# Moryu-Io/Roboken-FMSKF-robot-controller

Hardware: AMD Instinct MI355X
Metric: KF predict+update steps/s (whole node), 6-state fp32, at 1/2/4/8 MI355X (higher is better)
Workload: dtype f32; 1 GPU; cfg2: 2^20 independent 6-state fp32 KF instances per GPU, fused correct+predict per tick (fmskf_tick; every ensemble_every-th tick fmskf_tick_ensemble_begin: the tick kernel also writes the ensemble record, its fold carried by the next tick, libfmskf's ncclAllGather + copy-out on a side stream, fmskf_ensemble_end two events later); instances_per_gpu=1048576, global_instances=1048576, trig=table512, inputs=records, ensemble_every=16, ensemble=fused, gather=native, parallelism=instance-sharded x1

## Files before the change

roboken-fmskf-robot-controller_amd/csrc/api_comm.cpp:

```cpp
#include <dlfcn.h>
#include <elf.h>

#include <atomic>

#include "api_ctx.hpp"

using namespace fmskf;
using namespace fmskf::capi;

namespace fmskf {
namespace capi {

bool ens_exchanges(const fmskf_ctx *h) { return h->comm && h->world > 1; }
double *ens_fold_dst(const fmskf_ctx *h, const fmskf_ctx::EnsSlot &S) { return ens_exchanges(h) ? S.rec : S.host_dev; }
void ens_gather_async(fmskf_ctx *h, fmskf_ctx::EnsSlot &S);
void ens_fold_queued(fmskf_ctx *h, fmskf_ctx::EnsSlot &S) {
  if (ens_exchanges(h)) ens_gather_async(h, S);
  else hip_check(hipEventRecord(S.done, h->stream), "hipEventRecord");
  h->ens_carry = -1;
}
fmskf_ctx::EnsSlot *ens_carry_attach(fmskf_ctx *h, TickIn &t) {
  if (h->ens_carry < 0) return nullptr;
  fmskf_ctx::EnsSlot &C = h->eslot[h->ens_carry];
  t.fold_blocks = C.blocks;
  t.fold_nb = (uint32_t)C.nb;
  t.fold_out = ens_fold_dst(h, C);
  t.ens_shift = h->ens_shift;
  if (!ens_exchanges(h) && !h->timing) t.ens_done = C.done;
  return &C;
}
void ens_carry_launched(fmskf_ctx *h, fmskf_ctx::EnsSlot *C, const TickIn &t) {
  if (!C) return;
  if (t.ens_done) h->ens_carry = -1;
  else ens_fold_queued(h, *C);
}
bool ens_carry_plain() { return FMSKF_ENV_INT("FMSKF_ENS_CARRY_PLAIN", 1) != 0; }
void ens_flush(fmskf_ctx *h) {
  if (h->ens_carry < 0) return;
  fmskf_ctx::EnsSlot &S = h->eslot[h->ens_carry];
  launch_check(launch_ens_fold((int)h->d.nx, S.blocks, S.nb, h->ens_shift, ens_fold_dst(h, S), h->stream),
               "ensemble fold launch");
  ens_fold_queued(h, S);
}

void ensure_shift(fmskf_ctx *h) {
  if (h->ens_shift_ok) return;
  if (h->capturing) fail(FMSKF_EINVAL, "ensemble shift first taken inside a graph capture");
  ens_flush(h);
  launch_check(launch_ens_shift(h->s, (int)h->d.nx, h->d.elem == 8, h->ens_shift, h->stream),
               "ensemble shift launch");
  h->ens_shift_ok = true;
}

bool fused_record(const fmskf_ctx *h) {
  return (h->cfg.model == FMSKF_MODEL_KF6 && !h->gate_on) ||
         (h->cfg.model == FMSKF_MODEL_EKF9 && h->s.tile && !h->rowgate_on) ||
         (h->cfg.model == FMSKF_MODEL_KF12D && h->s.tile && h->kf12.decor);
}

}
}

namespace {

struct RcclApi {
  bool ok = false;
  std::string why;
  std::string path;
  ncclResult_t (*get_unique_id)(ncclUniqueId *) = nullptr;
  ncclResult_t (*comm_init_rank)(ncclComm_t *, int, ncclUniqueId, int) = nullptr;
  ncclResult_t (*comm_destroy)(ncclComm_t) = nullptr;
  ncclResult_t (*all_gather)(const void *, void *, size_t, ncclDataType_t, ncclComm_t, hipStream_t) = nullptr;
  ncclResult_t (*comm_count)(const ncclComm_t, int *) = nullptr;
  ncclResult_t (*comm_user_rank)(const ncclComm_t, int *) = nullptr;
  const char *(*error_string)(ncclResult_t) = nullptr;
};

bool elf_exports(const char *path, const char *name) {
  FILE *f = fopen(path, "rb");
  if (!f) return false;
  std::vector<unsigned char> img;
  unsigned char buf[1 << 16];
  size_t got;
  while ((got = fread(buf, 1, sizeof(buf), f)) > 0 && img.size() < ((size_t)256 << 20)) img.insert(img.end(), buf, buf + got);
  fclose(f);
  if (img.size() < sizeof(Elf64_Ehdr) || memcmp(img.data(), ELFMAG, SELFMAG) != 0 || img[EI_CLASS] != ELFCLASS64)
    return false;
  Elf64_Ehdr eh;
  memcpy(&eh, img.data(), sizeof(eh));
  const uint64_t size = img.size();
  auto within = [size](uint64_t off, uint64_t len) { return off <= size && len <= size - off; };
  if (eh.e_shentsize != sizeof(Elf64_Shdr) || eh.e_shoff > size ||
      eh.e_shnum > (size - eh.e_shoff) / sizeof(Elf64_Shdr))
    return false;
  auto shdr = [&](uint32_t k) {
    Elf64_Shdr sh;
    memcpy(&sh, img.data() + eh.e_shoff + (uint64_t)k * sizeof(Elf64_Shdr), sizeof(sh));
    return sh;
  };
  const size_t nlen = strlen(name);
  for (uint32_t k = 0; k < eh.e_shnum; k++) {
    const Elf64_Shdr sy = shdr(k);
    if (sy.sh_type != SHT_DYNSYM || sy.sh_link >= eh.e_shnum || !within(sy.sh_offset, sy.sh_size)) continue;
    const Elf64_Shdr st = shdr(sy.sh_link);
    if (!within(st.sh_offset, st.sh_size)) continue;
    for (uint64_t o = 0; o + sizeof(Elf64_Sym) <= sy.sh_size; o += sizeof(Elf64_Sym)) {
      Elf64_Sym sym;
      memcpy(&sym, img.data() + sy.sh_offset + o, sizeof(sym));
      if (sym.st_shndx == SHN_UNDEF || sym.st_name >= st.sh_size || nlen >= st.sh_size - sym.st_name) continue;
      if (memcmp(img.data() + st.sh_offset + sym.st_name, name, nlen + 1) == 0) return true;
    }
  }
  return false;
}

std::atomic<const RcclApi *> g_rccl_loaded{nullptr};

const RcclApi &rccl() {
  static RcclApi api = [] {
    RcclApi a;
    const char *alt = getenv("FMSKF_RCCL_LIBRARY");
    void *lib = nullptr;
    if (alt && *alt) {
      if (!elf_exports(alt, "fmskf_rccl_stand_in")) {
        a.why = std::string("FMSKF_RCCL_LIBRARY=") + alt + " is not the test stand-in (no fmskf_rccl_stand_in)";
        return a;
      }
      lib = dlopen(alt, RTLD_NOW | RTLD_LOCAL);
    } else {
      lib = dlopen("librccl.so.1", RTLD_NOW | RTLD_GLOBAL);
      if (!lib) lib = dlopen("/opt/rocm/lib/librccl.so.1", RTLD_NOW | RTLD_GLOBAL);
    }
    if (!lib) {
      a.why = std::string("cannot load librccl.so.1: ") + dlerror();
      return a;
    }
    a.get_unique_id = (decltype(a.get_unique_id))dlsym(lib, "ncclGetUniqueId");
    a.comm_init_rank = (decltype(a.comm_init_rank))dlsym(lib, "ncclCommInitRank");
    a.comm_destroy = (decltype(a.comm_destroy))dlsym(lib, "ncclCommDestroy");
    a.all_gather = (decltype(a.all_gather))dlsym(lib, "ncclAllGather");
    a.comm_count = (decltype(a.comm_count))dlsym(lib, "ncclCommCount");
    a.comm_user_rank = (decltype(a.comm_user_rank))dlsym(lib, "ncclCommUserRank");
    a.error_string = (decltype(a.error_string))dlsym(lib, "ncclGetErrorString");
    a.ok = a.get_unique_id && a.comm_init_rank && a.comm_destroy && a.all_gather && a.comm_count &&
           a.comm_user_rank && a.error_string;
    if (!a.ok) a.why = "librccl.so.1 lacks an entry point";
    Dl_info di{};
    if (a.all_gather && dladdr((void *)a.all_gather, &di) && di.dli_fname) a.path = di.dli_fname;
    return a;
  }();
  g_rccl_loaded.store(&api, std::memory_order_release);
  return api;
}

const RcclApi &need_rccl() {
  const RcclApi &a = rccl();
  if (!a.ok) fail(FMSKF_ERCCL, a.why);
  return a;
}

void nccl_check(ncclResult_t r, const char *what) {
  if (r != ncclSuccess) fail(FMSKF_ERCCL, std::string(what) + ": " + rccl().error_string(r));
}

}

void fmskf::capi::ens_gather_async(fmskf_ctx *h, fmskf_ctx::EnsSlot &S) {
  if (!h->ens_stream) {
    int lo = 0, hi = 0;
    hip_check(hipDeviceGetStreamPriorityRange(&lo, &hi), "hipDeviceGetStreamPriorityRange");
    hip_check(hipStreamCreateWithPriority(&h->ens_stream, hipStreamNonBlocking, hi), "hipStreamCreate");
    hip_check(hipEventCreateWithFlags(&h->ens_ticked, kSyncEvent), "hipEventCreate");
  }
  const uint32_t nx = h->d.nx, len = 1 + nx + nx * (nx + 1) / 2;
  const bool xtime = FMSKF_ENV_INT("FMSKF_ENS_XTIME", 1) != 0;
  if (xtime && !S.x0) {
    hip_check(hipEventCreate(&S.x0), "hipEventCreate");
    hip_check(hipEventCreate(&S.x1), "hipEventCreate");
  }
  hip_check(hipEventRecord(h->ens_ticked, h->stream), "hipEventRecord");
  hip_check(hipStreamWaitEvent(h->ens_stream, h->ens_ticked, 0), "hipStreamWaitEvent");
  if (xtime) hip_check(hipEventRecord(S.x0, h->ens_stream), "hipEventRecord");
  nccl_check(need_rccl().all_gather(S.rec, S.gather, len, ncclFloat64, h->comm, h->ens_stream),
             "ncclAllGather");
  hip_check(hipMemcpyAsync(S.host, S.gather, (size_t)S.ranks * len * 8, hipMemcpyDeviceToHost, h->ens_stream),
            "D2H");
  if (xtime) hip_check(hipEventRecord(S.x1, h->ens_stream), "hipEventRecord");
  hip_check(hipEventRecord(S.done, h->ens_stream), "hipEventRecord");
  S.exchanged = xtime;
}


void fmskf_ctx::destroy_comm() {
  if (comm) {
    (void)rccl().comm_destroy(comm);
    comm = nullptr;
  }
}

extern "C" {

int fmskf_comm_unique_id(uint8_t id[FMSKF_COMM_ID_BYTES]) {
  static_assert(sizeof(ncclUniqueId) == FMSKF_COMM_ID_BYTES, "RCCL unique id size");
  return guarded([&] {
    if (!id) fail(FMSKF_EINVAL, "null id");
    ncclUniqueId u;
    nccl_check(need_rccl().get_unique_id(&u), "ncclGetUniqueId");
    memcpy(id, &u, sizeof(u));
  });
}

int fmskf_comm_init(fmskf_handle h, const uint8_t id[FMSKF_COMM_ID_BYTES], int rank, int world) {
  return guarded([&] {
    check_handle(h);
    if (!id || world < 1 || rank < 0 || rank >= world) fail(FMSKF_EINVAL, "bad rank / world / id");
    if (h->ens_pending) fail(FMSKF_EINVAL, "collect the pending ensemble results (fmskf_ensemble_end) first");
    const RcclApi &a = need_rccl();
    DeviceGuard g(h->cfg.device);
    h->destroy_comm();
    h->rank = 0;
    h->world = 1;
    if ((size_t)world > h->ens_gather_cap) {
      double *buf = h->alloc<double>((size_t)world * 91);
      h->release(h->ens_gather);
      h->ens_gather = buf;
      h->ens_gather_cap = (size_t)world;
    }
    ncclUniqueId u;
    memcpy(&u, id, sizeof(u));
    ncclComm_t c = nullptr;
    nccl_check(a.comm_init_rank(&c, world, u, rank), "ncclCommInitRank");
    h->comm = c;
    h->rank = rank;
    h->world = world;
  });
}

int fmskf_comm_info(fmskf_handle h, int *world, int *rank) {
  return guarded([&] {
    check_handle(h);
    if (!h->comm) fail(FMSKF_EINVAL, "the handle has no communicator (fmskf_comm_init)");
    const RcclApi &a = need_rccl();
    int w = 0, r = -1;
    nccl_check(a.comm_count(h->comm, &w), "ncclCommCount");
    nccl_check(a.comm_user_rank(h->comm, &r), "ncclCommUserRank");
    if (world) *world = w;
    if (rank) *rank = r;
  });
}

const char *fmskf_rccl_library(void) {
  const RcclApi *a = g_rccl_loaded.load(std::memory_order_acquire);
  return a ? a->path.c_str() : "";
}

int fmskf_ensemble_stats(fmskf_handle h, double *mean, double *cov_packed) {
  return guarded([&] {
    check_handle(h);
    DeviceGuard g(h->cfg.device);
    const uint32_t nx = h->d.nx, len = 1 + nx + nx * (nx + 1) / 2;
    ensure_shift(h);
    launch_check(launch_ensemble(h->s, (int)nx, h->d.elem == 8, h->ens_blocks, h->ens_shift, h->ens_out,
                                 h->stream),
                 "ensemble launch");
    const double *src = h->ens_out;
    int ranks = 1;
    if (h->comm) {
      nccl_check(need_rccl().all_gather(h->ens_out, h->ens_gather, len, ncclFloat64, h->comm,
                                        h->stream),
                 "ncclAllGather");
      src = h->ens_gather;
      ranks = h->world;
    }
    std::vector<double> recs((size_t)ranks * len);
    hip_check(hipMemcpyAsync(recs.data(), src, recs.size() * 8, hipMemcpyDeviceToHost, h->stream),
              "D2H");
    hip_check(hipStreamSynchronize(h->stream), "hipStreamSynchronize");
    const int rc = fmskf_ensemble_combine(nx, recs.data(), (uint32_t)ranks, mean, cov_packed);
    if (rc != FMSKF_OK) fail(rc, "ensemble combine");
  });
}

}

namespace {


void ens_async_begin(fmskf_ctx *h, const fmskf_tick_inputs *in) {
  check_handle(h);
  if (h->capturing) fail(FMSKF_EINVAL, "asynchronous ensemble inside a graph capture");
  if (h->ens_pending == fmskf_ctx::kEnsSlots)
    fail(FMSKF_EINVAL, "four ensemble results pending: call fmskf_ensemble_end first");
  DeviceGuard g(h->cfg.device);
  const uint32_t nx = h->d.nx, len = 1 + nx + nx * (nx + 1) / 2;
  const int ranks = ens_exchanges(h) ? h->world : 1;
  const int si = (h->ens_head + h->ens_pending) % fmskf_ctx::kEnsSlots;
  fmskf_ctx::EnsSlot &S = h->eslot[si];
  if (!S.blocks) {
    size_t nb = (size_t)ensemble_nblocks(h->s.n);
    nb = std::max(nb, (size_t)((h->s.n + kBlock - 1) / kBlock));
    S.blocks = h->alloc<double>(nb * len);
    S.rec = h->alloc<double>(91);
    hip_check(hipEventCreateWithFlags(&S.done, kSyncEvent), "hipEventCreate");
  }
  if ((size_t)ranks > S.cap) {
    double *gbuf = h->alloc<double>((size_t)ranks * 91);
    if (S.gather) h->release(S.gather);
    S.gather = gbuf;
    if (S.host) hip_check(hipHostFree(S.host), "hipHostFree");
    S.host = nullptr;
    hip_check(hipHostMalloc((void **)&S.host, (size_t)ranks * 91 * 8, hipHostMallocMapped | hipHostMallocCoherent),
              "hipHostMalloc");
    S.host_dev = (double *)fmskf_ctx::dev_ptr(S.host);
    S.cap = (size_t)ranks;
  }
  ensure_shift(h);
  int nb = 0;
  if (in && fused_record(h)) {
    TickIn t = resolve_inputs(h, in, true, true, 1, h->s.n);
    t.ens_blocks = S.blocks;
    t.ens_shift = h->ens_shift;
    fmskf_ctx::EnsSlot *C = ens_carry_attach(h, t);
    const bool libm = h->cfg.trig == FMSKF_TRIG_LIBM;
    h->time_begin();
    int e = 0;
    if (h->cfg.model == FMSKF_MODEL_KF6) e = launch_kf6(h->s, t, h->kf6, libm, true, true, h->stream, &nb);
    else if (h->cfg.model == FMSKF_MODEL_EKF9) e = launch_ekf9(h->s, t, h->ekf9, libm, true, true, h->stream, &nb);
    else e = launch_kf12d(h->s, t, h->kf12, true, true, h->stream, &nb);
    launch_check(e, "tick kernel launch");
    h->time_end();
    ens_carry_launched(h, C, t);
  } else {
    ens_flush(h);
    if (in) run_tick(h, in, true, true, 1, h->s.n);
    launch_check(launch_ens_partial(h->s, (int)nx, h->d.elem == 8, S.blocks, h->ens_shift, h->stream, &nb),
                 "ensemble partial launch");
  }
  S.nb = nb;
  S.ranks = ranks;
  S.exchanged = false;
  h->ens_carry = si;
  h->ens_pending++;
}

}

extern "C" {

int fmskf_tick_ensemble_begin(fmskf_handle h, const fmskf_tick_inputs *in) {
  return guarded([&] {
    if (!in) fail(FMSKF_EINVAL, "null inputs");
    ens_async_begin(h, in);
  });
}

int fmskf_ensemble_begin(fmskf_handle h) {
  return guarded([&] { ens_async_begin(h, nullptr); });
}

int fmskf_ensemble_end(fmskf_handle h, double *mean, double *cov_packed) {
  return fmskf_ensemble_end_count(h, mean, cov_packed, nullptr, nullptr);
}

int fmskf_ensemble_end_count(fmskf_handle h, double *mean, double *cov_packed, double *count,
                             uint32_t *n_records) {
  return guarded([&] {
    check_handle(h);
    if (h->ens_pending == 0) fail(FMSKF_EINVAL, "no ensemble pending (fmskf_*ensemble_begin)");
    DeviceGuard g(h->cfg.device);
    fmskf_ctx::EnsSlot &S = h->eslot[h->ens_head];
    if (h->ens_carry == h->ens_head) {
      if (h->capturing) fail(FMSKF_EINVAL, "the newest ensemble result collected inside a graph capture");
      ens_flush(h);
    }
    hip_check(hipEventSynchronize(S.done), "hipEventSynchronize");
    h->ens_xms = -1.f;
    if (S.exchanged) {
      hip_check(hipEventElapsedTime(&h->ens_xms, S.x0, S.x1), "hipEventElapsedTime");
      S.exchanged = false;
    }
    h->ens_head = (h->ens_head + 1) % fmskf_ctx::kEnsSlots;
    h->ens_pending--;
    const int rc = fmskf_ensemble_combine(h->d.nx, S.host, (uint32_t)S.ranks, mean, cov_packed);
    if (rc != FMSKF_OK) fail(rc, "ensemble combine");
    const uint32_t len = 1 + h->d.nx + h->d.nx * (h->d.nx + 1) / 2;
    double c = 0.0;
    for (int r = 0; r < S.ranks; r++) c += S.host[(size_t)r * len];
    if (count) *count = c;
    if (n_records) *n_records = (uint32_t)S.ranks;
  });
}

int fmskf_ensemble_exchange_ms(fmskf_handle h, float *ms) {
  return guarded([&] {
    check_handle(h);
    if (!ms) fail(FMSKF_EINVAL, "null ms");
    *ms = h->ens_xms;
  });
}

}
```

roboken-fmskf-robot-controller_amd/csrc/api_ctrl.cpp:

```cpp
#include "api_ctx.hpp"

using namespace fmskf;
using namespace fmskf::capi;

namespace {

void ctrl_params_defaults(fmskf_ctrl_params *p) {
  memset(p, 0, sizeof(*p));
  p->ctrl_freq_hz = 100.0f;
  p->ff_gain = 0.0075f;
  p->p_gain = 0.02f;
  p->i_gain = 0.01f;
  p->d_gain = 0.0f;
  p->i_limit = 0.5f;
  p->lpf_freq_hz = 10.0f;
  p->ff_limit = 1.0f;
  p->interp_ts = 1.0f / (float)1000;
  p->curr_limit_raw = 3000;
}

CtrlPrm make_ctrl_prm(const fmskf_ctx *h) {
  const fmskf_ctrl_params &c = h->cprm;
  CtrlPrm p{};
  p.freq = c.ctrl_freq_hz;
  p.dt = 1.0f / c.ctrl_freq_hz;
  p.ff_gain = c.ff_gain;
  p.p_gain = c.p_gain;
  p.i_gain = c.i_gain;
  p.d_gain = c.d_gain;
  p.i_limit = c.i_limit;
  p.ff_limit = c.ff_limit;
  p.a1 = (2.0f * c.ctrl_freq_hz - c.lpf_freq_hz) / (2.0f * c.ctrl_freq_hz + c.lpf_freq_hz);
  p.b0 = c.lpf_freq_hz / (2.0f * c.ctrl_freq_hz + c.lpf_freq_hz);
  p.b1 = c.lpf_freq_hz / (2.0f * c.ctrl_freq_hz + c.lpf_freq_hz);
  p.ts = c.interp_ts;
  p.curr_limit = c.curr_limit_raw;
  for (int w = 0; w < 4; w++) p.dir[w] = h->cfg.motor_dir[w];
  return p;
}

CtrlPrm ctrl_step_prm(fmskf_ctx *h) {
  CtrlPrm p = make_ctrl_prm(h);
  p.store_derived = h->capturing ? 1u : 0u;
  if (h->capturing) {
    h->graph_has_ctrl = true;
  } else {
    h->ctrl_prm_last = p;
    h->ctrl_derived_stale = true;
  }
  return p;
}

}

namespace fmskf {
namespace capi {

void ctrl_materialize(fmskf_ctx *h) {
  if (!h->ctrl_ready || !h->ctrl_derived_stale) return;
  launch_check(launch_ctrl_derive(h->ctrl, h->ctrl_prm_last, h->stream), "control outputs");
  h->ctrl_derived_stale = false;
}

void zero_ctrl(fmskf_ctx *h) {
  CtrlDev &c = h->ctrl;
  hip_check(hipMemsetAsync(c.ax, 0, (size_t)3 * kAxF * c.pitch * 4, h->stream), "ctrl init");
  hip_check(hipMemsetAsync(c.pid, 0, (size_t)4 * kPidF * c.pitch * 4, h->stream), "ctrl init");
  hip_check(hipMemsetAsync(c.vel_tgt, 0, (size_t)3 * c.pitch * 4, h->stream), "ctrl init");
  hip_check(hipMemsetAsync(c.rpm_prev, 0, (size_t)4 * c.n * 2, h->stream), "ctrl init");
  hip_check(hipMemsetAsync(c.curr, 0, (size_t)4 * c.n * 2, h->stream), "ctrl init");
  hip_check(hipMemsetAsync(c.power, 0, (size_t)c.n, h->stream), "ctrl init");
  ctrl_params_defaults(&h->cprm);
  h->ctrl_derived_stale = false;
}

void ensure_ctrl(fmskf_ctx *h) {
  if (h->ctrl_ready) return;
  CtrlDev &c = h->ctrl;
  c.n = h->s.n;
  const uint64_t w = tile_w_elem(4);
  c.pitch = std::max(h->s.pitch, (c.n + w - 1) / w * w);
  c.ax = h->alloc<float>((size_t)3 * kAxF * c.pitch);
  c.pid = h->alloc<float>((size_t)4 * kPidF * c.pitch);
  c.vel_tgt = h->alloc<float>((size_t)3 * c.pitch);
  c.rpm_prev = h->alloc<int16_t>((size_t)4 * c.n);
  c.curr = h->alloc<int16_t>((size_t)4 * c.n);
  c.power = h->alloc<uint8_t>((size_t)c.n);
  zero_ctrl(h);
  h->ctrl_ready = true;
}

}
}

extern "C" {

int fmskf_ctrl_params_init(fmskf_ctrl_params *p) {
  return guarded([&] {
    if (!p) fail(FMSKF_EINVAL, "null params");
    ctrl_params_defaults(p);
  });
}

int fmskf_set_ctrl_params(fmskf_handle h, const fmskf_ctrl_params *p) {
  return guarded([&] {
    check_handle(h);
    if (!p) fail(FMSKF_EINVAL, "null params");
    if (!(p->ctrl_freq_hz > 0.0f) || !(p->interp_ts > 0.0f) || p->curr_limit_raw < 0)
      fail(FMSKF_EINVAL, "ctrl params: freq and ts must be > 0, current limit >= 0");
    DeviceGuard g(h->cfg.device);
    ensure_ctrl(h);
    h->cprm = *p;
  });
}

int fmskf_set_power(fmskf_handle h, const uint8_t *on, uint32_t mem) {
  return guarded([&] {
    check_handle(h);
    DeviceGuard g(h->cfg.device);
    ensure_ctrl(h);
    ctrl_materialize(h);
    const uint64_t n = h->s.n;
    if (!on) {
      hip_check(hipMemsetAsync(h->ctrl.power, 1, n, h->stream), "power");
      return;
    }
    if (mem != FMSKF_MEM_HOST && mem != FMSKF_MEM_DEVICE) fail(FMSKF_EINVAL, "bad mem flag");
    hip_check(hipMemcpyAsync(h->ctrl.power, on, n,
                             mem == FMSKF_MEM_HOST ? hipMemcpyHostToDevice : hipMemcpyDeviceToDevice,
                             h->stream),
              "power");
    finish_out(h, mem);
  });
}

int fmskf_set_target_vel(fmskf_handle h, const float *vel, const float *acl, const float *jrk,
                         const uint8_t *mask, uint32_t mem) {
  return guarded([&] {
    check_handle(h);
    if (!vel || !acl || !jrk) fail(FMSKF_EINVAL, "null vel/acl/jrk");
    DeviceGuard g(h->cfg.device);
    ensure_ctrl(h);
    const uint64_t n = h->s.n;
    Stager sg(h, mem);
    const void *v = vel, *a = acl, *j = jrk, *m = mask;
    sg.add(&v, 3 * n * 4);
    sg.add(&a, 3 * n * 4);
    sg.add(&j, 3 * n * 4);
    sg.add(&m, n);
    sg.run();
    launch_check(launch_ctrl_set_target(h->ctrl, (const float *)v, (const float *)a,
                                        (const float *)j, (const uint8_t *)m, h->stream),
                 "set_target_vel launch");
  });
}

int fmskf_control(fmskf_handle h, const int16_t *rpm, uint32_t mem) {
  return guarded([&] {
    check_handle(h);
    DeviceGuard g(h->cfg.device);
    ensure_ctrl(h);
    const void *r = rpm;
    if (r) {
      Stager sg(h, mem);
      sg.add(&r, h->s.n * 8);
      sg.run();
    } else {
      ensure_motors(h);
      r = h->s.m_rpm;
    }
    h->time_begin();
    launch_check(launch_ctrl_step(h->ctrl, ctrl_step_prm(h), (const int16_t *)r, 1, h->stream),
                 "control launch");
    h->time_end();
  });
}

int fmskf_can_tx(fmskf_handle h, uint8_t *frames, uint32_t mem) {
  return guarded([&] {
    check_handle(h);
    if (!frames) fail(FMSKF_EINVAL, "null frames");
    if (mem != FMSKF_MEM_HOST && mem != FMSKF_MEM_DEVICE) fail(FMSKF_EINVAL, "bad mem flag");
    DeviceGuard g(h->cfg.device);
    ensure_ctrl(h);
    const size_t bytes = h->s.n * 8;
    uint8_t *dst = mem == FMSKF_MEM_DEVICE ? frames : (uint8_t *)host_result(h, bytes);
    launch_check(launch_can_tx(h->ctrl, dst, h->stream), "can_tx launch");
    copy_out_sync(h, frames, dst, bytes, mem);
  });
}

static bool rs_prev_skip() { return FMSKF_ENV_INT("FMSKF_RS_PREV_SKIP", 1) != 0; }
static bool isr_kf6_fused() { return FMSKF_ENV_INT("FMSKF_ISR_FUSED", 1) != 0; }

static void isr_launches(fmskf_ctx *h, const TickIn &t, uint8_t *dst) {
  const bool libm = h->cfg.trig == FMSKF_TRIG_LIBM;
  const CtrlPrm p = ctrl_step_prm(h);
  int fused = (int)hipErrorNotSupported;
  if (h->cfg.model == FMSKF_MODEL_KF6 && isr_kf6_fused() && !h->gate_on) {
    if (!t.rec && !t.rpm) ensure_motors(h);
    fused = launch_isr_kf6(h->s, t, h->kf6, libm, h->ctrl, p, dst, h->stream);
    if (fused != (int)hipErrorNotSupported) launch_check(fused, "isr launch");
  } else if (h->cfg.model == FMSKF_MODEL_EKF9 && isr_kf6_fused() && !h->rowgate_on) {
    if (!t.rpm) ensure_motors(h);
    fused = launch_isr_ekf9(h->s, t, h->ekf9, libm, h->ctrl, p, t.rpm ? t.rpm : h->s.m_rpm, dst, h->stream);
    if (fused != (int)hipErrorNotSupported) launch_check(fused, "isr launch");
  }
  if (h->cfg.model == FMSKF_MODEL_RS) {
    rs_prev_materialize(h);
    launch_check(launch_isr_rs(h->s, t, libm, h->ctrl, p, dst, h->stream), "isr launch");
    h->rs_prev_synced = t.msum_lo != nullptr;
  } else if (fused == (int)hipErrorNotSupported) {
    h->isr_ctrl_split++;
    int e = 0;
    switch (h->cfg.model) {
      case FMSKF_MODEL_KF6: e = kf6_tick_launch(h, t, libm, true, true); break;
      case FMSKF_MODEL_EKF9: e = ekf9_tick_launch(h, t, libm, true, true); break;
      case FMSKF_MODEL_KF12D: e = launch_kf12d(h->s, t, h->kf12, true, true, h->stream); break;
    }
    launch_check(e, "tick kernel launch");
    if (!t.rec && !t.rpm) ensure_motors(h);
    const int16_t *rpm = t.rec ? (const int16_t *)(t.rec + 2) : t.rpm ? t.rpm : h->s.m_rpm;
    launch_check(launch_ctrl_step(h->ctrl, p, rpm, t.rec ? 2 : 1, h->stream), "control launch");
    if (dst) launch_check(launch_can_tx(h->ctrl, dst, h->stream), "can_tx launch");
  }
}

int fmskf_isr_tick(fmskf_handle h, const fmskf_tick_inputs *in, uint8_t *frames, uint32_t mem) {
  return guarded([&] {
    check_handle(h);
    if (frames && mem != FMSKF_MEM_HOST && mem != FMSKF_MEM_DEVICE) fail(FMSKF_EINVAL, "bad mem flag");
    DeviceGuard g(h->cfg.device);
    ensure_ctrl(h);
    const uint64_t n = h->s.n;
    const TickIn t = resolve_inputs(h, in, true, true, 1, n);
    const size_t bytes = n * 8;
    uint8_t *dst = !frames ? nullptr : mem == FMSKF_MEM_DEVICE ? frames : (uint8_t *)host_result(h, bytes);
    h->time_begin();
    isr_launches(h, t, dst);
    h->time_end();
    if (frames) copy_out_sync(h, frames, dst, bytes, mem);
  });
}

int fmskf_isr_tick_can(fmskf_handle h, const uint8_t *can_frames, const int16_t *can_stamps,
                       const fmskf_tick_inputs *in, uint8_t *frames, uint32_t mem) {
  return guarded([&] {
    check_handle(h);
    if (!can_frames || !can_stamps) fail(FMSKF_EINVAL, "null can_frames/can_stamps");
    if (!in) fail(FMSKF_EINVAL, "null inputs");
    if (mem != FMSKF_MEM_HOST && mem != FMSKF_MEM_DEVICE) fail(FMSKF_EINVAL, "bad mem flag");
    DeviceGuard g(h->cfg.device);
    ensure_ctrl(h);
    ensure_motors(h);
    const uint64_t n = h->s.n;
    const void *f = can_frames, *s = can_stamps;
    std::vector<std::pair<const void **, size_t>> cf{{&f, n * 32}, {&s, n * 8}};
    const bool together = in->mem == mem;
    const TickIn t = resolve_inputs(h, in, true, true, 1, n, together ? &cf : nullptr);
    if (!together) {
      Stager sg(h, mem);
      for (const auto &it : cf) sg.add(it.first, it.second);
      sg.run();
    }
    const bool libm = h->cfg.trig == FMSKF_TRIG_LIBM;
    const size_t bytes = n * 8;
    uint8_t *dst = !frames ? nullptr : mem == FMSKF_MEM_DEVICE ? frames : (uint8_t *)host_result(h, bytes);
    int fused = (int)hipErrorNotSupported;
    h->time_begin();
    if (h->cfg.model == FMSKF_MODEL_KF6 && isr_kf6_fused() && !h->gate_on && !in->kf6_rec && !in->rpm) {
      fused = launch_isr_kf6_can(h->s, t, h->kf6, libm, h->ctrl, ctrl_step_prm(h), dst, (const uint8_t *)f,
                                 (const int16_t *)s, h->cfg.motor_dir, h->stream);
    } else if (h->cfg.model == FMSKF_MODEL_EKF9 && isr_kf6_fused() && !h->rowgate_on && !in->rpm) {
      fused = launch_isr_ekf9_can(h->s, t, h->ekf9, libm, h->ctrl, ctrl_step_prm(h), dst, (const uint8_t *)f,
                                  (const int16_t *)s, h->cfg.motor_dir, h->stream);
    } else if (h->cfg.model == FMSKF_MODEL_RS && !in->rpm && !in->angle_sum) {
      const bool ps = h->rs_prev_synced && !h->capturing && rs_prev_skip();
      if (!ps) rs_prev_materialize(h);
      fused = launch_isr_rs_can(h->s, t, libm, h->ctrl, ctrl_step_prm(h), dst, (const uint8_t *)f,
                                (const int16_t *)s, h->cfg.motor_dir, ps, h->stream);
      if (fused != (int)hipErrorNotSupported) {
        h->rs_prev_synced = true;
        h->rs_prev_stale = h->rs_prev_stale || ps;
      }
    }
    if (fused != (int)hipErrorNotSupported) {
      launch_check(fused, "isr+can launch");
      h->s.m_par ^= 1u;
    }
    if (fused == (int)hipErrorNotSupported) {
      h->isr_can_split++;
      rs_prev_materialize(h);
      h->rs_prev_synced = false;
      launch_check(launch_can(h->s, (const uint8_t *)f, (const int16_t *)s, nullptr, h->cfg.motor_dir, h->stream),
                   "can launch");
      h->s.m_par ^= 1u;
      isr_launches(h, t, dst);
    }
    h->time_end();
    if (frames) copy_out_sync(h, frames, dst, bytes, mem);
  });
}

int fmskf_get_ctrl(fmskf_handle h, float *vel_tgt, int16_t *curr_raw, float *wheel_tgt,
                   float *wheel_ctrl, uint32_t mem) {
  return guarded([&] {
    check_handle(h);
    DeviceGuard g(h->cfg.device);
    ensure_ctrl(h);
    ctrl_materialize(h);
    const CtrlDev &c = h->ctrl;
    const size_t row = c.n * 4, pb = c.pitch * 4;
    copy_planes_out(h, vel_tgt, c.vel_tgt, row, pb, 3, mem);
    copy_out(h, curr_raw, c.curr, c.n * 8, mem);
    if (wheel_tgt || wheel_ctrl) {
      float *dense = (float *)h->stage_for((size_t)4 * kPidF * row);
      launch_check(launch_untile(c.pid, dense, 4 * kPidF, c.n, 4, h->stream), "untile pid");
      copy_planes_out(h, wheel_tgt, dense + 4 * c.n, row, row * kPidF, 4, mem);
      copy_planes_out(h, wheel_ctrl, dense + 5 * c.n, row, row * kPidF, 4, mem);
    }
    finish_out(h, mem);
  });
}

int fmskf_export_vehicle_info(fmskf_handle h, fmskf_vehicle_info *out, const uint8_t *floor,
                              const float *cam_pitch, const uint32_t *fault, uint32_t mem) {
  static_assert(sizeof(fmskf_vehicle_info) == 84, "VehicleInfo record layout");
  return guarded([&] {
    check_handle(h);
    if (!out) fail(FMSKF_EINVAL, "null out");
    DeviceGuard g(h->cfg.device);
    const uint64_t n = h->s.n;
    ensure_imu(h);
    Stager sg(h, mem);
    const void *f = floor, *c = cam_pitch, *u = fault;
    sg.add(&f, n * 8);
    sg.add(&c, n * 4);
    sg.add(&u, n * 4);
    sg.run();
    launch_check(launch_readout(h->s, h->readout, h->stream), "readout");
    const size_t bytes = n * sizeof(fmskf_vehicle_info);
    void *dst = mem == FMSKF_MEM_DEVICE ? (void *)out : host_result(h, bytes);
    launch_check(launch_vehicle_info(h->s, h->readout, dst, (const uint8_t *)f, (const float *)c,
                                     (const uint32_t *)u, h->stream),
                 "vehicle_info launch");
    copy_out_sync(h, out, dst, bytes, mem);
  });
}

int fmskf_eval_trig(fmskf_handle h, const float *x, float *s, float *c, uint64_t n, uint32_t mem) {
  return guarded([&] {
    check_handle(h);
    if (!x || !s || !c) fail(FMSKF_EINVAL, "null argument");
    DeviceGuard g(h->cfg.device);
    const bool libm = h->cfg.trig == FMSKF_TRIG_LIBM;
    if (mem == FMSKF_MEM_DEVICE) {
      launch_check(launch_trig(x, s, c, n, libm, h->s.sintab, h->stream), "trig launch");
      return;
    }
    if (mem != FMSKF_MEM_HOST) fail(FMSKF_EINVAL, "bad mem flag");
    if (n == 0) return;
    char *buf = (char *)h->stage_for(3 * n * 4);
    float *dx = (float *)buf, *ds = dx + n, *dc = ds + n;
    hip_check(hipMemcpyAsync(dx, x, n * 4, hipMemcpyHostToDevice, h->stream), "H2D");
    launch_check(launch_trig(dx, ds, dc, n, libm, h->s.sintab, h->stream), "trig launch");
    hip_check(hipMemcpyAsync(s, ds, n * 4, hipMemcpyDeviceToHost, h->stream), "D2H");
    hip_check(hipMemcpyAsync(c, dc, n * 4, hipMemcpyDeviceToHost, h->stream), "D2H");
    hip_check(hipStreamSynchronize(h->stream), "sync");
  });
}

int fmskf_set_timing(fmskf_handle h, int enable) {
  return guarded([&] {
    check_handle(h);
    h->timing = enable != 0;
    h->tcount = 0;
  });
}

int fmskf_kernel_time_total(fmskf_handle h, double *total_ms, uint32_t *count) {
  return guarded([&] {
    check_handle(h);
    if (!total_ms || !count) fail(FMSKF_EINVAL, "null argument");
    DeviceGuard g(h->cfg.device);
    double sum = 0.0;
    if (h->tcount) hip_check(hipEventSynchronize(h->tpool[2 * h->tcount - 1]), "hipEventSynchronize");
    for (size_t k = 0; k < h->tcount; k++) {
      float ms = 0.f;
      hip_check(hipEventElapsedTime(&ms, h->tpool[2 * k], h->tpool[2 * k + 1]), "hipEventElapsedTime");
      sum += ms;
    }
    *total_ms = sum;
    *count = (uint32_t)h->tcount;
  });
}

int fmskf_last_kernel_ms(fmskf_handle h, float *ms) {
  return guarded([&] {
    check_handle(h);
    if (!ms) fail(FMSKF_EINVAL, "null ms");
    if (!h->timing) fail(FMSKF_EINVAL, "timing not enabled");
    DeviceGuard g(h->cfg.device);
    hip_check(hipEventSynchronize(h->ev1), "hipEventSynchronize");
    hip_check(hipEventElapsedTime(ms, h->ev0, h->ev1), "hipEventElapsedTime");
  });
}

}
```

roboken-fmskf-robot-controller_amd/csrc/api_ctx.hpp:

```cpp
#pragma once
#include "../../include/fmskf.h"

#include <hip/hip_runtime.h>
#include <math.h>
#include <rccl/rccl.h>
#include <stdio.h>
#include <stdlib.h>
#include <string.h>

#include <algorithm>
#include <string>
#include <vector>

#include "fmskf_internal.hpp"
#include "window_pieces.hpp"

namespace fmskf {
namespace capi {

extern thread_local std::string g_last_error;

struct ApiError {
  int code;
  std::string msg;
};

[[noreturn]] inline void fail(int code, const std::string &msg) { throw ApiError{code, msg}; }

inline void hip_check(hipError_t e, const char *what) {
  if (e != hipSuccess) fail(FMSKF_EDEVICE, std::string(what) + ": " + hipGetErrorString(e));
}
inline void launch_check(int e, const char *what) { hip_check((hipError_t)e, what); }
constexpr unsigned kSyncEvent = hipEventDisableTiming | hipEventDisableSystemFence;

template <class F>
int guarded(F &&f) {
  try {
    g_last_error.clear();
    f();
    return FMSKF_OK;
  } catch (const ApiError &e) {
    g_last_error = e.msg;
    return e.code;
  } catch (const std::bad_alloc &) {
    g_last_error = "host allocation failed";
    return FMSKF_ENOMEM;
  } catch (...) {
    g_last_error = "unexpected exception";
    return FMSKF_EDEVICE;
  }
}

struct DeviceGuard {
  int prev = -1;
  explicit DeviceGuard(int dev) {
    hip_check(hipGetDevice(&prev), "hipGetDevice");
    if (prev != dev) hip_check(hipSetDevice(dev), "hipSetDevice");
  }
  ~DeviceGuard() {
    int cur = -1;
    if (hipGetDevice(&cur) == hipSuccess && cur != prev && prev >= 0) (void)hipSetDevice(prev);
  }
};

struct Dims {
  uint32_t nx, m, elem;
};

inline Dims dims_of(uint32_t model) {
  switch (model) {
    case FMSKF_MODEL_RS: return {6, 0, 4};
    case FMSKF_MODEL_KF6: return {6, 4, 4};
    case FMSKF_MODEL_EKF9: return {9, 6, 4};
    case FMSKF_MODEL_KF12D: return {12, 8, 8};
    default: fail(FMSKF_EINVAL, "unknown model");
  }
}

}
}


struct fmskf_ctx {
  fmskf_config cfg{};
  fmskf::capi::Dims d{};
  fmskf::DevState s{};
  hipStream_t stream = nullptr;
  std::vector<void *> allocs;
  void *stage = nullptr;
  size_t stage_bytes = 0;
  static constexpr size_t kPinned = (size_t)1 << 20;
  void *pin_in[2] = {nullptr, nullptr};
  hipEvent_t pin_ev[2] = {nullptr, nullptr};
  bool pin_open[2] = {false, false};
  int pin_slot = 0;
  void *pin_out = nullptr;
  double *ens_blocks = nullptr;
  double *ens_out = nullptr;
  double *ens_shift = nullptr;
  bool ens_shift_ok = false;
  size_t ens_gather_cap = 0;
  float *readout = nullptr;
  void *oscratch = nullptr;
  size_t oscratch_bytes = 0;
  hipGraph_t graph = nullptr;
  hipGraphExec_t graph_exec = nullptr;
  bool capturing = false;
  ncclComm_t comm = nullptr;
  int rank = 0, world = 1;
  double *ens_gather = nullptr;
  static constexpr int kEnsSlots = 4;
  struct EnsSlot {
    double *blocks = nullptr, *rec = nullptr, *gather = nullptr;
    double *host = nullptr;
    double *host_dev = nullptr;
    size_t cap = 0;
    hipEvent_t done = nullptr;
    hipEvent_t x0 = nullptr, x1 = nullptr;
    bool exchanged = false;
    int nb = 0;
    int ranks = 1;
  } eslot[kEnsSlots];
  hipEvent_t ens_ticked = nullptr;
  hipStream_t ens_stream = nullptr;
  int ens_head = 0, ens_pending = 0;
  int ens_carry = -1;
  float ens_xms = -1.f;
  fmskf::CtrlDev ctrl{};
  fmskf_ctrl_params cprm{};
  bool ctrl_ready = false;
  fmskf::Kf6Params kf6{};
  fmskf::Ekf9Params ekf9{};
  fmskf::Kf12dParams kf12{};
  bool gate_on = false;
  fmskf::GateDev gate{};
  bool rowgate_on = false;
  fmskf::RowGateDev rowgate{};
  unsigned long long *fix_ignored = nullptr;
  unsigned long long *subset_ignored = nullptr;
  float *anchors = nullptr;
  std::vector<float> anchors_host;
  uint32_t n_anchors = 0;
  unsigned long long *range_ignored = nullptr;
  uint8_t *sel_flag = nullptr;
  uint32_t *sel_blk = nullptr, *sel_chunk = nullptr;
  void *smooth_ws = nullptr;
  size_t smooth_ws_bytes = 0;
  double *loglik_partial = nullptr;
  double *em_partial = nullptr;
  uint64_t isr_can_split = 0, isr_ctrl_split = 0;
  bool rs_prev_synced = false, rs_prev_stale = false;
  bool ctrl_derived_stale = false, graph_has_ctrl = false;
  uint32_t graph_par0 = 0, graph_par_end = 0;
  fmskf::CtrlPrm ctrl_prm_last{};
  bool timing = false;
  hipEvent_t ev0 = nullptr, ev1 = nullptr;
  std::vector<hipEvent_t> tpool;
  size_t tcount = 0;
  static constexpr size_t kMaxTimed = 65536;

  void time_begin() {
    if (!timing) return;
    if (tcount < kMaxTimed) {
      while (tpool.size() < 2 * (tcount + 1)) {
        hipEvent_t e;
        fmskf::capi::hip_check(hipEventCreate(&e), "hipEventCreate");
        tpool.push_back(e);
      }
      fmskf::capi::hip_check(hipEventRecord(tpool[2 * tcount], stream), "hipEventRecord");
    }
    fmskf::capi::hip_check(hipEventRecord(ev0, stream), "hipEventRecord");
  }
  void time_end() {
    if (!timing) return;
    fmskf::capi::hip_check(hipEventRecord(ev1, stream), "hipEventRecord");
    if (tcount < kMaxTimed) {
      fmskf::capi::hip_check(hipEventRecord(tpool[2 * tcount + 1], stream), "hipEventRecord");
      tcount++;
    }
  }

  template <typename T>
  T *alloc(size_t count) {
    void *p = nullptr;
    if (count == 0) count = 1;
    hipError_t e = hipMalloc(&p, count * sizeof(T));
    if (e != hipSuccess) fmskf::capi::fail(FMSKF_ENOMEM, std::string("hipMalloc: ") + hipGetErrorString(e));
    allocs.push_back(p);
    return (T *)p;
  }
  void release(void *p) {
    if (!p) return;
    for (size_t i = 0; i < allocs.size(); i++)
      if (allocs[i] == p) {
        fmskf::capi::hip_check(hipStreamSynchronize(stream), "hipStreamSynchronize");
        (void)hipFree(p);
        allocs.erase(allocs.begin() + (long)i);
        return;
      }
  }
  void *stage_for(size_t bytes) {
    if (bytes > stage_bytes) {
      if (stage) {
        fmskf::capi::hip_check(hipStreamSynchronize(stream), "hipStreamSynchronize");
        fmskf::capi::hip_check(hipFree(stage), "hipFree");
        stage = nullptr;
        stage_bytes = 0;
      }
      hipError_t e = hipMalloc(&stage, bytes);
      if (e != hipSuccess) fmskf::capi::fail(FMSKF_ENOMEM, "staging hipMalloc failed");
      stage_bytes = bytes;
    }
    return stage;
  }
  char *pinned_in() {
    const int prev = pin_slot ^ 1, slot = pin_slot;
    if (pin_open[prev]) {
      fmskf::capi::hip_check(hipEventRecord(pin_ev[prev], stream), "hipEventRecord");
      pin_open[prev] = false;
    }
    pin_slot ^= 1;
    if (!pin_in[slot]) {
      fmskf::capi::hip_check(hipHostMalloc(&pin_in[slot], kPinned, hipHostMallocDefault), "hipHostMalloc");
      fmskf::capi::hip_check(hipEventCreateWithFlags(&pin_ev[slot], fmskf::capi::kSyncEvent), "hipEventCreate");
    } else {
      fmskf::capi::hip_check(hipEventSynchronize(pin_ev[slot]), "hipEventSynchronize");
    }
    pin_open[slot] = true;
    return (char *)pin_in[slot];
  }
  char *pinned_out() {
    if (!pin_out) fmskf::capi::hip_check(hipHostMalloc(&pin_out, kPinned, hipHostMallocDefault), "hipHostMalloc");
    return (char *)pin_out;
  }
  static void *dev_ptr(void *host) {
    void *d = nullptr;
    fmskf::capi::hip_check(hipHostGetDevicePointer(&d, host, 0), "hipHostGetDevicePointer");
    return d;
  }
  void destroy_comm();
  void *out_for(size_t bytes) {
    if (bytes > oscratch_bytes) {
      if (oscratch) {
        fmskf::capi::hip_check(hipStreamSynchronize(stream), "hipStreamSynchronize");
        fmskf::capi::hip_check(hipFree(oscratch), "hipFree");
        oscratch = nullptr;
        oscratch_bytes = 0;
      }
      hipError_t e = hipMalloc(&oscratch, bytes);
      if (e != hipSuccess) {
        oscratch = nullptr;
        (void)hipGetLastError();
        fmskf::capi::fail(FMSKF_ENOMEM, "output scratch hipMalloc failed");
      }
      oscratch_bytes = bytes;
    }
    return oscratch;
  }
  ~fmskf_ctx() {
    if (ens_stream) (void)hipStreamSynchronize(ens_stream);
    if (stream) (void)hipStreamSynchronize(stream);
    else (void)hipDeviceSynchronize();
    for (void *p : allocs) (void)hipFree(p);
    if (stage) (void)hipFree(stage);
    if (oscratch) (void)hipFree(oscratch);
    if (smooth_ws) (void)hipFree(smooth_ws);
    if (loglik_partial) (void)hipFree(loglik_partial);
    if (em_partial) (void)hipFree(em_partial);
    for (int k = 0; k < 2; k++) {
      if (pin_in[k]) (void)hipHostFree(pin_in[k]);
      if (pin_ev[k]) (void)hipEventDestroy(pin_ev[k]);
    }
    if (pin_out) (void)hipHostFree(pin_out);
    for (EnsSlot &e : eslot) {
      if (e.host) (void)hipHostFree(e.host);
      if (e.done) (void)hipEventDestroy(e.done);
      if (e.x0) (void)hipEventDestroy(e.x0);
      if (e.x1) (void)hipEventDestroy(e.x1);
    }
    if (ens_ticked) (void)hipEventDestroy(ens_ticked);
    if (ens_stream) (void)hipStreamDestroy(ens_stream);
    destroy_comm();
    if (graph_exec) (void)hipGraphExecDestroy(graph_exec);
    if (graph) (void)hipGraphDestroy(graph);
    if (ev0) (void)hipEventDestroy(ev0);
    if (ev1) (void)hipEventDestroy(ev1);
    for (hipEvent_t e : tpool) (void)hipEventDestroy(e);
  }
};

namespace fmskf {
namespace capi {

inline void check_handle(fmskf_handle h) {
  if (!h) fail(FMSKF_EINVAL, "null handle");
}


struct Stager {
  fmskf_ctx *h;
  bool host;
  std::vector<std::pair<const void **, size_t>> items;
  Stager(fmskf_ctx *hh, uint32_t mem) : h(hh), host(mem == FMSKF_MEM_HOST) {
    if (mem != FMSKF_MEM_HOST && mem != FMSKF_MEM_DEVICE) fail(FMSKF_EINVAL, "bad mem flag");
  }
  void add(const void **p, size_t bytes) {
    if (*p && host) items.push_back({p, bytes});
  }
  void run() {
    if (!host || items.empty()) return;
    size_t total = 0;
    for (auto &it : items) total += (it.second + 255) & ~size_t(255);
    size_t off = 0;
    if (total <= fmskf_ctx::kPinned && !h->capturing) {
      char *pin = h->pinned_in();
      char *base = (char *)fmskf_ctx::dev_ptr(pin);
      for (auto &it : items) {
        memcpy(pin + off, *it.first, it.second);
        *it.first = base + off;
        off += (it.second + 255) & ~size_t(255);
      }
      return;
    }
    char *base = (char *)h->stage_for(total);
    for (auto &it : items) {
      hip_check(hipMemcpyAsync(base + off, *it.first, it.second, hipMemcpyHostToDevice, h->stream),
                "stage H2D");
      *it.first = base + off;
      off += (it.second + 255) & ~size_t(255);
    }
  }
};

void zero_imu(fmskf_ctx *h);
void zero_motors(fmskf_ctx *h);
void ensure_imu(fmskf_ctx *h);
void ensure_motors(fmskf_ctx *h);
void rs_prev_materialize(fmskf_ctx *h);
TickIn resolve_inputs(fmskf_ctx *h, const fmskf_tick_inputs *in, bool need_upd, bool need_pred,
                      uint32_t n_ticks, uint64_t stride,
                      const std::vector<std::pair<const void **, size_t>> *extra = nullptr);
void run_tick(fmskf_ctx *h, const fmskf_tick_inputs *in, bool upd, bool pred, uint32_t n_ticks,
              uint64_t stride);
inline int kf6_tick_launch(fmskf_ctx *h, const TickIn &t, bool libm, bool upd, bool pred) {
  if (h->gate_on && upd) return launch_kf6_gate(h->s, t, h->kf6, h->gate, libm, pred, h->stream);
  return launch_kf6(h->s, t, h->kf6, libm, upd, pred, h->stream);
}
void zero_gate(fmskf_ctx *h);
inline int ekf9_tick_launch(fmskf_ctx *h, const TickIn &t, bool libm, bool upd, bool pred) {
  if (h->rowgate_on && upd) return launch_ekf9_rowgate(h->s, t, h->ekf9, h->rowgate, libm, pred, h->stream);
  return launch_ekf9(h->s, t, h->ekf9, libm, upd, pred, h->stream);
}
void zero_rowgate(fmskf_ctx *h);
void copy_out(fmskf_ctx *h, void *dst, const void *src, size_t bytes, uint32_t mem);
void copy_planes_out(fmskf_ctx *h, void *dst, const void *src, size_t row, size_t dev_pitch,
                     size_t planes, uint32_t mem);
void copy_planes_in(fmskf_ctx *h, void *dst, const void *src, size_t row, size_t dev_pitch,
                    size_t planes, uint32_t mem);
void finish_out(fmskf_ctx *h, uint32_t mem);
void *host_result(fmskf_ctx *h, size_t bytes);
void copy_out_sync(fmskf_ctx *h, void *dst, const void *src, size_t bytes, uint32_t mem);
void check_list_model(const fmskf_ctx *h, const char *what);
struct EntryOut {
  float *value = nullptr;
  uint8_t *status = nullptr;
  EntryOut(fmskf_ctx *h, float *value, uint8_t *status, uint64_t count, uint32_t mem);
  void deliver();

 private:
  fmskf_ctx *h;
  float *user_value;
  uint8_t *user_status;
  size_t count;
  uint32_t mem;
  char *res = nullptr;
};
double *ens_fold_dst(const fmskf_ctx *h, const fmskf_ctx::EnsSlot &S);
void ens_fold_queued(fmskf_ctx *h, fmskf_ctx::EnsSlot &S);
fmskf_ctx::EnsSlot *ens_carry_attach(fmskf_ctx *h, TickIn &t);
void ens_carry_launched(fmskf_ctx *h, fmskf_ctx::EnsSlot *C, const TickIn &t);
bool ens_carry_plain();
void ens_flush(fmskf_ctx *h);
void ensure_shift(fmskf_ctx *h);
bool fused_record(const fmskf_ctx *h);
SmoothHist smooth_hist(fmskf_ctx *h, uint32_t n_ticks);
void ensure_ctrl(fmskf_ctx *h);
void zero_ctrl(fmskf_ctx *h);
void ctrl_materialize(fmskf_ctx *h);


inline void check_window_model(const fmskf_ctx *h, const char *what) {
  const std::string w(what);
  if (h->cfg.model != FMSKF_MODEL_KF6) fail(FMSKF_ENOTSUP, w + " for KF6");
  if (h->cfg.flags & FMSKF_CFG_COMP_POS) fail(FMSKF_ENOTSUP, w + " for KF6 without FMSKF_CFG_COMP_POS");
  if (h->gate_on) fail(FMSKF_ENOTSUP, w + " for a KF6 handle without a gate (fmskf_set_gate)");
}

inline uint64_t bytes_mul(uint64_t a, uint64_t b, const char *what) {
  uint64_t r;
  if (!bytes_fit(a, b, &r)) fail(FMSKF_ENOMEM, std::string(what) + " too large");
  return r;
}

template <class F>
void window_call(fmskf_ctx *h, const char *name, const char *what, uint32_t mem, uint64_t pitch, bool misaligned,
                 const fmskf_tick_inputs *in, uint32_t n_ticks, uint64_t tick_stride, F &&body) {
  const std::string w(what), captured = std::string(name) + " cannot be captured";
  if (mem != FMSKF_MEM_HOST && mem != FMSKF_MEM_DEVICE) fail(FMSKF_EINVAL, "bad mem flag");
  if (pitch && pitch < h->s.n) fail(FMSKF_EINVAL, w + " output pitch < N");
  if (n_ticks == 0) fail(FMSKF_EINVAL, "n_ticks == 0");
  if (mem == FMSKF_MEM_DEVICE && misaligned) fail(FMSKF_EINVAL, "misaligned " + w + " device output");
  if (h->capturing) fail(FMSKF_EINVAL, captured);
  DeviceGuard g(h->cfg.device);
  hipStreamCaptureStatus cs = hipStreamCaptureStatusNone;
  if (h->stream && hipStreamIsCapturing(h->stream, &cs) == hipSuccess && cs != hipStreamCaptureStatusNone)
    fail(FMSKF_EINVAL, captured);
  TickIn t = resolve_inputs(h, in, true, true, n_ticks, tick_stride);
  body(t);
}

inline double *ensure_partial(fmskf_ctx *h, double **slot, size_t K, const char *what) {
  if (!*slot) {
    const size_t blocks = (size_t)((h->s.n + kBlock - 1) / kBlock);
    const hipError_t e = hipMalloc((void **)slot, K * blocks * sizeof(double));
    if (e != hipSuccess) {
      *slot = nullptr;
      (void)hipGetLastError();
      fail(FMSKF_ENOMEM, std::string(what) + " scratch hipMalloc: " + hipGetErrorString(e));
    }
  }
  return *slot;
}

inline char *stage_pieces(fmskf_ctx *h, Piece *pc, int count, const char *what) {
  uint64_t bytes;
  if (!plan_pieces(pc, count, &bytes)) fail(FMSKF_ENOMEM, std::string(what) + " output staging too large");
  return (char *)h->out_for(bytes);
}
template <class T>
T *piece_at(char *stg, const Piece &p) {
  return p.user ? (T *)(stg + p.off) : nullptr;
}
inline void pieces_in(fmskf_ctx *h, const Piece *pc, int count, const char *what) {
  const std::string msg = std::string(what) + " outputs H2D";
  for (int k = 0; k < count; k++)
    if (pc[k].user)
      hip_check(hipMemcpy2DAsync((char *)h->oscratch + pc[k].off, pc[k].step_bytes(), pc[k].user, pc[k].step_bytes(),
                                 pc[k].row_bytes(), pc[k].rows, hipMemcpyHostToDevice, h->stream), msg.c_str());
}
inline void pieces_out(fmskf_ctx *h, const Piece *pc, int count, const char *what) {
  const std::string msg = std::string(what) + " outputs D2H";
  for (int k = 0; k < count; k++)
    if (pc[k].user)
      hip_check(hipMemcpy2DAsync(pc[k].user, pc[k].step_bytes(), (char *)h->oscratch + pc[k].off, pc[k].step_bytes(),
                                 pc[k].row_bytes(), pc[k].rows, hipMemcpyDeviceToHost, h->stream), msg.c_str());
  finish_out(h, FMSKF_MEM_HOST);
}

template <class F, class B>
void timed_passes(fmskf_ctx *h, F &&fwd, B &&bwd) {
  const char *e = env_knob("FMSKF_SMOOTH_TIME");
  const int only = !e ? 0 : !strcmp(e, "fwd") ? 1 : !strcmp(e, "bwd") ? 2 : 0;
  if (only != 2) h->time_begin();
  fwd();
  if (only == 1) h->time_end();
  if (only == 2) h->time_begin();
  bwd();
  if (only != 1) h->time_end();
}

}
}
```

roboken-fmskf-robot-controller_amd/csrc/api_handle.cpp:

```cpp
#include "api_ctx.hpp"

using namespace fmskf;
using namespace fmskf::capi;

thread_local std::string fmskf::capi::g_last_error;

namespace {

void apply_defaults(fmskf_config *c, uint32_t model, uint64_t n) {
  memset(c, 0, sizeof(*c));
  c->abi_version = FMSKF_ABI_VERSION;
  c->model = model;
  c->n_instances = n;
  c->device = 0;
  c->trig = FMSKF_TRIG_TABLE512;
  c->dt = 0.001;
  c->motor_dir[0] = 1;
  c->motor_dir[1] = 1;
  c->motor_dir[2] = -1;
  c->motor_dir[3] = -1;
  c->imu_read_reg = 0x51;
  const double dt = c->dt;
  auto setq = [&](int i, int j, double v) { c->q[i * (i + 1) / 2 + j] = v; };
  auto setr = [&](int i, int j, double v) { c->r[i * (i + 1) / 2 + j] = v; };
  auto setp = [&](int i, double v) { c->p0[i * (i + 1) / 2 + i] = v; };
  auto cv_block = [&](int p, int v, double qc) {
    setq(p, p, qc * dt * dt * dt / 3.0);
    setq(v, p, qc * dt * dt / 2.0);
    setq(v, v, qc * dt);
  };
  switch (model) {
    case FMSKF_MODEL_KF6:
      cv_block(0, 3, 4.0);
      cv_block(1, 4, 4.0);
      cv_block(2, 5, 100.0);
      setr(0, 0, 2.5e-5);
      setr(1, 1, 2.5e-3);
      setr(2, 2, 4e-4);
      setr(3, 3, 4e-4);
      setr(3, 2, 1e-5);
      for (int i = 0; i < 6; i++) setp(i, i < 3 ? 1.0 : 0.25);
      break;
    case FMSKF_MODEL_EKF9: {
      const double qd[9] = {1e-10, 1e-10, 1e-10, 4e-3 * dt, 4e-3 * dt, 100.0 * dt, 1e-12, 2500.0 * dt, 2500.0 * dt};
      for (int i = 0; i < 9; i++) setq(i, i, qd[i]);
      const double rd[6] = {2.5e-5, 2.5e-3, 0.25, 0.25, 4e-4, 4e-4};
      for (int i = 0; i < 6; i++) setr(i, i, rd[i]);
      for (int i = 0; i < 9; i++) setp(i, i < 3 ? 1.0 : (i == 6 ? 1e-2 : 0.25));
      break;
    }
    case FMSKF_MODEL_KF12D: {
      cv_block(0, 3, 4.0);
      cv_block(1, 4, 4.0);
      cv_block(2, 5, 100.0);
      cv_block(6, 9, 1.0);
      cv_block(7, 10, 1.0);
      cv_block(8, 11, 1.0);
      const double rd[8] = {2.5e-5, 2.5e-3, 4e-4, 4e-4, 1e-6, 1e-6, 1e-6, 1e-4};
      for (int i = 0; i < 8; i++) setr(i, i, rd[i]);
      setr(3, 2, 1e-5);
      for (int i = 0; i < 12; i++) setp(i, (i % 6) < 3 ? 1.0 : 0.25);
      break;
    }
    default: break;
  }
}

void convert_params(fmskf_ctx *h) {
  const fmskf_config &c = h->cfg;
  h->kf6.dt = (float)c.dt;
  for (int k = 0; k < 21; k++) h->kf6.q[k] = (float)c.q[k];
  for (int k = 0; k < 10; k++) h->kf6.r[k] = (float)c.r[k];
  h->ekf9.dt = (float)c.dt;
  for (int k = 0; k < 45; k++) h->ekf9.q[k] = (float)c.q[k];
  for (int k = 0; k < 21; k++) h->ekf9.r[k] = (float)c.r[k];
  h->kf12.dt = c.dt;
  for (int k = 0; k < 78; k++) h->kf12.q[k] = c.q[k];
  for (int k = 0; k < 36; k++) h->kf12.r[k] = c.r[k];
  for (int a = 0; a < 4; a++)
    for (int b = 0; b <= a; b++) h->kf12.r2[a * (a + 1) / 2 + b] = c.r[(a + 4) * (a + 5) / 2 + (b + 4)];
  h->kf12.decor = kf12d_cinv(h->kf12.r, h->kf12.cinv) ? 1 : 0;
  h->kf12.sparse = h->kf12.decor && kf12d_sparse(h->kf12.cinv, h->kf12.q) ? 1 : 0;
}

}

namespace fmskf {
namespace capi {

void zero_imu(fmskf_ctx *h) {
  DevState &s = h->s;
  const uint64_t n = s.n;
  hipStream_t st = h->stream;
  hip_check(hipMemsetAsync(s.imu_reg, 0, 0x90 * n * 2, st), "reset imu");
  hip_check(hipMemsetAsync(s.imu_parser, 0, 3 * n * 4, st), "reset imu");
  hip_check(hipMemsetAsync(s.imu_cnt, 0, n, st), "reset imu");
  hip_check(hipMemsetAsync(s.imu_flags, 0, n, st), "reset imu");
  hip_check(hipMemsetAsync(s.imu_err, 0, n, st), "reset imu");
  hip_check(hipMemsetAsync(s.imu_qinit, 0, 4 * n * 4, st), "reset imu");
  hip_check(hipMemsetAsync(s.imu_snap, 0, kRowWords * n * 2, st), "reset imu");
  hip_check(hipMemsetAsync(s.imu_mag, 0, 4 * n * 2, st), "reset imu");
  hip_check(hipMemsetAsync(s.imu_yg, 0, n * 4, st), "reset imu");
  hip_check(hipMemsetAsync(s.imu_qprev, 0, 4 * n * 4, st), "reset imu");
}
void zero_motors(fmskf_ctx *h) {
  DevState &s = h->s;
  const uint64_t n = s.n;
  hipStream_t st = h->stream;
  hip_check(hipMemsetAsync(s.m_micro, 0, 4 * n * 2, st), "reset motors");
  hip_check(hipMemsetAsync(s.m_angle, 0, 4 * n * 2, st), "reset motors");
  hip_check(hipMemsetAsync(s.m_prev, 0, 4 * n * 2, st), "reset motors");
  hip_check(hipMemsetAsync(s.m_rpm, 0, 4 * n * 2, st), "reset motors");
  hip_check(hipMemsetAsync(s.m_curr, 0, 4 * n * 2, st), "reset motors");
  hip_check(hipMemsetAsync(s.m_sum_lo, 0, 4 * n * 4, st), "reset motors");
  hip_check(hipMemsetAsync(s.m_sum_hi, 0, 4 * n * 4, st), "reset motors");
  hip_check(hipMemsetAsync(s.m_iir_y, 0, 4 * n * 4, st), "reset motors");
  hip_check(hipMemsetAsync(s.m_prev_micro, 0, 4 * n * 2, st), "reset motors");
}

void ensure_imu(fmskf_ctx *h) {
  DevState &s = h->s;
  if (s.imu_reg) return;
  if (h->capturing) fail(FMSKF_EINVAL, "IMU state first used inside a graph capture");
  const uint64_t n = s.n;
  s.imu_reg = h->alloc<int16_t>(0x90 * n);
  s.imu_parser = h->alloc<uint32_t>(3 * n);
  s.imu_cnt = h->alloc<uint8_t>(n);
  s.imu_flags = h->alloc<uint8_t>(n);
  s.imu_err = h->alloc<uint8_t>(n);
  s.imu_qinit = h->alloc<float>(4 * n);
  s.imu_snap = h->alloc<int16_t>(kRowWords * n);
  s.imu_mag = h->alloc<int16_t>(4 * n);
  s.imu_yg = h->alloc<uint32_t>(n);
  s.imu_qprev = h->alloc<float>(4 * n);
  zero_imu(h);
}
void rs_prev_materialize(fmskf_ctx *h) {
  if (!h->rs_prev_stale) return;
  const DevState &s = h->s;
  launch_check(launch_motor_sums(s.m_sum_lo, s.m_sum_hi, s.prev_sum, s.n, 0, true, h->stream), "previous sums");
  h->rs_prev_stale = false;
}

void zero_gate(fmskf_ctx *h) {
  if (!h->gate.word) return;
  hip_check(hipMemsetAsync(h->gate.word, 0, h->s.n * 4, h->stream), "reset gate");
  hip_check(hipMemsetAsync(h->gate.nis, 0, h->s.n * 4, h->stream), "reset gate");
}

void zero_rowgate(fmskf_ctx *h) {
  if (!h->rowgate.word) return;
  hip_check(hipMemsetAsync(h->rowgate.word, 0, h->s.n * 8, h->stream), "reset row gate");
  hip_check(hipMemsetAsync(h->rowgate.d2, 0, (size_t)FMSKF_EKF9_ROWS * h->rowgate.d2_pitch * 4, h->stream),
            "reset row gate");
}

void ensure_motors(fmskf_ctx *h) {
  DevState &s = h->s;
  if (s.m_sum_lo) return;
  if (h->capturing) fail(FMSKF_EINVAL, "motor state first used inside a graph capture");
  const uint64_t n = s.n;
  s.m_micro = h->alloc<int16_t>(4 * n);
  s.m_angle = h->alloc<int16_t>(4 * n);
  s.m_prev = h->alloc<int16_t>(4 * n);
  s.m_rpm = h->alloc<int16_t>(4 * n);
  s.m_curr = h->alloc<int16_t>(4 * n);
  s.m_sum_lo = h->alloc<uint32_t>(4 * n);
  s.m_sum_hi = h->alloc<int32_t>(4 * n);
  s.m_iir_y = h->alloc<float>(4 * n);
  s.m_prev_micro = h->alloc<int16_t>(4 * n);
  zero_motors(h);
}

}
}

namespace {

void do_reset(fmskf_ctx *h) {
  DevState &s = h->s;
  const uint64_t n = s.n;
  const Dims d = h->d;
  const uint32_t np = d.nx * (d.nx + 1) / 2;
  hipStream_t st = h->stream;
  const uint64_t pp = s.pitch;
  hip_check(hipMemsetAsync(s.x, 0, (size_t)d.nx * pp * d.elem, st), "reset x");
  if (d.m > 0) {
    std::vector<uint64_t> bits(np);
    for (uint32_t k = 0; k < np; k++) {
      const double v = h->cfg.p0[k];
      if (d.elem == 4) {
        const float f = (float)v;
        uint32_t b;
        memcpy(&b, &f, 4);
        bits[k] = b;
      } else {
        memcpy(&bits[k], &v, 8);
      }
    }
    launch_check(launch_tiled_fill(s.P, np, n, bits.data(), d.elem, st), "reset P0");
  }
  if (s.prev_sum) hip_check(hipMemsetAsync(s.prev_sum, 0, 4 * pp * 8, st), "reset prev");
  if (s.thlo) hip_check(hipMemsetAsync(s.thlo, 0, n * 4, st), "reset heading low part");
  if (s.xlo) hip_check(hipMemsetAsync(s.xlo, 0, (size_t)kKf6LoRows * pp * 4, st), "reset position low parts");
  if (s.imu_reg) zero_imu(h);
  if (s.m_sum_lo) zero_motors(h);
  zero_gate(h);
  zero_rowgate(h);
  if (h->ctrl_ready) {
    const CtrlDev &c = h->ctrl;
    hip_check(hipMemsetAsync(c.ax, 0, (size_t)3 * kAxF * c.pitch * 4, st), "reset ctrl");
    hip_check(hipMemsetAsync(c.pid, 0, (size_t)4 * kPidF * c.pitch * 4, st), "reset ctrl");
    hip_check(hipMemsetAsync(c.vel_tgt, 0, (size_t)3 * c.pitch * 4, st), "reset ctrl");
    hip_check(hipMemsetAsync(c.rpm_prev, 0, (size_t)4 * c.n * 2, st), "reset ctrl");
    hip_check(hipMemsetAsync(c.curr, 0, (size_t)4 * c.n * 2, st), "reset ctrl");
    hip_check(hipMemsetAsync(c.power, 0, (size_t)c.n, st), "reset ctrl");
  }
  hip_check(hipMemsetAsync(s.counters, 0, 8 * 8, st), "reset counters");
  hip_check(hipMemsetAsync(h->fix_ignored, 0, 8, st), "reset counters");
  hip_check(hipMemsetAsync(h->subset_ignored, 0, 8, st), "reset counters");
  hip_check(hipMemsetAsync(h->range_ignored, 0, 8, st), "reset counters");
  h->isr_can_split = h->isr_ctrl_split = 0;
  h->rs_prev_synced = h->rs_prev_stale = false;
  h->ctrl_derived_stale = false;
  h->ens_shift_ok = false;
}

}

namespace fmskf {
namespace capi {

TickIn resolve_inputs(fmskf_ctx *h, const fmskf_tick_inputs *in, bool need_upd, bool need_pred,
                      uint32_t n_ticks, uint64_t stride,
                      const std::vector<std::pair<const void **, size_t>> *extra) {
  if (!in) fail(FMSKF_EINVAL, "null inputs");
  DevState &s = h->s;
  const uint64_t n = s.n;
  if (stride < n) fail(FMSKF_EINVAL, "tick_stride < N");
  if (n_ticks == 0) fail(FMSKF_EINVAL, "n_ticks == 0");
  TickIn t{};
  t.yaw_deg = in->yaw_deg;
  t.gyro_z = in->gyro_z_dps;
  t.rpm = in->rpm;
  t.angle_sum = in->angle_sum;
  t.raw = in->raw;
  t.z = in->z;
  t.valid = in->valid;
  t.rec = (const uint32_t *)in->kf6_rec;
  t.sintab = s.sintab;
  t.stride = stride;
  t.sum_pitch = stride;
  t.n_ticks = n_ticks;
  if (t.rec && h->cfg.model != FMSKF_MODEL_KF6) fail(FMSKF_EINVAL, "kf6_rec is a KF6 input");
  if (t.rec && (t.yaw_deg || t.gyro_z || t.rpm))
    fail(FMSKF_EINVAL, "kf6_rec replaces yaw_deg / gyro_z_dps / rpm: pass one or the other");
  if (in->angle_sum_pitch) {
    if (n_ticks != 1 || stride != n) fail(FMSKF_EINVAL, "angle_sum_pitch is for single-tick calls (tick_many: tick_stride)");
    if (in->angle_sum_pitch < n) fail(FMSKF_EINVAL, "angle_sum_pitch < N");
    t.sum_pitch = in->angle_sum_pitch;
  }
  const uint64_t span = (uint64_t)(n_ticks - 1) * stride + n;
  Stager sg(h, in->mem);
  sg.add((const void **)&t.yaw_deg, span * 4);
  sg.add((const void **)&t.gyro_z, span * 4);
  sg.add((const void **)&t.rpm, span * 8);
  sg.add((const void **)&t.angle_sum, ((uint64_t)(n_ticks - 1) * stride * 4 + 3 * t.sum_pitch + n) * 8);
  sg.add((const void **)&t.raw, span * 16);
  sg.add((const void **)&t.z, ((uint64_t)(n_ticks - 1) * stride * 8 + 7 * stride + n) * 8);
  sg.add((const void **)&t.valid, span);
  sg.add((const void **)&t.rec, span * 16);
  if (extra)
    for (const auto &it : *extra) sg.add(it.first, it.second);
  sg.run();
  const bool many = n_ticks > 1 || stride != n;
  auto dev_default = [&](const void *p, const char *name) {
    if (!p && many) fail(FMSKF_EINVAL, std::string("tick_many needs explicit plane ") + name);
  };
  switch (h->cfg.model) {
    case FMSKF_MODEL_RS:
      if (need_upd) {
        dev_default(t.yaw_deg, "yaw_deg");
        if (!t.yaw_deg) {
          ensure_imu(h);
          t.yaw_deg = (const float *)s.imu_yg;
          t.imu_words |= 1u;
        }
      }
      if (need_pred) {
        dev_default(t.rpm, "rpm");
        dev_default(t.angle_sum, "angle_sum");
        if (!t.rpm || !t.angle_sum) ensure_motors(h);
        if (!t.rpm) t.rpm = s.m_rpm;
        if (!t.angle_sum) {
          t.msum_lo = s.m_sum_lo;
          t.msum_hi = s.m_sum_hi;
        }
      }
      break;
    case FMSKF_MODEL_KF6:
      if (need_upd && !t.rec) {
        dev_default(t.yaw_deg, "yaw_deg");
        dev_default(t.gyro_z, "gyro_z_dps");
        dev_default(t.rpm, "rpm");
        if (!t.yaw_deg || !t.gyro_z) ensure_imu(h);
        if (!t.rpm) ensure_motors(h);
        if (!t.yaw_deg) {
          t.yaw_deg = (const float *)s.imu_yg;
          t.imu_words |= 1u;
        }
        if (!t.gyro_z) {
          t.gyro_z = (const float *)s.imu_yg;
          t.imu_words |= 2u;
        }
        if (!t.rpm) t.rpm = s.m_rpm;
      }
      break;
    case FMSKF_MODEL_EKF9:
      if (need_upd && !t.raw) fail(FMSKF_EINVAL, "EKF9 needs raw words");
      break;
    case FMSKF_MODEL_KF12D:
      if (need_upd && !t.z) fail(FMSKF_EINVAL, "KF12D needs z");
      break;
  }
  return t;
}

void run_tick(fmskf_ctx *h, const fmskf_tick_inputs *in, bool upd, bool pred, uint32_t n_ticks,
              uint64_t stride) {
  check_handle(h);
  DeviceGuard g(h->cfg.device);
  TickIn t = resolve_inputs(h, in, upd, pred, n_ticks, stride);
  fmskf_ctx::EnsSlot *C = nullptr;
  if (!h->capturing) {
    if (h->cfg.model == FMSKF_MODEL_KF6 && fused_record(h) && upd && pred && n_ticks == 1 && ens_carry_plain())
      C = ens_carry_attach(h, t);
    else
      ens_flush(h);
  }
  const bool libm = h->cfg.trig == FMSKF_TRIG_LIBM;
  const bool rs_pred = h->cfg.model == FMSKF_MODEL_RS && pred;
  if (rs_pred) rs_prev_materialize(h);
  h->time_begin();
  int e = 0;
  switch (h->cfg.model) {
    case FMSKF_MODEL_RS: e = launch_rs(h->s, t, libm, upd, pred, h->stream); break;
    case FMSKF_MODEL_KF6: e = kf6_tick_launch(h, t, libm, upd, pred); break;
    case FMSKF_MODEL_EKF9: e = ekf9_tick_launch(h, t, libm, upd, pred); break;
    case FMSKF_MODEL_KF12D: e = launch_kf12d(h->s, t, h->kf12, upd, pred, h->stream); break;
  }
  launch_check(e, "tick kernel launch");
  ens_carry_launched(h, C, t);
  if (rs_pred) h->rs_prev_synced = t.msum_lo != nullptr;
  h->time_end();
}

void copy_out(fmskf_ctx *h, void *dst, const void *src, size_t bytes, uint32_t mem) {
  if (!dst) return;
  if (mem == FMSKF_MEM_HOST) {
    hip_check(hipMemcpyAsync(dst, src, bytes, hipMemcpyDeviceToHost, h->stream), "D2H");
  } else if (mem == FMSKF_MEM_DEVICE) {
    hip_check(hipMemcpyAsync(dst, src, bytes, hipMemcpyDeviceToDevice, h->stream), "D2D");
  } else {
    fail(FMSKF_EINVAL, "bad mem flag");
  }
}
void copy_planes_out(fmskf_ctx *h, void *dst, const void *src, size_t row, size_t dev_pitch,
                     size_t planes, uint32_t mem) {
  if (!dst) return;
  if (mem != FMSKF_MEM_HOST && mem != FMSKF_MEM_DEVICE) fail(FMSKF_EINVAL, "bad mem flag");
  const hipMemcpyKind k = mem == FMSKF_MEM_HOST ? hipMemcpyDeviceToHost : hipMemcpyDeviceToDevice;
  hip_check(hipMemcpy2DAsync(dst, row, src, dev_pitch, row, planes, k, h->stream), "copy planes");
}
void copy_planes_in(fmskf_ctx *h, void *dst, const void *src, size_t row, size_t dev_pitch,
                    size_t planes, uint32_t mem) {
  if (mem != FMSKF_MEM_HOST && mem != FMSKF_MEM_DEVICE) fail(FMSKF_EINVAL, "bad mem flag");
  const hipMemcpyKind k = mem == FMSKF_MEM_HOST ? hipMemcpyHostToDevice : hipMemcpyDeviceToDevice;
  hip_check(hipMemcpy2DAsync(dst, dev_pitch, src, row, row, planes, k, h->stream), "copy planes");
}
void finish_out(fmskf_ctx *h, uint32_t mem) {
  if (mem == FMSKF_MEM_HOST) hip_check(hipStreamSynchronize(h->stream), "hipStreamSynchronize");
}
void *host_result(fmskf_ctx *h, size_t bytes) {
  if (bytes <= fmskf_ctx::kPinned && !h->capturing) return fmskf_ctx::dev_ptr(h->pinned_out());
  return h->out_for(bytes);
}
void copy_out_sync(fmskf_ctx *h, void *dst, const void *src, size_t bytes, uint32_t mem) {
  if (mem == FMSKF_MEM_HOST && h->pin_out && src == fmskf_ctx::dev_ptr(h->pin_out)) {
    hip_check(hipStreamSynchronize(h->stream), "hipStreamSynchronize");
    memcpy(dst, h->pin_out, bytes);
    return;
  }
  if (mem == FMSKF_MEM_HOST && bytes <= fmskf_ctx::kPinned && !h->capturing) {
    char *pin = h->pinned_out();
    hip_check(hipMemcpyAsync(pin, src, bytes, hipMemcpyDeviceToHost, h->stream), "D2H");
    hip_check(hipStreamSynchronize(h->stream), "hipStreamSynchronize");
    memcpy(dst, pin, bytes);
    return;
  }
  if (mem == FMSKF_MEM_HOST) copy_out(h, dst, src, bytes, mem);
  finish_out(h, mem);
}

void check_list_model(const fmskf_ctx *h, const char *what) {
  const uint32_t model = h->cfg.model;
  const bool comp = (h->cfg.flags & FMSKF_CFG_COMP_POS) != 0;
  if ((model != FMSKF_MODEL_KF6 && model != FMSKF_MODEL_EKF9) || (model == FMSKF_MODEL_EKF9 && comp))
    fail(FMSKF_ENOTSUP, std::string(what) + " for KF6 (plain, FMSKF_CFG_COMP_POS) and plain EKF9");
}

EntryOut::EntryOut(fmskf_ctx *hh, float *v, uint8_t *s, uint64_t n, uint32_t m)
    : value(v), status(s), h(hh), user_value(v), user_status(s), count((size_t)n), mem(m) {
  if (mem != FMSKF_MEM_HOST || (!v && !s)) return;
  res = (char *)host_result(h, count * 5);
  value = v ? (float *)res : nullptr;
  status = s ? (uint8_t *)res + count * 4 : nullptr;
}
void EntryOut::deliver() {
  if (!res) return;
  if (h->pin_out && res == fmskf_ctx::dev_ptr(h->pin_out)) {
    hip_check(hipStreamSynchronize(h->stream), "hipStreamSynchronize");
    if (user_value) memcpy(user_value, h->pin_out, count * 4);
    if (user_status) memcpy(user_status, (char *)h->pin_out + count * 4, count);
  } else {
    copy_out(h, user_value, res, count * 4, mem);
    copy_out(h, user_status, res + count * 4, count, mem);
    finish_out(h, mem);
  }
}

}
}

extern "C" {

int fmskf_abi_version(void) { return (int)FMSKF_ABI_VERSION; }

const char *fmskf_strerror(int status) {
  switch (status) {
    case FMSKF_OK: return "ok";
    case FMSKF_EINVAL: return "invalid argument";
    case FMSKF_ENOMEM: return "out of memory";
    case FMSKF_EDEVICE: return "device error";
    case FMSKF_ERCCL: return "collective error";
    case FMSKF_ENOTSUP: return "not supported for this model";
    default: return "unknown status";
  }
}

const char *fmskf_last_error(void) { return g_last_error.c_str(); }

int fmskf_model_dims(uint32_t model, uint32_t *n, uint32_t *m, uint32_t *elem_bytes) {
  return guarded([&] {
    Dims d = dims_of(model);
    if (n) *n = d.nx;
    if (m) *m = d.m;
    if (elem_bytes) *elem_bytes = d.elem;
  });
}

int fmskf_config_init(fmskf_config *cfg, uint32_t model, uint64_t n) {
  return guarded([&] {
    if (!cfg) fail(FMSKF_EINVAL, "null config");
    (void)dims_of(model);
    apply_defaults(cfg, model, n);
  });
}

int fmskf_create(const fmskf_config *cfg, fmskf_handle *out) {
  return guarded([&] {
    if (!cfg || !out) fail(FMSKF_EINVAL, "null argument");
    *out = nullptr;
    if (cfg->abi_version != FMSKF_ABI_VERSION) fail(FMSKF_EINVAL, "ABI version mismatch");
    const Dims d = dims_of(cfg->model);
    if (cfg->n_instances == 0) fail(FMSKF_EINVAL, "n_instances == 0");
    if (cfg->n_instances > (1ull << 30)) fail(FMSKF_EINVAL, "n_instances > 2^30 per handle");
    if (cfg->trig > FMSKF_TRIG_LIBM) fail(FMSKF_EINVAL, "bad trig policy");
    if (!(cfg->dt > 0.0) || !isfinite(cfg->dt)) fail(FMSKF_EINVAL, "dt must be > 0");
    if (cfg->imu_read_reg + 4 > 0x90) fail(FMSKF_EINVAL, "imu_read_reg out of range");
    if ((cfg->flags & ~FMSKF_CFG_COMP_POS) || cfg->reserved) fail(FMSKF_EINVAL, "unknown config flags");
    if ((cfg->flags & FMSKF_CFG_COMP_POS) && cfg->model != FMSKF_MODEL_KF6 && cfg->model != FMSKF_MODEL_EKF9)
      fail(FMSKF_ENOTSUP, "FMSKF_CFG_COMP_POS is a KF6 / EKF9 mode");
    for (int w = 0; w < 4; w++)
      if (cfg->motor_dir[w] != 1 && cfg->motor_dir[w] != -1) fail(FMSKF_EINVAL, "motor_dir must be +-1");
    int ndev = 0;
    if (hipGetDeviceCount(&ndev) != hipSuccess || ndev == 0) fail(FMSKF_EDEVICE, "no HIP device");
    if (cfg->device < 0 || cfg->device >= ndev) fail(FMSKF_EINVAL, "bad device ordinal");
    DeviceGuard g(cfg->device);
    fmskf_ctx *h = new fmskf_ctx();
    try {
      h->cfg = *cfg;
      h->d = d;
      const uint64_t n = cfg->n_instances;
      DevState &s = h->s;
      s.n = n;
      s.model = cfg->model;
      const uint32_t np = d.nx * (d.nx + 1) / 2;
      s.tile = cfg->model == FMSKF_MODEL_RS ? 0 : tile_w_elem(d.elem);
      s.pitch = s.tile ? std::max(plane_pitch(n), (n + s.tile - 1) / s.tile * s.tile) : plane_pitch(n);
      s.x = h->alloc<char>((size_t)d.nx * s.pitch * d.elem);
      s.P = d.m ? h->alloc<char>((size_t)np * s.pitch * d.elem) : nullptr;
      s.prev_sum = cfg->model == FMSKF_MODEL_RS ? h->alloc<int64_t>(4 * s.pitch) : nullptr;
      s.thlo = cfg->model == FMSKF_MODEL_EKF9 ? h->alloc<float>(n) : nullptr;
      s.xlo = (cfg->flags & FMSKF_CFG_COMP_POS) ? h->alloc<float>((size_t)kKf6LoRows * s.pitch) : nullptr;
      h->kf6.lo = s.xlo;
      s.counters = h->alloc<unsigned long long>(8);
      h->fix_ignored = h->alloc<unsigned long long>(1);
      h->subset_ignored = h->alloc<unsigned long long>(1);
      h->range_ignored = h->alloc<unsigned long long>(1);
      h->anchors = h->alloc<float>((size_t)FMSKF_RANGE_ANCHORS_MAX * 4);
      s.sintab = h->alloc<float>(513);
      {
        const size_t len = 1 + d.nx + np;
        size_t nb = (size_t)ensemble_nblocks(n);
        if (cfg->model == FMSKF_MODEL_KF6 || cfg->model == FMSKF_MODEL_EKF9 || cfg->model == FMSKF_MODEL_KF12D)
          nb = std::max(nb, (size_t)((n + kBlock - 1) / kBlock));
        h->ens_blocks = h->alloc<double>(nb * len);
        h->ens_out = h->alloc<double>(91);
        h->ens_shift = h->alloc<double>(12);
      }
      h->readout = h->alloc<float>(6 * n);
      static const float tab[513] = {
#include "cmsis_sintab.inc"
      };
      hip_check(hipMemcpy(s.sintab, tab, sizeof(tab), hipMemcpyHostToDevice), "sintab upload");
      hip_check(hipEventCreate(&h->ev0), "hipEventCreate");
      hip_check(hipEventCreate(&h->ev1), "hipEventCreate");
      convert_params(h);
      {
        double *coef = h->alloc<double>(36 + 78);
        hip_check(hipMemcpy(coef, h->kf12.cinv, 36 * sizeof(double), hipMemcpyHostToDevice), "coef upload");
        hip_check(hipMemcpy(coef + 36, h->kf12.q, 78 * sizeof(double), hipMemcpyHostToDevice), "coef upload");
        h->kf12.coef = coef;
      }
      do_reset(h);
      hip_check(hipStreamSynchronize(h->stream), "hipStreamSynchronize");
    } catch (...) {
      delete h;
      throw;
    }
    *out = h;
  });
}

int fmskf_destroy(fmskf_handle h) {
  return guarded([&] {
    if (!h) return;
    DeviceGuard g(h->cfg.device);
    delete h;
  });
}

int fmskf_reset(fmskf_handle h) {
  return guarded([&] {
    check_handle(h);
    DeviceGuard g(h->cfg.device);
    do_reset(h);
  });
}

int fmskf_set_stream(fmskf_handle h, void *stream) {
  return guarded([&] {
    check_handle(h);
    if (h->stream != (hipStream_t)stream && !h->capturing)
      hip_check(hipStreamSynchronize(h->stream), "hipStreamSynchronize");
    h->stream = (hipStream_t)stream;
  });
}

int fmskf_graph_begin(fmskf_handle h) {
  return guarded([&] {
    check_handle(h);
    if (!h->stream) fail(FMSKF_EINVAL, "graph capture needs a stream (fmskf_set_stream)");
    if (h->capturing) fail(FMSKF_EINVAL, "capture already open");
    if (h->timing) fail(FMSKF_EINVAL, "disable per-launch timing before capturing");
    DeviceGuard g(h->cfg.device);
    ensure_imu(h);
    ensure_motors(h);
    ensure_ctrl(h);
    ensure_shift(h);
    rs_prev_materialize(h);
    h->rs_prev_synced = false;
    ctrl_materialize(h);
    h->graph_has_ctrl = false;
    h->graph_par0 = h->s.m_par;
    hip_check(hipStreamBeginCapture(h->stream, hipStreamCaptureModeThreadLocal),
              "hipStreamBeginCapture");
    h->capturing = true;
  });
}

int fmskf_graph_end(fmskf_handle h) {
  return guarded([&] {
    check_handle(h);
    if (!h->capturing) fail(FMSKF_EINVAL, "no capture open");
    DeviceGuard g(h->cfg.device);
    h->capturing = false;
    h->rs_prev_synced = false;
    h->graph_par_end = h->s.m_par;
    h->s.m_par = h->graph_par0;
    hipGraph_t gnew = nullptr;
    hip_check(hipStreamEndCapture(h->stream, &gnew), "hipStreamEndCapture");
    if (h->graph_exec) hip_check(hipGraphExecDestroy(h->graph_exec), "hipGraphExecDestroy");
    if (h->graph) hip_check(hipGraphDestroy(h->graph), "hipGraphDestroy");
    h->graph_exec = nullptr;
    h->graph = gnew;
    hip_check(hipGraphInstantiate(&h->graph_exec, h->graph, nullptr, nullptr, 0),
              "hipGraphInstantiate");
  });
}

int fmskf_graph_launch(fmskf_handle h, uint32_t times) {
  return guarded([&] {
    check_handle(h);
    if (!h->graph_exec) fail(FMSKF_EINVAL, "no graph captured");
    if (h->capturing) fail(FMSKF_EINVAL, "capture still open");
    DeviceGuard g(h->cfg.device);
    rs_prev_materialize(h);
    ctrl_materialize(h);
    for (uint32_t k = 0; k < times; k++) {
      if (h->s.m_par != h->graph_par0) {
        launch_check(launch_motor_swap(h->s, h->stream), "motor history order");
        h->s.m_par ^= 1u;
      }
      hip_check(hipGraphLaunch(h->graph_exec, h->stream), "hipGraphLaunch");
      h->s.m_par = h->graph_par_end;
    }
    h->rs_prev_synced = false;
    if (h->graph_has_ctrl && times > 0) h->ctrl_derived_stale = false;
  });
}

int fmskf_sync(fmskf_handle h) {
  return guarded([&] {
    check_handle(h);
    DeviceGuard g(h->cfg.device);
    hip_check(hipStreamSynchronize(h->stream), "hipStreamSynchronize");
  });
}

int fmskf_get_config(fmskf_handle h, fmskf_config *out) {
  return guarded([&] {
    check_handle(h);
    if (!out) fail(FMSKF_EINVAL, "null out");
    *out = h->cfg;
  });
}

int fmskf_ingest_wt901(fmskf_handle h, const uint8_t *bytes, uint32_t stride, const uint32_t *len,
                       int latch_qinit, uint32_t mem) {
  return guarded([&] {
    check_handle(h);
    if (!bytes || !len) fail(FMSKF_EINVAL, "null bytes/len");
    DeviceGuard g(h->cfg.device);
    const uint64_t n = h->s.n;
    if (mem == FMSKF_MEM_HOST) {
      for (uint64_t i = 0; i < n; i++)
        if (len[i] > stride) fail(FMSKF_EINVAL, "len[i] > stride");
    }
    ensure_imu(h);
    Stager sg(h, mem);
    const void *b = bytes, *l = len;
    sg.add(&b, (size_t)stride * n);
    sg.add(&l, n * 4);
    sg.run();
    launch_check(launch_wt901(h->s, (const uint8_t *)b, stride, (const uint32_t *)l, latch_qinit,
                              h->cfg.imu_read_reg, h->stream),
                 "wt901 launch");
  });
}

int fmskf_ingest_can(fmskf_handle h, const uint8_t *frames, const int16_t *stamps,
                     const uint8_t *present, uint32_t mem) {
  return guarded([&] {
    check_handle(h);
    if (!frames || !stamps) fail(FMSKF_EINVAL, "null frames/stamps");
    DeviceGuard g(h->cfg.device);
    const uint64_t n = h->s.n;
    ensure_motors(h);
    Stager sg(h, mem);
    const void *f = frames, *s = stamps, *p = present;
    sg.add(&f, n * 32);
    sg.add(&s, n * 8);
    sg.add(&p, n);
    sg.run();
    rs_prev_materialize(h);
    launch_check(launch_can(h->s, (const uint8_t *)f, (const int16_t *)s, (const uint8_t *)p,
                            h->cfg.motor_dir, h->stream),
                 "can launch");
    h->s.m_par ^= 1u;
    h->rs_prev_synced = false;
  });
}

int fmskf_correct(fmskf_handle h, const fmskf_tick_inputs *in) {
  return guarded([&] { run_tick(h, in, true, false, 1, h ? h->s.n : 0); });
}

int fmskf_predict(fmskf_handle h, const fmskf_tick_inputs *in) {
  return guarded([&] { run_tick(h, in, false, true, 1, h ? h->s.n : 0); });
}

int fmskf_tick(fmskf_handle h, const fmskf_tick_inputs *in) {
  return guarded([&] { run_tick(h, in, true, true, 1, h ? h->s.n : 0); });
}

int fmskf_tick_many(fmskf_handle h, const fmskf_tick_inputs *in, uint32_t n_ticks,
                    uint64_t tick_stride) {
  return guarded([&] { run_tick(h, in, true, true, n_ticks, tick_stride); });
}

int fmskf_get_pose(fmskf_handle h, float *x, float *y, float *th, uint32_t mem) {
  return guarded([&] {
    check_handle(h);
    DeviceGuard g(h->cfg.device);
    const uint64_t n = h->s.n;
    launch_check(launch_readout(h->s, h->readout, h->stream), "readout");
    copy_out(h, x, h->readout, n * 4, mem);
    copy_out(h, y, h->readout + n, n * 4, mem);
    copy_out(h, th, h->readout + 2 * n, n * 4, mem);
    finish_out(h, mem);
  });
}

int fmskf_get_vel(fmskf_handle h, float *vx, float *vy, float *vth, uint32_t mem) {
  return guarded([&] {
    check_handle(h);
    DeviceGuard g(h->cfg.device);
    const uint64_t n = h->s.n;
    launch_check(launch_readout(h->s, h->readout, h->stream), "readout");
    copy_out(h, vx, h->readout + 3 * n, n * 4, mem);
    copy_out(h, vy, h->readout + 4 * n, n * 4, mem);
    copy_out(h, vth, h->readout + 5 * n, n * 4, mem);
    finish_out(h, mem);
  });
}

int fmskf_get_state(fmskf_handle h, void *x, void *p_packed, uint32_t mem) {
  return guarded([&] {
    check_handle(h);
    DeviceGuard g(h->cfg.device);
    const uint64_t n = h->s.n;
    const Dims d = h->d;
    const size_t row = (size_t)n * d.elem, pb = (size_t)h->s.pitch * d.elem;
    const uint32_t np = d.nx * (d.nx + 1) / 2;
    if (p_packed && !d.m) fail(FMSKF_ENOTSUP, "RS model has no covariance");
    if (h->s.tile) {
      if (mem != FMSKF_MEM_HOST && mem != FMSKF_MEM_DEVICE) fail(FMSKF_EINVAL, "bad mem flag");
      auto out = [&](void *dst, const void *src, uint32_t rows) {
        if (!dst) return;
        void *dense = mem == FMSKF_MEM_DEVICE ? dst : h->out_for(row * rows);
        launch_check(launch_untile(src, dense, rows, n, d.elem, h->stream), "untile");
        if (mem == FMSKF_MEM_HOST) {
          copy_out(h, dst, dense, row * rows, mem);
          hip_check(hipStreamSynchronize(h->stream), "get_state sync");
        }
      };
      out(x, h->s.x, d.nx);
      if (p_packed) out(p_packed, h->s.P, np);
    } else {
      copy_planes_out(h, x, h->s.x, row, pb, d.nx, mem);
      if (p_packed) copy_planes_out(h, p_packed, h->s.P, row, pb, np, mem);
    }
    finish_out(h, mem);
  });
}

int fmskf_set_state(fmskf_handle h, const void *x, const void *p_packed, uint32_t mem) {
  return guarded([&] {
    check_handle(h);
    DeviceGuard g(h->cfg.device);
    const uint64_t n = h->s.n;
    const Dims d = h->d;
    if (mem != FMSKF_MEM_HOST && mem != FMSKF_MEM_DEVICE) fail(FMSKF_EINVAL, "bad mem flag");
    const size_t row = (size_t)n * d.elem, pb = (size_t)h->s.pitch * d.elem;
    const uint32_t np = d.nx * (d.nx + 1) / 2;
    if (p_packed && !d.m) fail(FMSKF_ENOTSUP, "RS model has no covariance");
    if (h->s.tile) {
      auto in = [&](void *dst, const void *src, uint32_t rows) {
        if (!src) return;
        const void *dense = src;
        if (mem == FMSKF_MEM_HOST) {
          void *stg = h->stage_for(row * rows);
          hip_check(hipMemcpyAsync(stg, src, row * rows, hipMemcpyHostToDevice, h->stream), "stage H2D");
          dense = stg;
        }
        launch_check(launch_tile(dense, dst, rows, n, d.elem, h->stream), "tile");
        if (mem == FMSKF_MEM_HOST) hip_check(hipStreamSynchronize(h->stream), "set_state sync");
      };
      in(h->s.x, x, d.nx);
      if (p_packed) in(h->s.P, p_packed, np);
    } else {
      if (x) copy_planes_in(h, h->s.x, x, row, pb, d.nx, mem);
      if (p_packed) copy_planes_in(h, h->s.P, p_packed, row, pb, np, mem);
    }
    if (x) h->ens_shift_ok = false;
    if (x && h->s.thlo) hip_check(hipMemsetAsync(h->s.thlo, 0, n * 4, h->stream), "heading low part");
    if ((x || p_packed) && h->s.xlo)
      hip_check(hipMemsetAsync(h->s.xlo, 0, (size_t)kKf6LoRows * h->s.pitch * 4, h->stream), "position low parts");
    finish_out(h, mem);
  });
}

int fmskf_set_gate(fmskf_handle h, const fmskf_gate *g) {
  return guarded([&] {
    check_handle(h);
    if (h->cfg.model != FMSKF_MODEL_KF6 || (h->cfg.flags & FMSKF_CFG_COMP_POS))
      fail(FMSKF_ENOTSUP, "the innovation gate is for KF6 without FMSKF_CFG_COMP_POS");
    if (h->capturing) fail(FMSKF_EINVAL, "gate changed inside a graph capture");
    if (!g) {
      h->gate_on = false;
      return;
    }
    if (!(g->nis_max > 0.0f)) fail(FMSKF_EINVAL, "nis_max must be > 0 (+INFINITY: monitor only)");
    DeviceGuard dg(h->cfg.device);
    if (!h->gate.word) {
      h->gate.word = h->alloc<uint32_t>(h->s.n);
      h->gate.nis = h->alloc<float>(h->s.n);
    }
    if (!h->gate_on) zero_gate(h);
    h->gate.nis_max = g->nis_max;
    h->gate.max_run = g->max_consecutive;
    h->gate_on = true;
  });
}

int fmskf_get_gate(fmskf_handle h, float *nis, uint8_t *status, uint8_t *run, uint32_t *rejects, uint32_t mem) {
  return guarded([&] {
    check_handle(h);
    if (!h->gate_on) fail(FMSKF_EINVAL, "no gate set (fmskf_set_gate)");
    if (mem != FMSKF_MEM_HOST && mem != FMSKF_MEM_DEVICE) fail(FMSKF_EINVAL, "bad mem flag");
    DeviceGuard dg(h->cfg.device);
    const uint64_t n = h->s.n;
    copy_out(h, nis, h->gate.nis, n * 4, mem);
    if (status || run || rejects) {
      if (mem == FMSKF_MEM_DEVICE) {
        launch_check(launch_gate_unpack(h->gate.word, n, status, run, rejects, h->stream), "gate readout");
      } else {
        char *scr = (char *)h->out_for(n * 6);
        launch_check(launch_gate_unpack(h->gate.word, n, (uint8_t *)scr + 4 * n, (uint8_t *)scr + 5 * n,
                                        (uint32_t *)scr, h->stream),
                     "gate readout");
        copy_out(h, rejects, scr, n * 4, mem);
        copy_out(h, status, scr + 4 * n, n, mem);
        copy_out(h, run, scr + 5 * n, n, mem);
      }
    }
    finish_out(h, mem);
  });
}

int fmskf_set_row_gate(fmskf_handle h, const fmskf_row_gate *g) {
  return guarded([&] {
    check_handle(h);
    if (h->cfg.model != FMSKF_MODEL_EKF9 || (h->cfg.flags & FMSKF_CFG_COMP_POS) || !h->s.tile)
      fail(FMSKF_ENOTSUP, "the row gate is for EKF9 without FMSKF_CFG_COMP_POS");
    if (!ekf9_r_diagonal(h->ekf9.r))
      fail(FMSKF_ENOTSUP, "the row gate needs a diagonal R (the sequential scalar update)");
    if (h->capturing) fail(FMSKF_EINVAL, "row gate changed inside a graph capture");
    if (!g) {
      h->rowgate_on = false;
      return;
    }
    for (int a = 0; a < FMSKF_EKF9_ROWS; a++)
      if (!(g->d2_max[a] > 0.0f)) fail(FMSKF_EINVAL, "d2_max entries must be > 0 (+INFINITY: never reject)");
    if (g->max_consecutive > 255) fail(FMSKF_EINVAL, "max_consecutive above 255 (the runs saturate there)");
    if (g->flags & ~FMSKF_ROW_GATE_D2) fail(FMSKF_EINVAL, "unknown row gate flags");
    DeviceGuard dg(h->cfg.device);
    if (!h->rowgate.word) {
      h->rowgate.word = h->alloc<uint64_t>(h->s.n);
      h->rowgate.d2_pitch = h->s.pitch;
      h->rowgate.d2 = h->alloc<float>((size_t)FMSKF_EKF9_ROWS * h->s.pitch);
    }
    if (!h->rowgate_on) zero_rowgate(h);
    for (int a = 0; a < FMSKF_EKF9_ROWS; a++) h->rowgate.d2_max[a] = g->d2_max[a];
    h->rowgate.max_run = g->max_consecutive;
    h->rowgate.flags = g->flags;
    h->rowgate_on = true;
  });
}

int fmskf_get_row_gate(fmskf_handle h, uint8_t *status, uint8_t *run, float *d2, uint32_t mem) {
  return guarded([&] {
    check_handle(h);
    if (!h->rowgate_on) fail(FMSKF_EINVAL, "no row gate set (fmskf_set_row_gate)");
    if (d2 && !(h->rowgate.flags & FMSKF_ROW_GATE_D2))
      fail(FMSKF_EINVAL, "d2 is kept only with FMSKF_ROW_GATE_D2");
    if (mem != FMSKF_MEM_HOST && mem != FMSKF_MEM_DEVICE) fail(FMSKF_EINVAL, "bad mem flag");
    DeviceGuard dg(h->cfg.device);
    const uint64_t n = h->s.n;
    const size_t rows = FMSKF_EKF9_ROWS;
    copy_planes_out(h, d2, h->rowgate.d2, n * 4, h->rowgate.d2_pitch * 4, rows, mem);
    if (status || run) {
      if (mem == FMSKF_MEM_DEVICE) {
        launch_check(launch_rowgate_unpack(h->rowgate.word, n, status, run, h->stream), "row gate readout");
      } else {
        uint8_t *scr = (uint8_t *)h->out_for(2 * rows * n);
        launch_check(launch_rowgate_unpack(h->rowgate.word, n, scr, scr + rows * n, h->stream), "row gate readout");
        copy_out(h, status, scr, rows * n, mem);
        copy_out(h, run, scr + rows * n, rows * n, mem);
      }
    }
    finish_out(h, mem);
  });
}

}
```

roboken-fmskf-robot-controller_amd/csrc/api_readout.cpp:

```cpp
#include "api_ctx.hpp"

using namespace fmskf;
using namespace fmskf::capi;

extern "C" {

int fmskf_get_prev_sum(fmskf_handle h, int64_t *prev, uint32_t mem) {
  return guarded([&] {
    check_handle(h);
    if (!h->s.prev_sum) fail(FMSKF_ENOTSUP, "prev_sum exists in the RS model only");
    DeviceGuard g(h->cfg.device);
    if (mem != FMSKF_MEM_HOST && mem != FMSKF_MEM_DEVICE) fail(FMSKF_EINVAL, "bad mem flag");
    rs_prev_materialize(h);
    if (!prev) return;
    const uint64_t n = h->s.n;
    int64_t *dense = mem == FMSKF_MEM_DEVICE ? prev : (int64_t *)h->out_for((size_t)4 * n * 8);
    launch_check(launch_prev_out(h->s.prev_sum, dense, n, n, h->stream), "previous sums");
    if (mem == FMSKF_MEM_HOST) copy_out(h, prev, dense, (size_t)4 * n * 8, mem);
    finish_out(h, mem);
  });
}

int fmskf_get_imu(fmskf_handle h, float *data, uint8_t *is_error, uint32_t mem) {
  return guarded([&] {
    check_handle(h);
    DeviceGuard g(h->cfg.device);
    ensure_imu(h);
    if (data) {
      if (mem != FMSKF_MEM_HOST && mem != FMSKF_MEM_DEVICE) fail(FMSKF_EINVAL, "bad mem flag");
      float *dst = mem == FMSKF_MEM_DEVICE ? data : (float *)h->out_for(16 * h->s.n * 4);
      launch_check(launch_imu_data(h->s, dst, h->stream), "imu data");
      if (mem == FMSKF_MEM_HOST) copy_out(h, data, dst, 16 * h->s.n * 4, mem);
    }
    copy_out(h, is_error, h->s.imu_err, h->s.n, mem);
    finish_out(h, mem);
  });
}

int fmskf_get_imu_regs(fmskf_handle h, int16_t *regs, uint8_t *pending, uint32_t mem) {
  return guarded([&] {
    check_handle(h);
    DeviceGuard g(h->cfg.device);
    ensure_imu(h);
    launch_check(launch_wt901_regs_sync(h->s, h->stream), "register file sync");
    copy_out(h, regs, h->s.imu_reg, 0x90 * h->s.n * 2, mem);
    copy_out(h, pending, h->s.imu_cnt, h->s.n, mem);
    finish_out(h, mem);
  });
}

int fmskf_get_motors(fmskf_handle h, int16_t *angle, int16_t *rpm, int16_t *curr,
                     int64_t *angle_sum, float *speed_radps, uint32_t mem) {
  return guarded([&] {
    check_handle(h);
    DeviceGuard g(h->cfg.device);
    if (mem != FMSKF_MEM_HOST && mem != FMSKF_MEM_DEVICE) fail(FMSKF_EINVAL, "bad mem flag");
    const uint64_t n = h->s.n;
    ensure_motors(h);
    copy_out(h, angle, motor_slots(h->s).angle, 4 * n * 2, mem);
    copy_out(h, rpm, h->s.m_rpm, 4 * n * 2, mem);
    copy_out(h, curr, h->s.m_curr, 4 * n * 2, mem);
    if (angle_sum) {
      int64_t *dense = mem == FMSKF_MEM_DEVICE ? angle_sum : (int64_t *)h->out_for((size_t)4 * n * 8);
      launch_check(launch_motor_sums(h->s.m_sum_lo, h->s.m_sum_hi, dense, n, n, false, h->stream), "motor sums");
      if (mem == FMSKF_MEM_HOST) copy_out(h, angle_sum, dense, (size_t)4 * n * 8, mem);
    }
    if (speed_radps) {
      if (mem == FMSKF_MEM_HOST) {
        std::vector<float> rows(4 * n);
        copy_out(h, rows.data(), h->s.m_iir_y, 4 * n * 4, mem);
        hip_check(hipStreamSynchronize(h->stream), "hipStreamSynchronize");
        for (uint64_t i = 0; i < n; i++)
          for (int w = 0; w < 4; w++) speed_radps[(size_t)w * n + i] = rows[4 * i + w];
      } else if (mem == FMSKF_MEM_DEVICE) {
        for (int w = 0; w < 4; w++)
          hip_check(hipMemcpy2DAsync(speed_radps + (size_t)w * n, 4, h->s.m_iir_y + w, 16, 4, n,
                                     hipMemcpyDeviceToDevice, h->stream),
                    "speed transpose");
      } else {
        fail(FMSKF_EINVAL, "bad mem flag");
      }
    }
    finish_out(h, mem);
  });
}

int fmskf_get_motor_status(fmskf_handle h, int16_t *microsec_id, int16_t *angle, int16_t *rpm,
                           int16_t *curr, float *dlt_out_angle_rad, float *speed_radps, uint32_t mem) {
  return guarded([&] {
    check_handle(h);
    if (mem != FMSKF_MEM_HOST && mem != FMSKF_MEM_DEVICE) fail(FMSKF_EINVAL, "bad mem flag");
    DeviceGuard g(h->cfg.device);
    const uint64_t n = h->s.n;
    ensure_motors(h);
    const MotorSlots ms = motor_slots(h->s);
    copy_out(h, microsec_id, ms.micro, 4 * n * 2, mem);
    copy_out(h, angle, ms.angle, 4 * n * 2, mem);
    copy_out(h, rpm, h->s.m_rpm, 4 * n * 2, mem);
    copy_out(h, curr, h->s.m_curr, 4 * n * 2, mem);
    if (dlt_out_angle_rad) {
      float *dst = mem == FMSKF_MEM_DEVICE ? dlt_out_angle_rad : (float *)h->out_for(4 * n * 4);
      launch_check(launch_motor_dlt(ms.angle, ms.prev, dst, 4 * n, h->stream), "motor dlt");
      if (mem == FMSKF_MEM_HOST) copy_out(h, dlt_out_angle_rad, dst, 4 * n * 4, mem);
    }
    copy_out(h, speed_radps, h->s.m_iir_y, 4 * n * 4, mem);
    finish_out(h, mem);
  });
}

int fmskf_get_state_lo(fmskf_handle h, float *lo, uint32_t *rows, uint32_t mem) {
  return guarded([&] {
    check_handle(h);
    if (mem != FMSKF_MEM_HOST && mem != FMSKF_MEM_DEVICE) fail(FMSKF_EINVAL, "bad mem flag");
    DeviceGuard g(h->cfg.device);
    const uint64_t n = h->s.n;
    const uint32_t rh = h->s.thlo ? 1u : 0u, rx = h->s.xlo ? kKf6LoRows : 0u;
    if (rows) *rows = rh + rx;
    if (!lo || !(rh + rx)) return;
    if (rh) copy_out(h, lo, h->s.thlo, n * 4, mem);
    if (rx) {
      float *dst = lo + (size_t)rh * n;
      void *dense = mem == FMSKF_MEM_DEVICE ? (void *)dst : h->out_for((size_t)rx * n * 4);
      launch_check(launch_untile(h->s.xlo, dense, rx, n, 4, h->stream), "untile");
      if (mem == FMSKF_MEM_HOST) copy_out(h, dst, dense, (size_t)rx * n * 4, mem);
    }
    finish_out(h, mem);
  });
}

int fmskf_set_state_lo(fmskf_handle h, const float *lo, uint32_t mem) {
  return guarded([&] {
    check_handle(h);
    if (mem != FMSKF_MEM_HOST && mem != FMSKF_MEM_DEVICE) fail(FMSKF_EINVAL, "bad mem flag");
    if (!lo) fail(FMSKF_EINVAL, "null lo");
    DeviceGuard g(h->cfg.device);
    const uint64_t n = h->s.n;
    const uint32_t rh = h->s.thlo ? 1u : 0u, rx = h->s.xlo ? kKf6LoRows : 0u, r = rh + rx;
    if (!r) fail(FMSKF_ENOTSUP, "this model keeps no low-part rows");
    const float *src = lo;
    if (mem == FMSKF_MEM_HOST) {
      void *stg = h->stage_for((size_t)r * n * 4);
      hip_check(hipMemcpyAsync(stg, lo, (size_t)r * n * 4, hipMemcpyHostToDevice, h->stream), "stage H2D");
      src = (const float *)stg;
    }
    if (rh) hip_check(hipMemcpyAsync(h->s.thlo, src, n * 4, hipMemcpyDeviceToDevice, h->stream), "lo");
    if (rx) launch_check(launch_tile(src + (size_t)rh * n, h->s.xlo, rx, n, 4, h->stream), "tile");
    h->ens_shift_ok = false;
    finish_out(h, FMSKF_MEM_HOST);
  });
}

int fmskf_get_counters(fmskf_handle h, uint64_t *counters, uint32_t n_counters) {
  return guarded([&] {
    check_handle(h);
    if (!counters || n_counters == 0) return;
    DeviceGuard g(h->cfg.device);
    unsigned long long tmp[8];
    hip_check(hipMemcpyAsync(tmp, h->s.counters, sizeof(tmp), hipMemcpyDeviceToHost, h->stream), "D2H");
    unsigned long long ignored = 0;
    hip_check(hipMemcpyAsync(&ignored, h->fix_ignored, sizeof(ignored), hipMemcpyDeviceToHost, h->stream), "D2H");
    unsigned long long sub_ignored = 0;
    hip_check(hipMemcpyAsync(&sub_ignored, h->subset_ignored, sizeof(sub_ignored), hipMemcpyDeviceToHost, h->stream),
              "D2H");
    unsigned long long rng_ignored = 0;
    hip_check(hipMemcpyAsync(&rng_ignored, h->range_ignored, sizeof(rng_ignored), hipMemcpyDeviceToHost, h->stream),
              "D2H");
    hip_check(hipStreamSynchronize(h->stream), "sync");
    tmp[1] = h->isr_can_split;
    tmp[2] = h->isr_ctrl_split;
    tmp[3] = ignored;
    tmp[4] = sub_ignored;
    tmp[5] = rng_ignored;
    for (uint32_t k = 0; k < n_counters && k < 8; k++) counters[k] = tmp[k];
  });
}

int fmskf_ensemble_record_len(fmskf_handle h, uint32_t *len) {
  return guarded([&] {
    check_handle(h);
    if (!len) fail(FMSKF_EINVAL, "null len");
    const uint32_t nx = h->d.nx;
    *len = 1 + nx + nx * (nx + 1) / 2;
  });
}

int fmskf_ensemble_partial(fmskf_handle h, double *out, uint32_t mem) {
  return guarded([&] {
    check_handle(h);
    if (!out) fail(FMSKF_EINVAL, "null out");
    DeviceGuard g(h->cfg.device);
    const uint32_t nx = h->d.nx;
    const uint32_t len = 1 + nx + nx * (nx + 1) / 2;
    double *dst = mem == FMSKF_MEM_DEVICE ? out : h->ens_out;
    ensure_shift(h);
    launch_check(launch_ensemble(h->s, (int)nx, h->d.elem == 8, h->ens_blocks, h->ens_shift, dst,
                                 h->stream),
                 "ensemble launch");
    if (mem == FMSKF_MEM_HOST) {
      copy_out(h, out, h->ens_out, len * 8, mem);
      finish_out(h, mem);
    } else if (mem != FMSKF_MEM_DEVICE) {
      fail(FMSKF_EINVAL, "bad mem flag");
    }
  });
}

int fmskf_tick_ensemble(fmskf_handle h, const fmskf_tick_inputs *in, double *out, uint32_t mem) {
  return guarded([&] {
    check_handle(h);
    if (!out) fail(FMSKF_EINVAL, "null out");
    if (mem != FMSKF_MEM_HOST && mem != FMSKF_MEM_DEVICE) fail(FMSKF_EINVAL, "bad mem flag");
    DeviceGuard g(h->cfg.device);
    const uint32_t nx = h->d.nx;
    const uint32_t len = 1 + nx + nx * (nx + 1) / 2;
    double *dst = mem == FMSKF_MEM_DEVICE ? out : h->ens_out;
    ensure_shift(h);
    if (fused_record(h)) {
      TickIn t = resolve_inputs(h, in, true, true, 1, h->s.n);
      t.ens_blocks = h->ens_blocks;
      t.ens_shift = h->ens_shift;
      int nb = 0;
      const bool libm = h->cfg.trig == FMSKF_TRIG_LIBM;
      h->time_begin();
      if (h->cfg.model == FMSKF_MODEL_KF6)
        launch_check(launch_kf6(h->s, t, h->kf6, libm, true, true, h->stream, &nb), "tick kernel launch");
      else if (h->cfg.model == FMSKF_MODEL_EKF9)
        launch_check(launch_ekf9(h->s, t, h->ekf9, libm, true, true, h->stream, &nb), "tick kernel launch");
      else
        launch_check(launch_kf12d(h->s, t, h->kf12, true, true, h->stream, &nb), "tick kernel launch");
      h->time_end();
      launch_check(launch_ens_fold((int)nx, h->ens_blocks, nb, h->ens_shift, dst, h->stream),
                   "ensemble fold launch");
    } else {
      run_tick(h, in, true, true, 1, h->s.n);
      launch_check(launch_ensemble(h->s, (int)nx, h->d.elem == 8, h->ens_blocks, h->ens_shift, dst,
                                   h->stream),
                   "ensemble launch");
    }
    if (mem == FMSKF_MEM_HOST) {
      copy_out(h, out, h->ens_out, len * 8, mem);
      finish_out(h, mem);
    }
  });
}

int fmskf_ensemble_combine(uint32_t n_state, const double *records, uint32_t n_records,
                           double *mean, double *cov_packed) {
  return guarded([&] {
    if (n_state == 0 || n_state > 12 || !records) fail(FMSKF_EINVAL, "bad arguments");
    const uint32_t nx = n_state, np = nx * (nx + 1) / 2, len = 1 + nx + np;
    std::vector<double> acc(len, 0.0);
    for (uint32_t r = 0; r < n_records; r++) {
      const double *b = records + (size_t)r * len;
      const double na = acc[0], nb = b[0];
      if (nb == 0.0) continue;
      if (na == 0.0) {
        acc.assign(b, b + len);
        continue;
      }
      const double nn = na + nb;
      double d[12];
      for (uint32_t k = 0; k < nx; k++) d[k] = b[1 + k] - acc[1 + k];
      const double f = na * nb / nn;
      for (uint32_t k = 0; k < nx; k++) acc[1 + k] = acc[1 + k] + d[k] * (nb / nn);
      for (uint32_t p = 0; p < nx; p++)
        for (uint32_t q = 0; q <= p; q++) {
          const uint32_t k = p * (p + 1) / 2 + q;
          acc[1 + nx + k] = acc[1 + nx + k] + b[1 + nx + k] + d[p] * d[q] * f;
        }
      acc[0] = nn;
    }
    if (mean)
      for (uint32_t k = 0; k < nx; k++) mean[k] = acc[1 + k];
    if (cov_packed)
      for (uint32_t k = 0; k < np; k++) cov_packed[k] = acc[0] > 1.0 ? acc[1 + nx + k] / (acc[0] - 1.0) : 0.0;
  });
}

}
```

roboken-fmskf-robot-controller_amd/csrc/fmskf_internal.hpp:

```cpp
#pragma once
#include <cstdlib>
#include <cmath>
#include <type_traits>
#include <hip/hip_runtime.h>
#include <hip/hip_ext.h>
#include <stdint.h>
#include "../../include/fmskf.h"
#include "launch_regime.hpp"

namespace fmskf {

constexpr int kBlock = 256;

constexpr int kSnapWords = 16, kRowWords = 12;
enum : int { kSnapValid = 1, kSnapLatched = 2 };

struct DevState {
  uint64_t n = 0;
  uint64_t pitch = 0;
  uint32_t tile = 0;
  uint32_t model = 0;
  void *x = nullptr;
  void *P = nullptr;
  int64_t *prev_sum = nullptr;
  float *thlo = nullptr;
  float *xlo = nullptr;
  int16_t *imu_reg = nullptr;
  uint32_t *imu_parser = nullptr;
  uint8_t *imu_cnt = nullptr;
  uint8_t *imu_flags = nullptr;
  uint8_t *imu_err = nullptr;
  float *imu_qinit = nullptr;
  int16_t *imu_snap = nullptr;
  int16_t *imu_mag = nullptr;
  uint32_t *imu_yg = nullptr;
  float *imu_qprev = nullptr;
  int16_t *m_micro = nullptr;
  int16_t *m_angle = nullptr;
  int16_t *m_prev = nullptr;
  int16_t *m_rpm = nullptr;
  int16_t *m_curr = nullptr;
  uint32_t *m_sum_lo = nullptr;
  int32_t *m_sum_hi = nullptr;
  float *m_iir_y = nullptr;
  int16_t *m_prev_micro = nullptr;
  uint32_t m_par = 0;
  unsigned long long *counters = nullptr;
  float *sintab = nullptr;
};

struct MotorSlots {
  int16_t *micro, *angle, *prev_micro, *prev;
};
inline MotorSlots motor_slots(const DevState &s) {
  return s.m_par ? MotorSlots{s.m_prev_micro, s.m_prev, s.m_micro, s.m_angle}
                 : MotorSlots{s.m_micro, s.m_angle, s.m_prev_micro, s.m_prev};
}

struct TickIn {
  const float *yaw_deg;
  const float *gyro_z;
  const int16_t *rpm;
  const int64_t *angle_sum;
  const int16_t *raw;
  const double *z;
  const uint8_t *valid;
  const uint32_t *rec;
  const float *sintab;
  uint64_t stride;
  uint64_t sum_pitch;
  const uint32_t *msum_lo;
  const int32_t *msum_hi;
  uint32_t n_ticks;
  double *ens_blocks;
  const double *ens_shift;
  uint32_t ens_grid;
  uint32_t fold_nb;
  const double *fold_blocks;
  double *fold_out;
  hipEvent_t ens_done;
  uint32_t imu_words;
};

template <typename A>
inline void launch_signal(void (*k)(A), dim3 g, unsigned lds, hipStream_t st, hipEvent_t done, const A &a) {
  if (done) hipExtLaunchKernelGGL(k, g, dim3(kBlock), lds, st, nullptr, done, 0u, a);
  else k<<<g, kBlock, lds, st>>>(a);
}

template <typename T, int NP, int MP>
struct KfParams {
  T dt;
  T q[NP];
  T r[MP];
};
struct Kf6Params {
  float dt;
  float q[21];
  float r[10];
  float *lo;
};
struct GateDev {
  uint32_t *word;
  float *nis;
  float nis_max;
  uint32_t max_run;
};
constexpr uint32_t kGateRunShift = 2, kGateRunMax = 255, kGateRejShift = 10, kGateRejMax = (1u << 22) - 1u;
struct RowGateDev {
  uint64_t *word;
  float *d2;
  uint64_t d2_pitch;
  float d2_max[6];
  uint32_t max_run;
  uint32_t flags;
};
struct PoseFixDev {
  const uint32_t *fixes;
  uint64_t count;
  float *nis;
  uint8_t *status;
  unsigned long long *ignored;
  float r[6];
  float nis_max;
  uint32_t m;
};
struct RangeDev {
  const uint32_t *fixes;
  uint64_t count;
  const float *anchors;
  uint32_t n_anchors;
  float *d2;
  uint8_t *status;
  unsigned long long *ignored;
  float tag[3];
  float var, d2_max, d_min;
};
struct SelectDev {
  uint32_t criteria;
  float pos_var_min;
  uint32_t run_min, row_mask;
  const uint32_t *gate_word;
  const uint64_t *rowgate_word;
  uint8_t *flag;
  uint32_t *blk, *chunk;
  uint32_t *robots;
  uint8_t *reason;
  uint64_t capacity;
  uint64_t *count;
};
constexpr uint32_t kSelChunk = 256;
struct SubsetDev {
  const uint32_t *robots;
  uint64_t count;
  float *x, *p, *lo;
  unsigned long long *ignored;
  bool set;
};
struct SmoothHist {
  float *x, *P;
  uint64_t sx, sp;
};
struct SmoothOut {
  float *x, *P;
  uint64_t pitch;
};
struct LoglikOut {
  uint32_t *n_meas;
  double *nis_sum, *logdet_sum, *innov_sum, *innov_outer;
  uint64_t pitch;
  double *partial;
  uint32_t accumulate;
};
struct EmOut {
  uint32_t *n_meas;
  double *sq, *sr;
  uint64_t pitch;
  double *partial;
  uint32_t accumulate;
};
struct TraceOut {
  float *nis;
  uint8_t *status;
  uint8_t *applied;
  float *x, *P;
  uint64_t pitch;
  uint32_t every;
};
struct Ekf9Params {
  float dt;
  float q[45];
  float r[21];
  float *thlo;
  float *clo;
};
struct Kf12dParams {
  double dt;
  double q[78];
  double r[36];
  double r2[10];
  double cinv[36];
  int decor;
  int sparse;
  const double *coef;
};
inline bool kf12d_sparse(const double *cinv36, const double *q78) {
  for (int a = 0; a < 8; a++)
    for (int b = 0; b < a; b++)
      if (!(a == 3 && b == 2) && cinv36[a * (a + 1) / 2 + b] != 0.0) return false;
  auto pair = [](int s) { return s < 6 ? s % 3 : 3 + (s - 6) % 3; };
  for (int i = 0; i < 12; i++)
    for (int j = 0; j <= i; j++)
      if (pair(i) != pair(j) && q78[i * (i + 1) / 2 + j] != 0.0) return false;
  return true;
}
inline bool kf12d_cinv(const double *r, double *ci) {
  auto pk2 = [](int i, int j) { return i >= j ? i * (i + 1) / 2 + j : j * (j + 1) / 2 + i; };
  double c[8][8] = {}, v[8][8] = {};
  for (int j = 0; j < 8; j++) {
    double s = r[pk2(j, j)];
    for (int k = 0; k < j; k++) s = s - c[j][k] * c[j][k];
    if (!(s > 0.0) || !std::isfinite(s)) return false;
    c[j][j] = std::sqrt(s);
    for (int i = j + 1; i < 8; i++) {
      double t = r[pk2(i, j)];
      for (int k = 0; k < j; k++) t = t - c[i][k] * c[j][k];
      c[i][j] = t / c[j][j];
    }
  }
  for (int j = 0; j < 8; j++) {
    v[j][j] = 1.0 / c[j][j];
    for (int i = j + 1; i < 8; i++) {
      double t = 0.0;
      for (int k = j; k < i; k++) t = t + c[i][k] * v[k][j];
      v[i][j] = -t / c[i][i];
    }
  }
  for (int i = 0; i < 8; i++)
    for (int j = 0; j <= i; j++) ci[pk2(i, j)] = v[i][j];
  return true;
}
inline bool kf12d_sequential(const double *r36) {
  for (int i = 4; i < 8; i++)
    for (int j = 0; j < 4; j++)
      if (r36[i * (i + 1) / 2 + j] != 0.0) return false;
  return true;
}

inline bool ekf9_r_diagonal(const float *r21) {
  for (int i = 1; i < 6; i++)
    for (int j = 0; j < i; j++)
      if (r21[i * (i + 1) / 2 + j] != 0.0f) return false;
  return true;
}

struct CtrlDev {
  uint64_t n = 0, pitch = 0;
  float *ax = nullptr;
  float *pid = nullptr;
  float *vel_tgt = nullptr;
  int16_t *rpm_prev = nullptr;
  int16_t *curr = nullptr;
  uint8_t *power = nullptr;
};
constexpr int kAxF = 12, kPidF = 6;
struct CtrlPrm {
  float freq, dt, ff_gain, p_gain, i_gain, d_gain, i_limit, ff_limit, a1, b0, b1, ts;
  int32_t curr_limit;
  int32_t dir[4];
  uint32_t store_derived;
};

inline uint64_t plane_pitch(uint64_t n) { return ((n + 511) / 512) * 512 + 256; }

template <typename T>
constexpr uint32_t tile_w() { return sizeof(T) == 8 ? 4096u : 2048u; }
inline uint32_t tile_w_elem(uint32_t elem) { return elem == 8 ? 4096u : 2048u; }

constexpr int kStateNT = 2;
#ifndef FMSKF_ST_CACHED
#define FMSKF_ST_CACHED 16
#endif
#ifndef FMSKF_ST_STREAM
#define FMSKF_ST_STREAM 2
#endif
constexpr int st_pol(int cp) { return cp == kStateNT ? FMSKF_ST_STREAM : FMSKF_ST_CACHED; }

inline uint64_t est_state_bytes(const DevState &s) { return est_state_bytes(s.model, s.xlo != nullptr); }

inline bool kf6_small(const DevState &s) { return s.pitch * 84 < 0xFFFFFFFFull; }
inline bool ctrl_small(const CtrlDev &c) { return c.pitch * 4 * 3 * kAxF < 0xFFFFFFFFull; }

template <class F>
inline auto with_bools(F &&f) { return f(); }
template <class F, class... Bs>
inline auto with_bools(F &&f, bool b, Bs... bs) {
  return b ? with_bools([&](auto... k) { return f(std::true_type{}, k...); }, bs...)
           : with_bools([&](auto... k) { return f(std::false_type{}, k...); }, bs...);
}

__host__ __device__ inline uint64_t st_at(uint32_t tile, uint64_t pitch, uint32_t rows, uint32_t k,
                                          uint64_t i) {
  return tile ? ((i / tile) * rows + k) * tile + i % tile : k * pitch + i;
}

struct Wt901Cfg {
  uint32_t read_reg_index;
};

int launch_rs(const DevState &s, const TickIn &in, bool libm, bool correct, bool predict,
              hipStream_t st);
int launch_kf6(const DevState &s, const TickIn &in, const Kf6Params &p, bool libm, bool upd,
               bool pred, hipStream_t st, int *ens_nb = nullptr);
int launch_kf6_gate(const DevState &s, const TickIn &in, const Kf6Params &p, const GateDev &g, bool libm,
                    bool pred, hipStream_t st);
int launch_kf6_smooth_fwd(const DevState &s, const TickIn &in, const Kf6Params &p, bool libm, const SmoothHist &hist,
                          hipStream_t st);
int launch_kf6_smooth_bwd(const DevState &s, const TickIn &in, const Kf6Params &p, bool libm, const SmoothHist &hist,
                          const SmoothOut &out, hipStream_t st);
int launch_kf6_loglik(const DevState &s, const TickIn &in, const Kf6Params &p, bool libm, const LoglikOut &out,
                      double *total, hipStream_t st);
int launch_kf6_em_bwd(const DevState &s, const TickIn &in, const Kf6Params &p, bool libm, const SmoothHist &hist,
                      const EmOut &out, double *total, hipStream_t st);
int launch_kf6_trace(const DevState &s, const TickIn &in, const Kf6Params &p, const GateDev *gate, bool libm,
                     const TraceOut &out, hipStream_t st);
int launch_gate_unpack(const uint32_t *word, uint64_t n, uint8_t *status, uint8_t *run, uint32_t *rejects,
                       hipStream_t st);
int launch_pose_fix(const DevState &s, const PoseFixDev &f, hipStream_t st);
int launch_range_fix(const DevState &s, const RangeDev &f, bool libm, hipStream_t st);
int launch_select(const DevState &s, const SelectDev &d, hipStream_t st);
int launch_state_subset(const DevState &s, const SubsetDev &d, hipStream_t st);
int launch_ekf9(const DevState &s, const TickIn &in, const Ekf9Params &p, bool libm, bool upd,
                bool pred, hipStream_t st, int *ens_nb = nullptr);
int launch_ekf9_rowgate(const DevState &s, const TickIn &in, const Ekf9Params &p, const RowGateDev &g,
                        bool libm, bool pred, hipStream_t st);
int launch_rowgate_unpack(const uint64_t *word, uint64_t n, uint8_t *status, uint8_t *run, hipStream_t st);
int launch_kf12d(const DevState &s, const TickIn &in, const Kf12dParams &p, bool upd, bool pred,
                 hipStream_t st, int *ens_nb = nullptr);
int launch_wt901(const DevState &s, const uint8_t *bytes, uint32_t stride, const uint32_t *len,
                 int latch_qinit, uint32_t read_reg_index, hipStream_t st);
int launch_can(const DevState &s, const uint8_t *frames, const int16_t *stamps,
               const uint8_t *present, const int8_t dir[4], hipStream_t st);
int launch_trig(const float *x, float *sv, float *cv, uint64_t n, bool libm, const float *tab,
                hipStream_t st);
int launch_ensemble(const DevState &s, int nx, bool f64, double *blocks, const double *shift,
                    double *out, hipStream_t st);
int launch_ens_fold(int nx, const double *blocks, int nb, const double *shift, double *out,
                    hipStream_t st);
int launch_ens_partial(const DevState &s, int nx, bool f64, double *blocks, const double *shift,
                       hipStream_t st, int *nb);
int launch_ens_shift(const DevState &s, int nx, bool f64, double *shift, hipStream_t st);
int ensemble_nblocks(uint64_t n);
int launch_ctrl_set_target(const CtrlDev &c, const float *vel, const float *acl, const float *jrk,
                           const uint8_t *mask, hipStream_t st);
int launch_ctrl_derive(const CtrlDev &c, const CtrlPrm &p, hipStream_t st);
int launch_ctrl_step(const CtrlDev &c, const CtrlPrm &p, const int16_t *rpm, uint32_t rstride,
                     hipStream_t st);
int launch_can_tx(const CtrlDev &c, uint8_t *frames, hipStream_t st);
int launch_isr_kf6(const DevState &s, const TickIn &in, const Kf6Params &kp, bool libm, const CtrlDev &c,
                   const CtrlPrm &p, uint8_t *frames, hipStream_t st);
int launch_isr_kf6_can(const DevState &s, const TickIn &in, const Kf6Params &kp, bool libm, const CtrlDev &c,
                       const CtrlPrm &p, uint8_t *frames, const uint8_t *can_frames, const int16_t *can_stamps,
                       const int8_t dir[4], hipStream_t st);
int launch_isr_ekf9(const DevState &s, const TickIn &in, const Ekf9Params &prm, bool libm, const CtrlDev &c,
                    const CtrlPrm &p, const int16_t *rpm, uint8_t *frames, hipStream_t st);
int launch_isr_ekf9_can(const DevState &s, const TickIn &in, const Ekf9Params &prm, bool libm, const CtrlDev &c,
                        const CtrlPrm &p, uint8_t *frames, const uint8_t *can_frames, const int16_t *can_stamps,
                        const int8_t dir[4], hipStream_t st);
int launch_prev_out(const int64_t *prev, int64_t *dst, uint64_t n, uint64_t pitch, hipStream_t st);
int launch_motor_sums(const uint32_t *lo, const int32_t *hi, int64_t *dst, uint64_t n, uint64_t pitch, bool to_prev,
                      hipStream_t st);
int launch_wt901_regs_sync(const DevState &s, hipStream_t st);
int launch_isr_rs_can(const DevState &s, const TickIn &in, bool libm, const CtrlDev &c, const CtrlPrm &p,
                      uint8_t *frames, const uint8_t *can_frames, const int16_t *can_stamps, const int8_t dir[4],
                      bool prev_in_sums, hipStream_t st);
int launch_isr_rs(const DevState &s, const TickIn &in, bool libm, const CtrlDev &c,
                  const CtrlPrm &p, uint8_t *frames, hipStream_t st);
int launch_imu_data(const DevState &s, float *out, hipStream_t st);
int launch_vehicle_info(const DevState &s, const float *readout, void *out, const uint8_t *floor,
                        const float *cam_pitch, const uint32_t *fault, hipStream_t st);
int launch_tiled_fill(void *base, uint32_t rows, uint64_t n, const uint64_t *bits, uint32_t elem,
                      hipStream_t st);
int launch_untile(const void *tiled, void *dense, uint32_t rows, uint64_t n, uint32_t elem,
                  hipStream_t st);
int launch_tile(const void *dense, void *tiled, uint32_t rows, uint64_t n, uint32_t elem,
                hipStream_t st);
int launch_readout(const DevState &s, float *out, hipStream_t st);
int launch_motor_dlt(const int16_t *angle, const int16_t *prev, float *out, uint64_t count, hipStream_t st);
int launch_motor_swap(const DevState &s, hipStream_t st);

}
```

roboken-fmskf-robot-controller_amd/csrc/kernels_kf6.hip:

```cpp
#include "ens_device.hpp"
#include "kf6_lane.hpp"

#pragma clang fp contract(off)

namespace fmskf {

template <int WPE, class O, class A = Kf6Args>
__global__ __launch_bounds__(kBlock) __attribute__((amdgpu_waves_per_eu(WPE, 8))) void k_kf6(A aa) {
  const Kf6Args &a = kf_args(aa);
  __shared__ float stab[O::LIBM ? 1 : 513];
  const uint64_t n = a.n;
  const uint32_t i = blockIdx.x * kBlock + threadIdx.x;
  const bool live = i < (uint32_t)n;
  const uint32_t ic = live ? i : (uint32_t)n - 1u;
  const uint32_t T = a.in.n_ticks;
  float x[6], P[21];
  Kf6Lo<O> lo;
  Kf6GateOf<O, A> gt;
  Kf6In ma, mb;
  kf6_load_state<O>(a.x, a.P, a.pitch, ic, x, P);
  const auto old = kf6_keep_old<kf6_mask<O>()>(P);
  kf6_load_lo<O>(a.prm.lo, ic, lo);
  gt.load(gate_dev(aa), ic, n);
  if (O::UPD) ma = kf6_load_in<O>(a.in, n, 0, ic);
  stage_table<O::LIBM>(stab, a.in.sintab);
  for (uint32_t t = 0; t < T; t += 2) {
    if (O::UPD && t + 1 < T) mb = kf6_load_in<O>(a.in, n, t + 1, ic);
    kf6_tick1<O>(ma, stab, a.prm, x, P, lo, gt);
    if (t + 1 >= T) break;
    if (O::UPD && t + 2 < T) ma = kf6_load_in<O>(a.in, n, t + 2, ic);
    kf6_tick1<O>(mb, stab, a.prm, x, P, lo, gt);
  }
  if (live) {
    kf6_store_state<O>(a.x, a.P, a.pitch, i, x, P, old);
    kf6_store_lo<O>(a.prm.lo, i, lo);
    gt.store(gate_dev(aa), i, n);
  }
  nan_guard(x, P, a.counters, live);
}

template <int WPE, class O>
__global__ __launch_bounds__(kBlock) __attribute__((amdgpu_waves_per_eu(WPE, 8))) void k_kf6t(Kf6Args a) {
  uint32_t bid = blockIdx.x;
  if constexpr (O::ENS || O::FOLD) {
    if (ens_fold_front<6>(a.in, bid)) return;
  }
  const uint64_t n = a.n;
  const uint32_t i = bid * kBlock + threadIdx.x;
  const bool live = i < (uint32_t)n;
  const uint32_t ic = live ? i : (uint32_t)n - 1u;
  float x[6], P[21];
  Kf6In m;
  __shared__ float wtab[O::LIBM ? 1 : kBlock / 64][O::LIBM ? 1 : kWaveTab];
  float *stab = wtab[O::LIBM ? 0 : threadIdx.x >> 6];
  WaveTable<O::LIBM> tv(a.in.sintab);
  Kf6Lo<O> lo;
  Kf6Gate<O, false> gt;
  kf6_load_state<O>(a.x, a.P, a.pitch, ic, x, P);
  const auto old = kf6_keep_old<kf6_mask<O>()>(P);
  kf6_load_lo<O>(a.prm.lo, ic, lo);
  if (O::UPD) m = kf6_load_in<O>(a.in, n, 0, ic);
  tv.store(stab);
  kf6_tick1<O>(m, stab, a.prm, x, P, lo, gt);
  if (live) {
    kf6_store_state<O>(a.x, a.P, a.pitch, i, x, P, old);
    kf6_store_lo<O>(a.prm.lo, i, lo);
  }
  nan_guard(x, P, a.counters, live);
  if constexpr (O::ENS) {
    float xs[1][6];
#pragma unroll
    for (int k = 0; k < 6; k++) xs[0][k] = x[k];
    const bool lv[1] = {live};
    ens_epilogue<6, 1>(a.in, xs, lv, bid);
  }
}

template <int WPE, int R, class O, class A = Kf6Args>
__global__ __launch_bounds__(kBlock) __attribute__((amdgpu_waves_per_eu(WPE, 8))) void k_kf6p(A aa) {
  const Kf6Args &a = kf_args(aa);
  uint32_t bid = blockIdx.x;
  if constexpr (O::ENS || O::FOLD) {
    if (ens_fold_front<6>(a.in, bid)) return;
  }
  const uint64_t n = a.n;
  const uint32_t nn = (uint32_t)n, last = nn - 1u;
  const uint32_t G = (O::ENS || O::FOLD ? a.in.ens_grid : gridDim.x) * kBlock;
  const uint32_t i0 = bid * kBlock + threadIdx.x;
  float x[6], P[21];
  __shared__ float wtab[O::LIBM ? 1 : kBlock / 64][O::LIBM ? 1 : kWaveTab];
  float *stab = wtab[O::LIBM ? 0 : threadIdx.x >> 6];
  WaveTable<O::LIBM> tv(a.in.sintab);
  Kf6In m[R];
  float xs[O::ENS ? R : 1][6];
  bool lv[R];
  if (O::UPD) {
#pragma unroll
    for (int r = 0; r < R; r++) m[r] = kf6_load_in<O>(a.in, n, 0, min(i0 + r * G, last));
  }
#pragma unroll
  for (int r = 0; r < R; r++) {
    const uint32_t i = i0 + r * G;
    const bool live = i < nn;
    Kf6Lo<O> lo;
    Kf6GateOf<O, A> gt;
    kf6_load_state<O>(a.x, a.P, a.pitch, live ? i : last, x, P);
    const auto old = kf6_keep_old<kf6_mask<O>()>(P);
    kf6_load_lo<O>(a.prm.lo, live ? i : last, lo);
    gt.load(gate_dev(aa), live ? i : last, n);
    if (r == 0) tv.store(stab);
    kf6_tick1<O>(m[r], stab, a.prm, x, P, lo, gt);
    if (live) {
      kf6_store_state<O>(a.x, a.P, a.pitch, i, x, P, old);
      kf6_store_lo<O>(a.prm.lo, i, lo);
      gt.store(gate_dev(aa), i, n);
    }
    nan_guard(x, P, a.counters, live);
    if constexpr (O::ENS) {
#pragma unroll
      for (int k = 0; k < 6; k++) xs[r][k] = x[k];
    }
    lv[r] = live;
  }
  if constexpr (O::ENS) ens_epilogue<6, R>(a.in, xs, lv, bid);
}

template <class A>
static void launch_fold(void (*k)(A), A a, unsigned g, unsigned lds, hipStream_t st) {
  a.in.ens_grid = g;
  launch_signal(k, dim3(g + (unsigned)EnsRec<6>::LEN), lds, st, a.in.ens_done, a);
}

template <class O, class A>
static void launch_one(const A &aa, unsigned lds, hipStream_t st) {
  const dim3 g = grid_for(kf_args(aa).n);
  if constexpr (std::is_same<A, GateArgs>::value) k_kf6p<4, 1, O, A><<<g, kBlock, lds, st>>>(aa);
  else if constexpr (O::FOLD) launch_fold(k_kf6t<4, O>, aa, g.x, lds, st);
  else k_kf6t<4, O><<<g, kBlock, lds, st>>>(aa);
}

template <class O, class A>
static void launch_o(const A &aa, hipStream_t st) {
  constexpr bool GATED = std::is_same<A, GateArgs>::value;
  const Kf6Args &a = kf_args(aa);
  if constexpr (GATED && !O::PRED) {
    launch_one<O>(aa, 0u, st);
  } else {
    if (a.in.n_ticks != 1) {
      k_kf6<4, O, A><<<grid_for(a.n), kBlock, 0, st>>>(aa);
      return;
    }
    const LaunchRegime r = kf6_regime(a.n, O::COMP, GATED, a.in.rec != nullptr);
    constexpr bool NT = O::UPD && O::PRED;
    if (r.two) {
      const unsigned g = (unsigned)((a.n + 2 * kBlock - 1) / (2 * kBlock));
      if constexpr (NT && !GATED) {
        const bool wide = !O::COMP && kf6_wide(a.n), fold = a.in.fold_blocks != nullptr;
        if (r.nt || wide || fold) {
          with_bools([&](auto N, auto W, auto F) {
            using ON = std::conditional_t<N(), WithNT<O>, O>;
            using OW = std::conditional_t<W() && !O::COMP, WithWide<ON>, ON>;
            if constexpr (F()) launch_fold(k_kf6p<4, 2, WithFold<OW>, A>, aa, g, r.lds, st);
            else k_kf6p<4, 2, OW, A><<<g, kBlock, r.lds, st>>>(aa);
          }, r.nt, wide, fold);
          return;
        }
      }
      k_kf6p<4, 2, O, A><<<g, kBlock, r.lds, st>>>(aa);
      return;
    }
    if constexpr (NT && !GATED) {
      if (a.in.fold_blocks) {
        with_bools([&](auto N) { launch_one<WithFold<std::conditional_t<N(), WithNT<O>, O>>>(aa, r.lds, st); }, r.nt);
        return;
      }
    }
    with_bools([&](auto N) { launch_one<std::conditional_t<N() && NT, WithNT<O>, O>>(aa, r.lds, st); }, r.nt);
  }
}

template <class O>
static int launch_ens_o(KfArgs<MdKF6, Kf6Params> a, hipStream_t st) {
  using E = WithEns<O>;
  const unsigned carry = a.in.fold_blocks ? (unsigned)EnsRec<6>::LEN : 0u;
  const LaunchRegime r = kf6_ens_regime(a.n, O::COMP);
  const unsigned g = r.two ? (unsigned)((a.n + 2 * kBlock - 1) / (2 * kBlock)) : grid_for(a.n).x;
  a.in.ens_grid = g;
  with_bools([&](auto TWO, auto N, auto W) {
    using EN = std::conditional_t<N(), WithNT<E>, E>;
    if constexpr (TWO()) {
      using EW = std::conditional_t<W() && !O::COMP, WithWide<EN>, EN>;
      launch_signal(k_kf6p<4, 2, EW>, dim3(g + carry), r.lds, st, a.in.ens_done, a);
    } else if constexpr (!W()) {
      launch_signal(k_kf6t<4, EN>, dim3(g + carry), r.lds, st, a.in.ens_done, a);
    }
  }, r.two, r.nt, r.two && !O::COMP && kf6_wide(a.n));
  return (int)g;
}

template <class O>
static void launch_sel(const KfArgs<MdKF6, Kf6Params> &a, hipStream_t st, int *ens_nb) {
  if constexpr (O::UPD && O::PRED) {
    if (ens_nb) {
      *ens_nb = launch_ens_o<O>(a, st);
      return;
    }
  }
  launch_o<O>(a, st);
}

int launch_kf6(const DevState &s, const TickIn &in, const Kf6Params &p, bool libm, bool upd,
               bool pred, hipStream_t st, int *ens_nb) {
  KfArgs<MdKF6, Kf6Params> a{s.n, s.pitch, (float *)s.x, (float *)s.P, in, s.counters, p};
  const bool small = kf6_small(s);
  const bool valid = upd && in.valid != nullptr, rec = upd && in.rec != nullptr;
  const bool comp = p.lo != nullptr;
  int *nb = in.ens_blocks && upd && pred && in.n_ticks == 1 ? ens_nb : nullptr;
  if ((in.ens_blocks && !nb) || (in.fold_blocks && !(upd && pred && in.n_ticks == 1)))
    return (int)hipErrorInvalidValue;
  if (upd) {
    with_bools([&](auto LIBM, auto PRED, auto REC, auto COMP, auto SMALL, auto VALID) {
      launch_sel<Opt<LIBM(), true, PRED(), SMALL(), VALID(), REC(), false, false, COMP()>>(a, st, nb);
    }, libm, pred, rec, comp, small, valid);
  } else {
    with_bools([&](auto LIBM, auto COMP) {
      launch_o<Opt<LIBM(), false, true, true, false, false, false, false, COMP()>>(a, st);
    }, libm, comp);
  }
  return (int)hipGetLastError();
}

int launch_kf6_gate(const DevState &s, const TickIn &in, const Kf6Params &p, const GateDev &g, bool libm,
                    bool pred, hipStream_t st) {
  if (p.lo || in.ens_blocks || in.fold_blocks || !g.word || !g.nis) return (int)hipErrorInvalidValue;
  if (!pred && in.n_ticks != 1) return (int)hipErrorInvalidValue;
  const GateArgs ga{{s.n, s.pitch, (float *)s.x, (float *)s.P, in, s.counters, p}, g};
  with_bools([&](auto LIBM, auto PRED, auto VALID, auto REC) {
    launch_o<Opt<LIBM(), true, PRED(), false, VALID(), REC()>>(ga, st);
  }, libm, pred, in.valid != nullptr, in.rec != nullptr);
  return (int)hipGetLastError();
}

}
```

roboken-fmskf-robot-controller_amd/csrc/kf6_lane.hpp:

```cpp
#pragma once
#include <type_traits>
#include "kf_generic.hpp"

#pragma clang fp contract(off)

namespace fmskf {

template <bool LIBM_, bool UPD_, bool PRED_, bool SMALL_, bool VALID_, bool REC_ = false, bool NT_ = false,
          bool ENS_ = false, bool COMP_ = false>
struct Opt {
  static constexpr bool LIBM = LIBM_, UPD = UPD_, PRED = PRED_, SMALL = SMALL_, VALID = VALID_,
                        REC = REC_, NT = NT_, ENS = ENS_, COMP = COMP_;
  static constexpr int CP = NT_ ? kStateNT : 0;
  static constexpr bool WIDE = false, FOLD = false;
  using Plain = Opt;
};
template <class O>
using WithNT = Opt<O::LIBM, O::UPD, O::PRED, O::SMALL, O::VALID, O::REC, true, O::ENS, O::COMP>;
template <class O>
using WithEns = Opt<O::LIBM, O::UPD, O::PRED, O::SMALL, O::VALID, O::REC, O::NT, true, O::COMP>;
template <class O>
using WithComp = Opt<O::LIBM, O::UPD, O::PRED, O::SMALL, O::VALID, O::REC, O::NT, O::ENS, true>;
template <class O, bool WIDE_, bool FOLD_>
struct OptX : O {
  static constexpr bool WIDE = WIDE_, FOLD = FOLD_;
};
template <class O>
using WithWide = OptX<typename O::Plain, true, O::FOLD>;
template <class O>
using WithFold = OptX<typename O::Plain, O::WIDE, true>;

constexpr unsigned kKf6CXM = kPosCXM;
constexpr unsigned long long kKf6CPM = kPosCPM;
template <class O>
struct Kf6Lo {
  float v[O::COMP ? kKf6LoRows : 1];
};

struct Kf6In {
  float yaw, gz;
  uint2 rpm;
  uint32_t valid;
};

using Kf6Args = KfArgs<MdKF6, Kf6Params>;
struct GateArgs {
  Kf6Args k;
  GateDev g;
};
struct NoGate {};
__host__ __device__ __forceinline__ const Kf6Args &kf_args(const Kf6Args &a) { return a; }
__host__ __device__ __forceinline__ const Kf6Args &kf_args(const GateArgs &a) { return a.k; }
__device__ __forceinline__ NoGate gate_dev(const Kf6Args &) { return {}; }
__device__ __forceinline__ const GateDev &gate_dev(const GateArgs &a) { return a.g; }

template <int CP = 0>
__device__ __forceinline__ float ld_f32(__amdgpu_buffer_rsrc_t r, uint32_t voff, uint32_t soff) {
  return __builtin_bit_cast(float, __builtin_amdgcn_raw_buffer_load_b32(r, voff, soff, CP));
}
template <int CP = 0>
__device__ __forceinline__ void st_f32(__amdgpu_buffer_rsrc_t r, uint32_t voff, uint32_t soff,
                                       float v) {
  __builtin_amdgcn_raw_buffer_store_b32(__builtin_bit_cast(uint32_t, v), r, voff, soff, CP);
}

#ifndef FMSKF_IN_CPOL
#define FMSKF_IN_CPOL 2
#endif
template <class O>
__device__ __forceinline__ Kf6In kf6_load_in(const TickIn &in, uint64_t n, uint64_t t, uint32_t i) {
  const uint64_t tb = t * in.stride;
  const uint32_t hb = O::SMALL ? 0u : __builtin_amdgcn_readfirstlane(i) & ~(uint32_t)(kBlock - 1);
  const uint32_t li = i - hb;
  const uint64_t base = tb + hb, left = n - hb;
  Kf6In m;
  if constexpr (O::REC) {
    const auto r = __builtin_amdgcn_raw_buffer_load_b128(rsrc(in.rec + base * 4, left * 16), li * 16u, 0,
                                                         FMSKF_IN_CPOL);
    const uint32_t w0 = r[0], w1 = r[1];
    m.yaw = __builtin_bit_cast(float, w0);
    m.gz = __builtin_bit_cast(float, w1);
    m.rpm = make_uint2(r[2], r[3]);
    m.valid = O::VALID ? (uint32_t)in.valid[tb + i] : 1u;
    return m;
  }
  const bool yw = (in.imu_words & 1u) != 0, gw = (in.imu_words & 2u) != 0;
  m.yaw = tick_yaw(yw, __builtin_amdgcn_raw_buffer_load_b32(rsrc(in.yaw_deg + base, left * 4), li * 4u, 0,
                                                            FMSKF_IN_CPOL));
  m.gz = tick_gz(gw, __builtin_amdgcn_raw_buffer_load_b32(rsrc(in.gyro_z + base, left * 4), li * 4u, 0,
                                                          FMSKF_IN_CPOL));
  const auto rr = __builtin_amdgcn_raw_buffer_load_b64(rsrc(in.rpm + base * 4, left * 8), li * 8u, 0,
                                                       FMSKF_IN_CPOL);
  m.rpm = make_uint2(rr[0], rr[1]);
  m.valid = O::VALID ? (uint32_t)in.valid[tb + i] : 1u;
  return m;
}

template <class O>
__device__ __forceinline__ void kf6_load_state(const float *xg, const float *Pg, uint64_t, uint32_t i,
                                               float (&x)[6], float (&P)[21]) {
  constexpr uint32_t W = tile_w<float>();
  const uint32_t tl = (uint32_t)__builtin_amdgcn_readfirstlane(i / W);
  const uint32_t c = (i - tl * W) * 4u;
  const auto rx = rsrc(xg + (uint64_t)tl * (6 * W), 6 * W * 4), rp = rsrc(Pg + (uint64_t)tl * (21 * W), 21 * W * 4);
#pragma unroll
  for (int k = 0; k < 6; k++) x[k] = ld_f32<O::CP>(rx, c, k * W * 4);
#pragma unroll
  for (int k = 0; k < 21; k++) P[k] = ld_f32<O::CP>(rp, c, k * W * 4);
}

#ifndef FMSKF_KF6_SKIP_MASK
#define FMSKF_KF6_SKIP_MASK ((1u << 3) | (1u << 4) | (1u << 15) | (1u << 16))
#endif
constexpr uint32_t kKf6SkipMask = FMSKF_KF6_SKIP_MASK;
constexpr uint32_t kKf6SkipWide = kKf6SkipMask | (1u << 8) | (1u << 12) | (1u << 18) | (1u << 19);
constexpr bool kf6_mask_ok(uint32_t m) { return (m >> 21) == 0 && (m & (uint32_t)kKf6CPM) == 0; }
static_assert(kf6_mask_ok(kKf6SkipMask) && kf6_mask_ok(kKf6SkipWide),
              "packed P planes only, none of the compensated ones");
template <class O>
constexpr uint32_t kf6_mask() {
  return O::WIDE ? kKf6SkipWide : kKf6SkipMask;
}
template <uint32_t M>
constexpr bool kf6_skip(int k) {
  return ((M >> k) & 1u) != 0;
}
template <uint32_t M>
constexpr int kf6_skip_slot(int k) {
  return __builtin_popcount(M & ((1u << k) - 1u));
}
template <uint32_t M = kKf6SkipMask>
struct Kf6Old {
  static_assert(kf6_mask_ok(M), "packed P planes only, none of the compensated ones");
  uint32_t v[__builtin_popcount(M) ? __builtin_popcount(M) : 1];
};
template <uint32_t M = kKf6SkipMask>
__device__ __forceinline__ Kf6Old<M> kf6_keep_old(const float (&P)[21]) {
  Kf6Old<M> o;
#pragma unroll
  for (int k = 0; k < 21; k++)
    if (kf6_skip<M>(k)) o.v[kf6_skip_slot<M>(k)] = __builtin_bit_cast(uint32_t, P[k]);
  return o;
}
template <int SP, uint32_t M>
__device__ __forceinline__ void kf6_st_p(__amdgpu_buffer_rsrc_t r, uint32_t voff, uint32_t soff, int k, float v,
                                         const Kf6Old<M> &old) {
  if (kf6_skip<M>(k) && __builtin_bit_cast(uint32_t, v) == old.v[kf6_skip_slot<M>(k)]) return;
  st_f32<SP>(r, voff, soff, v);
}

template <class O, uint32_t M>
__device__ __forceinline__ void kf6_store_state(float *xg, float *Pg, uint64_t, uint32_t i, const float (&x)[6],
                                                const float (&P)[21], const Kf6Old<M> &old) {
  constexpr int SP = st_pol(O::CP);
  constexpr uint32_t W = tile_w<float>();
  const uint32_t tl = (uint32_t)__builtin_amdgcn_readfirstlane(i / W);
  const uint32_t c = (i - tl * W) * 4u;
  const auto rx = rsrc(xg + (uint64_t)tl * (6 * W), 6 * W * 4), rp = rsrc(Pg + (uint64_t)tl * (21 * W), 21 * W * 4);
#pragma unroll
  for (int k = 0; k < 6; k++) st_f32<SP>(rx, c, k * W * 4, x[k]);
#pragma unroll
  for (int k = 0; k < 21; k++) kf6_st_p<SP>(rp, c, k * W * 4, k, P[k], old);
}

template <class O>
__device__ __forceinline__ void kf6_load_lo(const float *lg, uint32_t i, Kf6Lo<O> &l) {
  if constexpr (O::COMP) {
    constexpr uint32_t W = tile_w<float>();
    const uint32_t tl = (uint32_t)__builtin_amdgcn_readfirstlane(i / W);
    const uint32_t c = (i - tl * W) * 4u;
    const auto r = rsrc(lg + (uint64_t)tl * (kKf6LoRows * W), kKf6LoRows * W * 4);
#pragma unroll
    for (int k = 0; k < (int)kKf6LoRows; k++) l.v[k] = ld_f32<O::CP>(r, c, k * W * 4);
  }
}
template <class O>
__device__ __forceinline__ void kf6_store_lo(float *lg, uint32_t i, const Kf6Lo<O> &l) {
  if constexpr (O::COMP) {
    constexpr uint32_t W = tile_w<float>();
    const uint32_t tl = (uint32_t)__builtin_amdgcn_readfirstlane(i / W);
    const uint32_t c = (i - tl * W) * 4u;
    const auto r = rsrc(lg + (uint64_t)tl * (kKf6LoRows * W), kKf6LoRows * W * 4);
#pragma unroll
    for (int k = 0; k < (int)kKf6LoRows; k++) st_f32<st_pol(O::CP)>(r, c, k * W * 4, l.v[k]);
  }
}

__device__ __forceinline__ uint32_t gate_chunk(uint32_t ic) {
  return (uint32_t)__builtin_amdgcn_readfirstlane(ic) & ~(uint32_t)(kBlock - 1);
}
template <class O, bool ON_>
struct Kf6Gate {
  static constexpr bool ON = false;
  __device__ __forceinline__ void load(NoGate, uint32_t, uint64_t) {}
  __device__ __forceinline__ void store(NoGate, uint32_t, uint64_t) const {}
};
template <class O>
struct Kf6Gate<O, true> {
  static constexpr bool ON = true;
  static_assert(O::UPD && !O::COMP && !O::ENS, "the gate: plain state, no fused ensemble record");
  uint32_t hb, li, word, word0, max_run;
  float nis_max, nis;
  bool seen;
  __device__ __forceinline__ void load(const GateDev &g, uint32_t ic, uint64_t n) {
    hb = gate_chunk(ic);
    li = ic - hb;
    word = word0 = ld_chunk<uint32_t, O::CP>(g.word, hb, n, li);
    max_run = g.max_run;
    nis_max = g.nis_max;
    nis = 0.f;
    seen = false;
  }
  __device__ __forceinline__ void store(const GateDev &g, uint32_t, uint64_t n) const {
    if (word != word0) st_chunk<uint32_t, st_pol(O::CP)>(g.word, hb, n, li, word);
    if (seen) st_chunk<float, st_pol(O::CP)>(g.nis, hb, n, li, nis);
  }
};
template <class O, class A>
using Kf6GateOf = Kf6Gate<O, std::is_same<A, GateArgs>::value>;

template <bool LIBM>
__device__ __forceinline__ void stage_table(float *stab, const float *g) {
  if (!LIBM) {
    const int t = threadIdx.x;
    const float a = g[t], b = g[t + kBlock];
    const float c = t == 0 ? g[2 * kBlock] : 0.f;
    stab[t] = a;
    stab[t + kBlock] = b;
    if (t == 0) stab[2 * kBlock] = c;
    __syncthreads();
  }
}
static_assert(2 * kBlock + 1 == 513, "table staging assumes 256-thread blocks");

template <bool LIBM>
__device__ __forceinline__ void kf6_innov(const Kf6In &m, const float *tab, const float (&x)[6],
                                          float (&y)[4]) {
  int16_t r[4];
  unpack4(m.rpm, r);
  const float th = deg2rad(m.yaw);
  const float om = -deg2rad(m.gz);
  float vx, vy, vth;
  mdir_to_vdir(rpm_to_mvel(r[0]), rpm_to_mvel(r[1]), rpm_to_mvel(r[2]), rpm_to_mvel(r[3]), vx, vy,
               vth);
  const float c = cos_p<LIBM>(th, tab), s = sin_p<LIBM>(th, tab);
  const float z2 = (vx * c - vy * s) * 0.001f;
  const float z3 = (vx * s + vy * c) * 0.001f;
  y[0] = wrap_innov(th - x[2]);
  y[1] = om - x[5];
  y[2] = z2 - x[3];
  y[3] = z3 - x[4];
}

template <class O, class G>
__device__ __forceinline__ void kf6_tick1(const Kf6In &m, const float *tab, const Kf6Params &prm,
                                          float (&x)[6], float (&P)[21], Kf6Lo<O> &l, G &g) {
  if constexpr (G::ON) {
    uint32_t status = FMSKF_GATE_NONE;
    uint32_t run = (g.word >> kGateRunShift) & kGateRunMax, rej = g.word >> kGateRejShift;
    if (!O::VALID || m.valid) {
      float y[4], U[4][6], dinv[4], w[4];
      kf6_innov<O::LIBM>(m, tab, x, y);
      kf_update_factor<MdKF6>(P, y, prm.r, U, dinv, w);
      const float v = kf_nis(w, dinv);
      const bool forced = g.max_run > 0 && run >= g.max_run;
      const bool apply = forced || v <= g.nis_max;
      if (apply) kf_update_apply<MdKF6>(x, P, U, dinv, w);
      status = forced ? FMSKF_GATE_FORCED : apply ? FMSKF_GATE_ACCEPTED : FMSKF_GATE_REJECTED;
      run = apply ? 0u : min(run + 1u, kGateRunMax);
      rej = apply ? rej : min(rej + 1u, kGateRejMax);
      g.nis = v;
      g.seen = true;
    }
    g.word = status | (run << kGateRunShift) | (rej << kGateRejShift);
  } else if (O::UPD && (!O::VALID || m.valid)) {
    float y[4];
    kf6_innov<O::LIBM>(m, tab, x, y);
    if constexpr (O::COMP) kf_update<MdKF6, -1, float, 6, 4, 21, kKf6CXM, kKf6CPM>(x, P, y, prm.r, nullptr, l.v);
    else kf_update<MdKF6>(x, P, y, prm.r);
  }
  if (O::PRED) {
    const float dt = prm.dt;
    if constexpr (O::COMP) {
      th_add(x[0], l.v[0], dt * x[3]);
      th_add(x[1], l.v[1], dt * x[4]);
      th_norm(x[0], l.v[0]);
      th_norm(x[1], l.v[1]);
      x[2] = wrap_pi(dfma(dt, x[5], x[2]));
      kf_predict_cov_c<MdKF6, kKf6CXM, kKf6CPM>(P, [&](int, int) { return dt; }, prm.q, l.v);
    } else {
      x[0] = dfma(dt, x[3], x[0]);
      x[1] = dfma(dt, x[4], x[1]);
      x[2] = wrap_pi(dfma(dt, x[5], x[2]));
      kf_predict_cov<MdKF6>(P, [&](int, int) { return dt; }, prm.q);
    }
  }
}

}
```

roboken-fmskf-robot-controller_amd/csrc/launch_regime.hpp:

```cpp
#pragma once
#include <cstdint>
#include <cstdlib>
#include "../../include/fmskf.h"

namespace fmskf {

inline const char *env_knob(const char *name) { return getenv(name); }
#define FMSKF_ENV_INT(NAME, DFLT)                       \
  ([]() -> int {                                        \
    static const int v_ = [] {                          \
      const char *e_ = ::fmskf::env_knob(NAME);         \
      return e_ ? atoi(e_) : (int)(DFLT);               \
    }();                                                \
    return v_;                                          \
  }())
#define FMSKF_LDS_CAP(NAME, HBM, DFLT)                                 \
  ([&]() -> unsigned {                                                 \
    const int v_ = FMSKF_ENV_INT(NAME, -1);                            \
    return v_ >= 0 ? (unsigned)v_ : ((HBM) ? (unsigned)(DFLT) : 0u);   \
  }())

constexpr uint32_t kKf6LoRows = 5;
constexpr uint64_t xp_bytes(uint64_t nx, uint64_t elem) { return (nx + nx * (nx + 1) / 2) * elem; }
constexpr uint64_t kf6_state_bytes(bool comp, bool gated = false) {
  return xp_bytes(6, 4) + (comp ? kKf6LoRows * 4 : 0) + (gated ? 4 + 4 : 0);
}
constexpr uint64_t kKf6InBytes = 16;
constexpr uint64_t ekf9_state_bytes(bool comp, bool gated = false) {
  return xp_bytes(9, 4) + 4 + (comp ? kKf6LoRows * 4 : 0) + (gated ? 8 : 0);
}
constexpr uint64_t kKf12dStateBytes = xp_bytes(12, 8);
constexpr uint64_t kRsStateBytes = 6 * 4 + 4 * 8;
constexpr uint64_t kRsTickBytes = 2 * (3 * 4 + 4 * 8) + 4 * 8 + 4;
constexpr uint64_t kMotorStateBytes = 66, kCanInBytes = 40;
static_assert(kf6_state_bytes(false) == 108 && kf6_state_bytes(false, true) == 116 && kf6_state_bytes(true) == 128, "");
static_assert(ekf9_state_bytes(false) == 220 && ekf9_state_bytes(false, true) == 228 && ekf9_state_bytes(true) == 240, "");
static_assert(kKf12dStateBytes == 720 && kRsStateBytes == 56 && kRsTickBytes == 124, "");
static_assert(kf6_state_bytes(false) + kKf6InBytes == 124, "");

constexpr uint64_t est_state_bytes(uint32_t model, bool comp) {
  return model == FMSKF_MODEL_RS ? kRsStateBytes
         : model == FMSKF_MODEL_KF6 ? kf6_state_bytes(comp)
         : model == FMSKF_MODEL_EKF9 ? ekf9_state_bytes(comp)
                                     : kKf12dStateBytes;
}

constexpr uint64_t kInfinityCacheBytes = 256ull << 20;
constexpr bool fits_cache(uint64_t bytes) { return bytes <= kInfinityCacheBytes; }
constexpr bool fits_half_cache(uint64_t bytes) { return bytes <= kInfinityCacheBytes / 2; }

inline bool state_nt(uint64_t state_bytes) {
  const int force = FMSKF_ENV_INT("FMSKF_STATE_NT", -1);
  if (force >= 0) return force != 0;
  return !fits_cache(state_bytes);
}

struct LaunchRegime {
  bool two, nt;
  unsigned lds;
};

inline int kf6_variant() {
  const int x = FMSKF_ENV_INT("FMSKF_KF6_VARIANT", 0);
  return x == 12 || x == 15 ? x : 0;
}

inline LaunchRegime kf6_regime(uint64_t n, bool comp, bool gated, bool rec) {
  const int v = kf6_variant();
  const uint64_t sb = kf6_state_bytes(comp, gated), rb = sb + kKf6InBytes;
  const bool nt = state_nt(n * sb);
  if ((!gated || !nt) && (v == 12 || (v == 0 && fits_cache(n * rb)))) {
    if (v == 12) return {true, nt, 0u};
    const bool rec_half = rec && fits_half_cache(n * rb);
    return {true, nt, FMSKF_LDS_CAP("FMSKF_KF6P_LDS", true, rec_half ? 48u * 1024u : 32u * 1024u)};
  }
  return {false, nt, FMSKF_LDS_CAP("FMSKF_KF6_LDS", nt, 48u * 1024u)};
}

inline bool kf6_wide(uint64_t n) {
  const int force = FMSKF_ENV_INT("FMSKF_KF6_SKIP_WIDE", -1);
  if (force == 0 || force == 1) return force == 1;
  return fits_half_cache(n * (kf6_state_bytes(false) + kKf6InBytes));
}

inline LaunchRegime kf6_ens_regime(uint64_t n, bool comp) {
  const uint64_t sb = kf6_state_bytes(comp);
  const bool nt = state_nt(n * sb);
  if (fits_cache(n * (sb + kKf6InBytes))) return {true, nt, FMSKF_LDS_CAP("FMSKF_KF6PE_LDS", true, 32u * 1024u)};
  return {false, nt, FMSKF_LDS_CAP("FMSKF_KF6E_LDS", nt, 32u * 1024u)};
}

inline LaunchRegime ekf9_regime(uint64_t n, bool comp, bool gated, bool libm) {
  const uint64_t sb = ekf9_state_bytes(comp, gated);
  const bool nt = state_nt(n * sb);
  const int var = FMSKF_ENV_INT("FMSKF_EKF9_VARIANT", 0);
  const int v = var == 2 || var == 4 ? var : (fits_cache(n * sb) ? 2 : 4);
  if (!libm && v == 2) return {true, nt, FMSKF_LDS_CAP("FMSKF_EKF9P_LDS", true, 64u * 1024u)};
  if (libm) return {false, nt, 0u};
  return {false, nt, FMSKF_LDS_CAP("FMSKF_EKF9_LDS", nt, 64u * 1024u)};
}

inline LaunchRegime ekf9_ens_regime(uint64_t n, bool comp, bool libm) {
  const uint64_t sb = ekf9_state_bytes(comp);
  const bool nt = state_nt(n * sb);
  if (!libm && fits_cache(n * sb)) return {true, nt, FMSKF_LDS_CAP("FMSKF_EKF9P_LDS", true, 64u * 1024u)};
  return {false, nt, libm ? 0u : FMSKF_LDS_CAP("FMSKF_EKF9E_LDS", nt, 32u * 1024u)};
}

inline LaunchRegime kf12d_regime(uint64_t n) {
  const bool nt = state_nt(n * kKf12dStateBytes);
  return {false, nt, FMSKF_LDS_CAP("FMSKF_KF12D_LDS", nt, 0u)};
}

inline LaunchRegime rs_regime(uint64_t n) {
  const bool nt = state_nt(n * kRsTickBytes);
  return {FMSKF_ENV_INT("FMSKF_RS_TWO", 1) != 0, nt, FMSKF_LDS_CAP("FMSKF_RS_LDS", nt, 64u * 1024u)};
}

}
```

Before: 31.30 billion steps/s.

## Skip loading structurally-zero KF6 covariance planes using per-chunk device flags

Adds a per-64-instance device flag array recording whether the cross-covariance planes selected by the wide write-back mask are all zero after each tick. When the Q/R configuration keeps those entries structurally zero and the host can trust the flags (no intervening non-whitelisted API call, no graph capture), the KF6 tick kernel skips loading those P planes and materialises zeros instead. This cuts global memory reads in the memory-bound fused tick. In exchange it adds a flag read and write per chunk, host-side trust-tracking state on every API entry, and a correctness risk if the trust invalidation misses a path that mutates the state.

```diff
diff --git a/roboken-fmskf-robot-controller_amd/csrc/api_comm.cpp b/roboken-fmskf-robot-controller_amd/csrc/api_comm.cpp
--- a/roboken-fmskf-robot-controller_amd/csrc/api_comm.cpp
+++ b/roboken-fmskf-robot-controller_amd/csrc/api_comm.cpp
@@ -238,7 +238,7 @@
 
 int fmskf_comm_info(fmskf_handle h, int *world, int *rank) {
   return guarded([&] {
-    check_handle(h);
+    check_handle(h, Entry::comm_info);
     if (!h->comm) fail(FMSKF_EINVAL, "the handle has no communicator (fmskf_comm_init)");
     const RcclApi &a = need_rccl();
     int w = 0, r = -1;
@@ -324,10 +324,12 @@
     const bool libm = h->cfg.trig == FMSKF_TRIG_LIBM;
     h->time_begin();
     int e = 0;
-    if (h->cfg.model == FMSKF_MODEL_KF6) e = launch_kf6(h->s, t, h->kf6, libm, true, true, h->stream, &nb);
+    Kf6Zero z = zero_begin(h);
+    if (h->cfg.model == FMSKF_MODEL_KF6) e = launch_kf6(h->s, t, h->kf6, libm, true, true, h->stream, &nb, &z);
     else if (h->cfg.model == FMSKF_MODEL_EKF9) e = launch_ekf9(h->s, t, h->ekf9, libm, true, true, h->stream, &nb);
     else e = launch_kf12d(h->s, t, h->kf12, true, true, h->stream, &nb);
     launch_check(e, "tick kernel launch");
+    zero_launched(h, z);
     h->time_end();
     ens_carry_launched(h, C, t);
   } else {
@@ -365,7 +367,7 @@
 int fmskf_ensemble_end_count(fmskf_handle h, double *mean, double *cov_packed, double *count,
                              uint32_t *n_records) {
   return guarded([&] {
-    check_handle(h);
+    check_handle(h, Entry::ensemble_end);
     if (h->ens_pending == 0) fail(FMSKF_EINVAL, "no ensemble pending (fmskf_*ensemble_begin)");
     DeviceGuard g(h->cfg.device);
     fmskf_ctx::EnsSlot &S = h->eslot[h->ens_head];
@@ -393,7 +395,7 @@
 
 int fmskf_ensemble_exchange_ms(fmskf_handle h, float *ms) {
   return guarded([&] {
-    check_handle(h);
+    check_handle(h, Entry::ensemble_xms);
     if (!ms) fail(FMSKF_EINVAL, "null ms");
     *ms = h->ens_xms;
   });
diff --git a/roboken-fmskf-robot-controller_amd/csrc/api_ctrl.cpp b/roboken-fmskf-robot-controller_amd/csrc/api_ctrl.cpp
--- a/roboken-fmskf-robot-controller_amd/csrc/api_ctrl.cpp
+++ b/roboken-fmskf-robot-controller_amd/csrc/api_ctrl.cpp
@@ -380,7 +380,7 @@
 
 int fmskf_kernel_time_total(fmskf_handle h, double *total_ms, uint32_t *count) {
   return guarded([&] {
-    check_handle(h);
+    check_handle(h, Entry::timing);
     if (!total_ms || !count) fail(FMSKF_EINVAL, "null argument");
     DeviceGuard g(h->cfg.device);
     double sum = 0.0;
@@ -397,7 +397,7 @@
 
 int fmskf_last_kernel_ms(fmskf_handle h, float *ms) {
   return guarded([&] {
-    check_handle(h);
+    check_handle(h, Entry::timing);
     if (!ms) fail(FMSKF_EINVAL, "null ms");
     if (!h->timing) fail(FMSKF_EINVAL, "timing not enabled");
     DeviceGuard g(h->cfg.device);
diff --git a/roboken-fmskf-robot-controller_amd/csrc/api_ctx.hpp b/roboken-fmskf-robot-controller_amd/csrc/api_ctx.hpp
--- a/roboken-fmskf-robot-controller_amd/csrc/api_ctx.hpp
+++ b/roboken-fmskf-robot-controller_amd/csrc/api_ctx.hpp
@@ -134,6 +134,8 @@
   fmskf::Kf12dParams kf12{};
   bool gate_on = false;
   fmskf::GateDev gate{};
+  uint32_t *zero_flags = nullptr;
+  bool zero_ok = false, zero_trust = false, zero_prev = false;
   bool rowgate_on = false;
   fmskf::RowGateDev rowgate{};
   unsigned long long *fix_ignored = nullptr;
@@ -292,8 +294,33 @@
 namespace fmskf {
 namespace capi {
 
-inline void check_handle(fmskf_handle h) {
+enum class Entry {
+  other,
+  sync,
+  get_config,
+  get_counters,
+  comm_info,
+  ensemble_end,
+  ensemble_xms,
+  timing,
+  get_state,
+};
+constexpr bool keeps_zero_trust(Entry e) { return e != Entry::other; }
+
+inline void check_handle(fmskf_handle h, Entry e = Entry::other) {
   if (!h) fail(FMSKF_EINVAL, "null handle");
+  h->zero_prev = h->zero_trust;
+  h->zero_trust = keeps_zero_trust(e) && h->zero_prev;
+}
+inline Kf6Zero zero_begin(const fmskf_ctx *h) {
+  bool captured = h->capturing;
+  hipStreamCaptureStatus cs = hipStreamCaptureStatusNone;
+  if (!captured && h->zero_ok && h->stream)
+    captured = hipStreamIsCapturing(h->stream, &cs) != hipSuccess || cs != hipStreamCaptureStatusNone;
+  return {h->zero_ok && !captured ? h->zero_flags : nullptr, h->zero_prev, false};
+}
+inline void zero_launched(fmskf_ctx *h, const Kf6Zero &z) {
+  if (z.used) h->zero_trust = true;
 }
 
 
@@ -342,9 +369,9 @@
                       const std::vector<std::pair<const void **, size_t>> *extra = nullptr);
 void run_tick(fmskf_ctx *h, const fmskf_tick_inputs *in, bool upd, bool pred, uint32_t n_ticks,
               uint64_t stride);
-inline int kf6_tick_launch(fmskf_ctx *h, const TickIn &t, bool libm, bool upd, bool pred) {
+inline int kf6_tick_launch(fmskf_ctx *h, const TickIn &t, bool libm, bool upd, bool pred, Kf6Zero *z = nullptr) {
   if (h->gate_on && upd) return launch_kf6_gate(h->s, t, h->kf6, h->gate, libm, pred, h->stream);
-  return launch_kf6(h->s, t, h->kf6, libm, upd, pred, h->stream);
+  return launch_kf6(h->s, t, h->kf6, libm, upd, pred, h->stream, nullptr, z);
 }
 void zero_gate(fmskf_ctx *h);
 inline int ekf9_tick_launch(fmskf_ctx *h, const TickIn &t, bool libm, bool upd, bool pred) {
diff --git a/roboken-fmskf-robot-controller_amd/csrc/api_handle.cpp b/roboken-fmskf-robot-controller_amd/csrc/api_handle.cpp
--- a/roboken-fmskf-robot-controller_amd/csrc/api_handle.cpp
+++ b/roboken-fmskf-robot-controller_amd/csrc/api_handle.cpp
@@ -81,6 +81,10 @@
     for (int b = 0; b <= a; b++) h->kf12.r2[a * (a + 1) / 2 + b] = c.r[(a + 4) * (a + 5) / 2 + (b + 4)];
   h->kf12.decor = kf12d_cinv(h->kf12.r, h->kf12.cinv) ? 1 : 0;
   h->kf12.sparse = h->kf12.decor && kf12d_sparse(h->kf12.cinv, h->kf12.q) ? 1 : 0;
+  bool ok = c.model == FMSKF_MODEL_KF6 && !(c.flags & FMSKF_CFG_COMP_POS);
+  for (int k : {3, 4, 8, 12, 15, 16, 18, 19}) ok = ok && h->kf6.q[k] == 0.f;
+  for (int k : {3, 4, 6, 7}) ok = ok && h->kf6.r[k] == 0.f;
+  h->zero_ok = ok;
 }
 
 }
@@ -343,13 +347,15 @@
   if (rs_pred) rs_prev_materialize(h);
   h->time_begin();
   int e = 0;
+  Kf6Zero z = zero_begin(h);
   switch (h->cfg.model) {
     case FMSKF_MODEL_RS: e = launch_rs(h->s, t, libm, upd, pred, h->stream); break;
-    case FMSKF_MODEL_KF6: e = kf6_tick_launch(h, t, libm, upd, pred); break;
+    case FMSKF_MODEL_KF6: e = kf6_tick_launch(h, t, libm, upd, pred, &z); break;
     case FMSKF_MODEL_EKF9: e = ekf9_tick_launch(h, t, libm, upd, pred); break;
     case FMSKF_MODEL_KF12D: e = launch_kf12d(h->s, t, h->kf12, upd, pred, h->stream); break;
   }
   launch_check(e, "tick kernel launch");
+  zero_launched(h, z);
   ens_carry_launched(h, C, t);
   if (rs_pred) h->rs_prev_synced = t.msum_lo != nullptr;
   h->time_end();
@@ -504,6 +510,11 @@
       s.thlo = cfg->model == FMSKF_MODEL_EKF9 ? h->alloc<float>(n) : nullptr;
       s.xlo = (cfg->flags & FMSKF_CFG_COMP_POS) ? h->alloc<float>((size_t)kKf6LoRows * s.pitch) : nullptr;
       h->kf6.lo = s.xlo;
+      if (cfg->model == FMSKF_MODEL_KF6) {
+        const size_t words = (size_t)((n + 63) / 64);
+        h->zero_flags = h->alloc<uint32_t>(words);
+        hip_check(hipMemset(h->zero_flags, 0, words * 4), "zero flags");
+      }
       s.counters = h->alloc<unsigned long long>(8);
       h->fix_ignored = h->alloc<unsigned long long>(1);
       h->subset_ignored = h->alloc<unsigned long long>(1);
@@ -633,7 +644,7 @@
 
 int fmskf_sync(fmskf_handle h) {
   return guarded([&] {
-    check_handle(h);
+    check_handle(h, Entry::sync);
     DeviceGuard g(h->cfg.device);
     hip_check(hipStreamSynchronize(h->stream), "hipStreamSynchronize");
   });
@@ -641,7 +652,7 @@
 
 int fmskf_get_config(fmskf_handle h, fmskf_config *out) {
   return guarded([&] {
-    check_handle(h);
+    check_handle(h, Entry::get_config);
     if (!out) fail(FMSKF_EINVAL, "null out");
     *out = h->cfg;
   });
@@ -712,7 +723,7 @@
 
 int fmskf_get_pose(fmskf_handle h, float *x, float *y, float *th, uint32_t mem) {
   return guarded([&] {
-    check_handle(h);
+    check_handle(h, Entry::get_state);
     DeviceGuard g(h->cfg.device);
     const uint64_t n = h->s.n;
     launch_check(launch_readout(h->s, h->readout, h->stream), "readout");
@@ -725,7 +736,7 @@
 
 int fmskf_get_vel(fmskf_handle h, float *vx, float *vy, float *vth, uint32_t mem) {
   return guarded([&] {
-    check_handle(h);
+    check_handle(h, Entry::get_state);
     DeviceGuard g(h->cfg.device);
     const uint64_t n = h->s.n;
     launch_check(launch_readout(h->s, h->readout, h->stream), "readout");
@@ -738,7 +749,7 @@
 
 int fmskf_get_state(fmskf_handle h, void *x, void *p_packed, uint32_t mem) {
   return guarded([&] {
-    check_handle(h);
+    check_handle(h, Entry::get_state);
     DeviceGuard g(h->cfg.device);
     const uint64_t n = h->s.n;
     const Dims d = h->d;
diff --git a/roboken-fmskf-robot-controller_amd/csrc/api_readout.cpp b/roboken-fmskf-robot-controller_amd/csrc/api_readout.cpp
--- a/roboken-fmskf-robot-controller_amd/csrc/api_readout.cpp
+++ b/roboken-fmskf-robot-controller_amd/csrc/api_readout.cpp
@@ -152,7 +152,7 @@
 
 int fmskf_get_counters(fmskf_handle h, uint64_t *counters, uint32_t n_counters) {
   return guarded([&] {
-    check_handle(h);
+    check_handle(h, Entry::get_counters);
     if (!counters || n_counters == 0) return;
     DeviceGuard g(h->cfg.device);
     unsigned long long tmp[8];
@@ -222,9 +222,11 @@
       int nb = 0;
       const bool libm = h->cfg.trig == FMSKF_TRIG_LIBM;
       h->time_begin();
-      if (h->cfg.model == FMSKF_MODEL_KF6)
-        launch_check(launch_kf6(h->s, t, h->kf6, libm, true, true, h->stream, &nb), "tick kernel launch");
-      else if (h->cfg.model == FMSKF_MODEL_EKF9)
+      if (h->cfg.model == FMSKF_MODEL_KF6) {
+        Kf6Zero z = zero_begin(h);
+        launch_check(launch_kf6(h->s, t, h->kf6, libm, true, true, h->stream, &nb, &z), "tick kernel launch");
+        zero_launched(h, z);
+      } else if (h->cfg.model == FMSKF_MODEL_EKF9)
         launch_check(launch_ekf9(h->s, t, h->ekf9, libm, true, true, h->stream, &nb), "tick kernel launch");
       else
         launch_check(launch_kf12d(h->s, t, h->kf12, true, true, h->stream, &nb), "tick kernel launch");
diff --git a/roboken-fmskf-robot-controller_amd/csrc/fmskf_internal.hpp b/roboken-fmskf-robot-controller_amd/csrc/fmskf_internal.hpp
--- a/roboken-fmskf-robot-controller_amd/csrc/fmskf_internal.hpp
+++ b/roboken-fmskf-robot-controller_amd/csrc/fmskf_internal.hpp
@@ -310,8 +310,13 @@
 
 int launch_rs(const DevState &s, const TickIn &in, bool libm, bool correct, bool predict,
               hipStream_t st);
+struct Kf6Zero {
+  uint32_t *flags;
+  bool trusted;
+  bool used;
+};
 int launch_kf6(const DevState &s, const TickIn &in, const Kf6Params &p, bool libm, bool upd,
-               bool pred, hipStream_t st, int *ens_nb = nullptr);
+               bool pred, hipStream_t st, int *ens_nb = nullptr, Kf6Zero *z = nullptr);
 int launch_kf6_gate(const DevState &s, const TickIn &in, const Kf6Params &p, const GateDev &g, bool libm,
                     bool pred, hipStream_t st);
 int launch_kf6_smooth_fwd(const DevState &s, const TickIn &in, const Kf6Params &p, bool libm, const SmoothHist &hist,
diff --git a/roboken-fmskf-robot-controller_amd/csrc/kernels_kf6.hip b/roboken-fmskf-robot-controller_amd/csrc/kernels_kf6.hip
--- a/roboken-fmskf-robot-controller_amd/csrc/kernels_kf6.hip
+++ b/roboken-fmskf-robot-controller_amd/csrc/kernels_kf6.hip
@@ -94,6 +94,11 @@
   Kf6In m[R];
   float xs[O::ENS ? R : 1][6];
   bool lv[R];
+  uint32_t zf[O::ZL ? R : 1];
+  if constexpr (O::ZL) {
+#pragma unroll
+    for (int r = 0; r < R; r++) zf[r] = kf6_zero_flag(aa.flags, min(i0 + r * G, last));
+  }
   if (O::UPD) {
 #pragma unroll
     for (int r = 0; r < R; r++) m[r] = kf6_load_in<O>(a.in, n, 0, min(i0 + r * G, last));
@@ -104,7 +109,8 @@
     const bool live = i < nn;
     Kf6Lo<O> lo;
     Kf6GateOf<O, A> gt;
-    kf6_load_state<O>(a.x, a.P, a.pitch, live ? i : last, x, P);
+    if constexpr (O::ZL) kf6_load_state_zl<O>(a.x, a.P, live ? i : last, aa.trusted && zf[r], x, P);
+    else kf6_load_state<O>(a.x, a.P, a.pitch, live ? i : last, x, P);
     const auto old = kf6_keep_old<kf6_mask<O>()>(P);
     kf6_load_lo<O>(a.prm.lo, live ? i : last, lo);
     gt.load(gate_dev(aa), live ? i : last, n);
@@ -115,6 +121,10 @@
       kf6_store_lo<O>(a.prm.lo, i, lo);
       gt.store(gate_dev(aa), i, n);
     }
+    if constexpr (O::ZL) {
+      const uint32_t nf = kf6_zero_now(P) ? 1u : 0u;
+      if (live && (threadIdx.x & 63u) == 0 && (!aa.trusted || nf != zf[r])) aa.flags[i / kZeroChunk] = nf;
+    }
     nan_guard(x, P, a.counters, live);
     if constexpr (O::ENS) {
 #pragma unroll
@@ -126,9 +136,9 @@
 }
 
 template <class A>
-static void launch_fold(void (*k)(A), A a, unsigned g, unsigned lds, hipStream_t st) {
-  a.in.ens_grid = g;
-  launch_signal(k, dim3(g + (unsigned)EnsRec<6>::LEN), lds, st, a.in.ens_done, a);
+static void launch_fold(void (*k)(A), A aa, unsigned g, unsigned lds, hipStream_t st) {
+  kf_args_mut(aa).in.ens_grid = g;
+  launch_signal(k, dim3(g + (unsigned)EnsRec<6>::LEN), lds, st, kf_args(aa).in.ens_done, aa);
 }
 
 template <class O, class A>
@@ -140,7 +150,7 @@
 }
 
 template <class O, class A>
-static void launch_o(const A &aa, hipStream_t st) {
+static void launch_o(const A &aa, hipStream_t st, Kf6Zero *z = nullptr) {
   constexpr bool GATED = std::is_same<A, GateArgs>::value;
   const Kf6Args &a = kf_args(aa);
   if constexpr (GATED && !O::PRED) {
@@ -156,13 +166,21 @@
       const unsigned g = (unsigned)((a.n + 2 * kBlock - 1) / (2 * kBlock));
       if constexpr (NT && !GATED) {
         const bool wide = !O::COMP && kf6_wide(a.n), fold = a.in.fold_blocks != nullptr;
+        const bool zl = wide && z && z->flags && kf6_zero_loads(a.n);
         if (r.nt || wide || fold) {
-          with_bools([&](auto N, auto W, auto F) {
+          with_bools([&](auto N, auto W, auto F, auto Z) {
             using ON = std::conditional_t<N(), WithNT<O>, O>;
             using OW = std::conditional_t<W() && !O::COMP, WithWide<ON>, ON>;
-            if constexpr (F()) launch_fold(k_kf6p<4, 2, WithFold<OW>, A>, aa, g, r.lds, st);
-            else k_kf6p<4, 2, OW, A><<<g, kBlock, r.lds, st>>>(aa);
-          }, r.nt, wide, fold);
+            if constexpr (Z() && W() && !O::COMP) {
+              const ZeroArgs za{aa, z->flags, z->trusted ? 1u : 0u};
+              if constexpr (F()) launch_fold(k_kf6p<4, 2, WithZero<WithFold<OW>>, ZeroArgs>, za, g, r.lds, st);
+              else k_kf6p<4, 2, WithZero<OW>, ZeroArgs><<<g, kBlock, r.lds, st>>>(za);
+              z->used = true;
+            } else if constexpr (!Z()) {
+              if constexpr (F()) launch_fold(k_kf6p<4, 2, WithFold<OW>, A>, aa, g, r.lds, st);
+              else k_kf6p<4, 2, OW, A><<<g, kBlock, r.lds, st>>>(aa);
+            }
+          }, r.nt, wide, fold, zl);
           return;
         }
       }
@@ -180,37 +198,45 @@
 }
 
 template <class O>
-static int launch_ens_o(KfArgs<MdKF6, Kf6Params> a, hipStream_t st) {
+static int launch_ens_o(KfArgs<MdKF6, Kf6Params> a, hipStream_t st, Kf6Zero *z) {
   using E = WithEns<O>;
   const unsigned carry = a.in.fold_blocks ? (unsigned)EnsRec<6>::LEN : 0u;
   const LaunchRegime r = kf6_ens_regime(a.n, O::COMP);
   const unsigned g = r.two ? (unsigned)((a.n + 2 * kBlock - 1) / (2 * kBlock)) : grid_for(a.n).x;
   a.in.ens_grid = g;
-  with_bools([&](auto TWO, auto N, auto W) {
+  const bool wide = r.two && !O::COMP && kf6_wide(a.n);
+  with_bools([&](auto TWO, auto N, auto W, auto Z) {
     using EN = std::conditional_t<N(), WithNT<E>, E>;
     if constexpr (TWO()) {
       using EW = std::conditional_t<W() && !O::COMP, WithWide<EN>, EN>;
-      launch_signal(k_kf6p<4, 2, EW>, dim3(g + carry), r.lds, st, a.in.ens_done, a);
-    } else if constexpr (!W()) {
+      if constexpr (Z() && W() && !O::COMP) {
+        const ZeroArgs za{a, z->flags, z->trusted ? 1u : 0u};
+        launch_signal(k_kf6p<4, 2, WithZero<EW>, ZeroArgs>, dim3(g + carry), r.lds, st, a.in.ens_done, za);
+        z->used = true;
+      } else if constexpr (!Z()) {
+        launch_signal(k_kf6p<4, 2, EW>, dim3(g + carry), r.lds, st, a.in.ens_done, a);
+      }
+    } else if constexpr (!W() && !Z()) {
       launch_signal(k_kf6t<4, EN>, dim3(g + carry), r.lds, st, a.in.ens_done, a);
     }
-  }, r.two, r.nt, r.two && !O::COMP && kf6_wide(a.n));
+  }, r.two, r.nt, wide, wide && z && z->flags && kf6_zero_loads(a.n));
   return (int)g;
 }
 
 template <class O>
-static void launch_sel(const KfArgs<MdKF6, Kf6Params> &a, hipStream_t st, int *ens_nb) {
+static void launch_sel(const KfArgs<MdKF6, Kf6Params> &a, hipStream_t st, int *ens_nb, Kf6Zero *z) {
   if constexpr (O::UPD && O::PRED) {
     if (ens_nb) {
-      *ens_nb = launch_ens_o<O>(a, st);
+      *ens_nb = launch_ens_o<O>(a, st, z);
       return;
     }
   }
-  launch_o<O>(a, st);
+  launch_o<O>(a, st, z);
 }
 
 int launch_kf6(const DevState &s, const TickIn &in, const Kf6Params &p, bool libm, bool upd,
-               bool pred, hipStream_t st, int *ens_nb) {
+               bool pred, hipStream_t st, int *ens_nb, Kf6Zero *z) {
+  if (z) z->used = false;
   KfArgs<MdKF6, Kf6Params> a{s.n, s.pitch, (float *)s.x, (float *)s.P, in, s.counters, p};
   const bool small = kf6_small(s);
   const bool valid = upd && in.valid != nullptr, rec = upd && in.rec != nullptr;
@@ -220,7 +246,7 @@
     return (int)hipErrorInvalidValue;
   if (upd) {
     with_bools([&](auto LIBM, auto PRED, auto REC, auto COMP, auto SMALL, auto VALID) {
-      launch_sel<Opt<LIBM(), true, PRED(), SMALL(), VALID(), REC(), false, false, COMP()>>(a, st, nb);
+      launch_sel<Opt<LIBM(), true, PRED(), SMALL(), VALID(), REC(), false, false, COMP()>>(a, st, nb, z);
     }, libm, pred, rec, comp, small, valid);
   } else {
     with_bools([&](auto LIBM, auto COMP) {
diff --git a/roboken-fmskf-robot-controller_amd/csrc/kf6_lane.hpp b/roboken-fmskf-robot-controller_amd/csrc/kf6_lane.hpp
--- a/roboken-fmskf-robot-controller_amd/csrc/kf6_lane.hpp
+++ b/roboken-fmskf-robot-controller_amd/csrc/kf6_lane.hpp
@@ -12,7 +12,7 @@
   static constexpr bool LIBM = LIBM_, UPD = UPD_, PRED = PRED_, SMALL = SMALL_, VALID = VALID_,
                         REC = REC_, NT = NT_, ENS = ENS_, COMP = COMP_;
   static constexpr int CP = NT_ ? kStateNT : 0;
-  static constexpr bool WIDE = false, FOLD = false;
+  static constexpr bool WIDE = false, FOLD = false, ZL = false;
   using Plain = Opt;
 };
 template <class O>
@@ -29,6 +29,13 @@
 using WithWide = OptX<typename O::Plain, true, O::FOLD>;
 template <class O>
 using WithFold = OptX<typename O::Plain, O::WIDE, true>;
+template <class O>
+struct OptZ : O {
+  static_assert(O::WIDE && !O::COMP, "zero-load skipping rides on the wide write-back mask");
+  static constexpr bool ZL = true;
+};
+template <class O>
+using WithZero = OptZ<O>;
 
 constexpr unsigned kKf6CXM = kPosCXM;
 constexpr unsigned long long kKf6CPM = kPosCPM;
@@ -48,10 +55,19 @@
   Kf6Args k;
   GateDev g;
 };
+struct ZeroArgs {
+  Kf6Args k;
+  uint32_t *flags;
+  uint32_t trusted;
+};
 struct NoGate {};
 __host__ __device__ __forceinline__ const Kf6Args &kf_args(const Kf6Args &a) { return a; }
 __host__ __device__ __forceinline__ const Kf6Args &kf_args(const GateArgs &a) { return a.k; }
+__host__ __device__ __forceinline__ const Kf6Args &kf_args(const ZeroArgs &a) { return a.k; }
+inline Kf6Args &kf_args_mut(Kf6Args &a) { return a; }
+inline Kf6Args &kf_args_mut(ZeroArgs &a) { return a.k; }
 __device__ __forceinline__ NoGate gate_dev(const Kf6Args &) { return {}; }
+__device__ __forceinline__ NoGate gate_dev(const ZeroArgs &) { return {}; }
 __device__ __forceinline__ const GateDev &gate_dev(const GateArgs &a) { return a.g; }
 
 template <int CP = 0>
@@ -161,6 +177,44 @@
   for (int k = 0; k < 6; k++) st_f32<SP>(rx, c, k * W * 4, x[k]);
 #pragma unroll
   for (int k = 0; k < 21; k++) kf6_st_p<SP>(rp, c, k * W * 4, k, P[k], old);
+}
+
+#ifndef FMSKF_KF6_ZERO_LOAD_MASK
+#define FMSKF_KF6_ZERO_LOAD_MASK kKf6SkipWide
+#endif
+constexpr uint32_t kKf6ZeroLoad = FMSKF_KF6_ZERO_LOAD_MASK;
+static_assert(kKf6ZeroLoad != 0 && (kKf6ZeroLoad & ~kKf6SkipWide) == 0, "cross planes of the wide mask only");
+constexpr uint32_t kZeroChunk = 64;
+__device__ __forceinline__ uint32_t kf6_zero_flag(const uint32_t *flags, uint32_t ic) {
+  return flags[(uint32_t)__builtin_amdgcn_readfirstlane(ic) / kZeroChunk];
+}
+template <class O>
+__device__ __forceinline__ void kf6_load_state_zl(const float *xg, const float *Pg, uint32_t i, bool skip,
+                                                  float (&x)[6], float (&P)[21]) {
+  constexpr uint32_t W = tile_w<float>();
+  const uint32_t tl = (uint32_t)__builtin_amdgcn_readfirstlane(i / W);
+  const uint32_t c = (i - tl * W) * 4u;
+  const auto rx = rsrc(xg + (uint64_t)tl * (6 * W), 6 * W * 4), rp = rsrc(Pg + (uint64_t)tl * (21 * W), 21 * W * 4);
+#pragma unroll
+  for (int k = 0; k < 6; k++) x[k] = ld_f32<O::CP>(rx, c, k * W * 4);
+#pragma unroll
+  for (int k = 0; k < 21; k++)
+    if (!kf6_skip<kKf6ZeroLoad>(k)) P[k] = ld_f32<O::CP>(rp, c, k * W * 4);
+#pragma unroll
+  for (int k = 0; k < 21; k++)
+    if (kf6_skip<kKf6ZeroLoad>(k)) asm volatile("v_mov_b32 %0, 0" : "=v"(P[k]));
+  if (!skip) {
+#pragma unroll
+    for (int k = 0; k < 21; k++)
+      if (kf6_skip<kKf6ZeroLoad>(k)) P[k] = ld_f32<O::CP>(rp, c, k * W * 4);
+  }
+}
+__device__ __forceinline__ bool kf6_zero_now(const float (&P)[21]) {
+  uint32_t any = 0;
+#pragma unroll
+  for (int k = 0; k < 21; k++)
+    if (kf6_skip<kKf6ZeroLoad>(k)) any |= __builtin_bit_cast(uint32_t, P[k]);
+  return __builtin_amdgcn_ballot_w64(any != 0) == 0;
 }
 
 template <class O>
diff --git a/roboken-fmskf-robot-controller_amd/csrc/launch_regime.hpp b/roboken-fmskf-robot-controller_amd/csrc/launch_regime.hpp
--- a/roboken-fmskf-robot-controller_amd/csrc/launch_regime.hpp
+++ b/roboken-fmskf-robot-controller_amd/csrc/launch_regime.hpp
@@ -83,6 +83,12 @@
   return fits_half_cache(n * (kf6_state_bytes(false) + kKf6InBytes));
 }
 
+inline bool kf6_zero_loads(uint64_t n) {
+  const int force = FMSKF_ENV_INT("FMSKF_KF6_ZERO_LOADS", -1);
+  if (force == 0 || force == 1) return force == 1;
+  return fits_half_cache(n * (kf6_state_bytes(false) + kKf6InBytes));
+}
+
 inline LaunchRegime kf6_ens_regime(uint64_t n, bool comp) {
   const uint64_t sb = kf6_state_bytes(comp);
   const bool nt = state_nt(n * sb);
```

After: 33.49 billion steps/s, median of 6. +7.0%, better.
